# Cibiv/NextGenMap

Hardware: AMD Instinct MI355X
Metric: mapped reads/sec + SW Gcells/sec, 150bp vs GRCh38, at 1/2/4/8 MI355X (higher is better)
Workload: dtype int32

## Files before the change

include/ngm_pipeline.h:

```cpp
#ifndef NGM_PIPELINE_H
#define NGM_PIPELINE_H

#include <stddef.h>
#include <stdint.h>

#ifdef __cplusplus
extern "C" {
#endif

typedef struct ngm_ref ngm_ref;
typedef struct ngm_mapper ngm_mapper;

typedef struct ngm_ref_params {
	int kmer;
	int kmer_skip;
	int bin_size;
} ngm_ref_params;

const char *ngm_pipeline_last_error(void);

ngm_ref *ngm_ref_create(int device, const ngm_ref_params *p, int n_contigs, const char *const *names,
		const uint8_t *const *seqs, const uint64_t *lens);
ngm_ref *ngm_ref_create_from_fasta(int device, const ngm_ref_params *p, const char *path);
ngm_ref *ngm_ref_create_from_cache(int device, const ngm_ref_params *params, const char *fasta_path);
// ... 85 lines not shown
	int paired;
	int min_insert_size, max_insert_size;
	int min_mq;
	float min_identity, min_residues;
	int no_unal;
	const char *rg_id;
	int bs_mapping;
	int slam_seq;
	int bam;
} ngm_sam_options;
int ngm_mapper_set_sam_options(ngm_mapper *m, const ngm_sam_options *o);
typedef struct ngm_sam_read {
	uint32_t name_off;
	uint16_t name_len;
	uint16_t qual_len;
} ngm_sam_read;
long long ngm_mapper_map_sam(ngm_mapper *m, int n, const char *reads, const char *quals, const char *names, size_t names_bytes,
		const ngm_sam_read *meta, char *out, size_t out_cap, uint64_t stats[3], float *kernel_ms);
long long ngm_mapper_map_sam_trimmed(ngm_mapper *m, int n, const char *reads, const char *quals, const char *names, size_t names_bytes,
		const ngm_sam_read *meta, const uint16_t *polya_trimmed, char *out, size_t out_cap, uint64_t stats[3], float *kernel_ms);
int ngm_mapper_sam_fetch(ngm_mapper *m, char *out, size_t out_cap);

typedef struct ngm_pair_state ngm_pair_state;
ngm_pair_state *ngm_pair_state_create(void);
void ngm_pair_state_destroy(ngm_pair_state *ps);
int ngm_mapper_set_pair_state(ngm_mapper *m, ngm_pair_state *ps);
int ngm_mapper_set_batch_seq(ngm_mapper *m, uint64_t seq);
int ngm_mapper_set_fast_pairing(ngm_mapper *m, int on);

typedef struct ngm_bgzf ngm_bgzf;
ngm_bgzf *ngm_bgzf_create(int device);
void ngm_bgzf_destroy(ngm_bgzf *z);
size_t ngm_bgzf_bound(size_t n);
long long ngm_bgzf_compress(ngm_bgzf *z, const void *raw, size_t n, void *out, size_t out_cap);
long long ngm_bgzf_compress_device(ngm_bgzf *z, const void *d_raw, size_t n, void *out, size_t out_cap);
float ngm_bgzf_last_kernel_ms(const ngm_bgzf *z);
size_t ngm_bgzf_inflated_size(const void *members, size_t n);
long long ngm_bgzf_inflate(ngm_bgzf *z, const void *members, size_t n, void *out, size_t out_cap);

typedef struct ngm_bam_sort ngm_bam_sort;
typedef struct ngm_bam_sort_params {
	int device;
	size_t chunk_bytes;
	size_t max_bytes;
} ngm_bam_sort_params;
ngm_bam_sort *ngm_bam_sort_create(const ngm_bam_sort_params *p);
void ngm_bam_sort_destroy(ngm_bam_sort *s);
int ngm_bam_sort_add(ngm_bam_sort *s, uint64_t seq, const void *records, size_t n_bytes);
int ngm_bam_sort_finish(ngm_bam_sort *s, int n_ref);
long long ngm_bam_sort_next(ngm_bam_sort *s, void *out, size_t out_cap);
long long ngm_bam_sort_index(ngm_bam_sort *s, uint64_t first_member_offset, void *out, size_t out_cap);
int ngm_bam_sort_stats(const ngm_bam_sort *s, uint64_t counts[5], float ms[5]);
int ngm_mapper_set_bam_sorter(ngm_mapper *m, ngm_bam_sort *s);

void *ngm_host_alloc(size_t bytes);
void ngm_host_free(void *p);

int ngm_host_pin_to_device_node(int device);

int ngm_mapper_set_reference_score_buffer(ngm_mapper *m, int entries);
int ngm_mapper_lost_pairs(ngm_mapper *m, uint64_t *out);
int ngm_mapper_set_reference_cs_batch(ngm_mapper *m, int reads);

int ngm_mapper_path_counters(ngm_mapper *m, uint64_t out[8]);

int ngm_mapper_order_table_reads(ngm_mapper *m, uint64_t *out);

int ngm_debug_pair_walk(uint32_t cnt_a, int len_a, uint32_t cnt_b, int len_b, const uint32_t *loc, const uint32_t *sv, const float *score, const uint32_t *rank,
		float cutoff, int min_insert, int max_insert, uint32_t *out_a, uint32_t *out_b, int *mq_a, int *mq_b, uint64_t cap, float *combo_score, int *combo_dist, int *combo_a, int *combo_b,
		uint64_t *n_combo);

int ngm_debug_pair_eval(uint64_t n, const float *pair_score, const int *dist, const int *ia, const int *ib, int avg, int out_all[6], int out_kept[6]);

int ngm_debug_select_top1(int device, int n_reads, const uint32_t *base, const uint32_t *count, uint64_t n_cand, const float *scores, const uint32_t *loc,
		const uint32_t *strand_votes, uint32_t *winner, int32_t *mapq, int32_t *n_best, float *best_score);

int ngm_debug_align_finish(void *engine , int mode, int n, const char *const *ref, const char *const *qry, void *out ,
		uint64_t *n_fallback);

int ngm_debug_expand_pairs(int device, int n_reads, const uint32_t *base, const uint32_t *count, uint64_t n_cand, uint32_t *out);

int ngm_mapper_heavy_counters(ngm_mapper *m, uint64_t out[4]);

int ngm_mapper_cs_counters(ngm_mapper *m, uint64_t out[3]);

typedef struct ngm_stats_comm ngm_stats_comm;
int ngm_stats_unique_id(char hex[257]);
ngm_stats_comm *ngm_stats_comm_create(int device, int rank, int world, const char *hex);
int ngm_stats_allreduce(ngm_stats_comm *c, int64_t v[8]);
void ngm_stats_comm_destroy(ngm_stats_comm *c);
int ngm_mapper_last_pair_stats(ngm_mapper *m, uint64_t out[3]);

int ngm_mapper_last_kernel_ms(ngm_mapper *m, float ms[8]);
float ngm_mapper_last_order_replay_ms(ngm_mapper *m);

int ngm_mapper_set_argos(ngm_mapper *m, float min_score);
long long ngm_mapper_map_argos(ngm_mapper *m, int n, const char *reads, const char *names, size_t names_bytes, const ngm_sam_read *meta,
		char *out, size_t out_cap, uint64_t stats[3], float *kernel_ms);
int ngm_argos_prolog(const ngm_ref *ref, uint64_t total_reads, char *out, size_t cap);
int ngm_mapper_argos_counters(ngm_mapper *m, uint64_t out[4]);
int ngm_mapper_argos_path_counters(ngm_mapper *m, uint64_t out[2]);
int ngm_debug_argos_order(uint32_t n, const float *score, const uint32_t *rank, float min_score, int read_len, int match_bonus, uint32_t *order, uint32_t out[3]);

#ifdef __cplusplus
}
#endif
#endif
```

nextgenmap_amd/csrc/cigar_device.h:

```cpp
#pragma once

#include <hip/hip_runtime.h>
#include <stdint.h>

#include "sw_device.h"
#include "affine_device.h"

namespace ngm {

struct CigarDevOut {
	uint32_t cig_off, md_off;
	uint16_t cig_len, md_len;
	int32_t position_offset, qstart, qend, nm;
	float identity, score_token;
	int32_t flags;
};

__device__ __forceinline__ uint32_t packed_class(const uint32_t *base, int m_base, int j) {
	const uint32_t w = base[(size_t) (m_base + (j >> 3)) * kSlots];
	const int b = j & 7;
	return (b < 4) ? (w >> (8 * b)) & 15u : (w >> (8 * (b - 4) + 4)) & 15u;
}
__device__ __forceinline__ char class_to_char(uint32_t c) {
	switch (c) { case 0: return 'A'; case 1: return 'C'; case 2: return 'G'; case 3: return 'T'; case 4: return 'x'; case 5: return 'N'; default: return 0; }
// ... 78 lines not shown
						if (rc == 4u) odd_symbol = true;
						const bool eq = (op == 1) && ((variant_cpu && !alt) ? (rc <= 3u && rc == fc) : (rc == fc));
						if (eq) { match += 1; md_eq += 1; in_x_run = false; }
						else {
							if (alt && rc == bs_from && fc == bs_to) match += 1; else mismatch += 1;
							if (mo > lim) { fits = false; break; }
							if (!in_x_run) { mo += dev_put_num(mdp + mo, md_eq); md_eq = 0; in_x_run = true; }
							mdp[mo++] = class_to_char(fc);
						}
						m_len += 1; ref_i += 1; read_i += 1;
					}
				} else if (op == 3) {
					in_x_run = false;
					if (m_len > 0) { co += dev_put_num(cg + co, m_len); cg[co++] = 'M'; m_len = 0; }
					co += dev_put_num(cg + co, len); cg[co++] = 'D';
					mo += dev_put_num(mdp + mo, md_eq); md_eq = 0;
					mdp[mo++] = '^';
					for (int t = 0; t < len; ++t) { if (mo > lim) { fits = false; break; } mdp[mo++] = class_to_char(fclass(ref0 + ref_i)); ref_i += 1; }
					mismatch += len;
				} else {
					in_x_run = false;
					if (m_len > 0) { co += dev_put_num(cg + co, m_len); cg[co++] = 'M'; m_len = 0; }
					co += dev_put_num(cg + co, len); cg[co++] = 'I';
					read_i += len;
					mismatch += len;
				}
			}
			if (co > lim || mo > lim) fits = false;
			if (fits) {
				mo += dev_put_num(mdp + mo, md_eq);
				if (m_len > 0) { co += dev_put_num(cg + co, m_len); cg[co++] = 'M'; }
				if (trail > 0) {
					if (hard_clip == 1) { co += dev_put_num(cg + co, trail); cg[co++] = 'H'; }
					else if (silent_clip != 1) { co += dev_put_num(cg + co, trail); cg[co++] = 'S'; }
					o.qend = trail;
				}
			}
			o.identity = (float) match * 1.0f / (float) total;
			o.nm = mismatch;
			o.score_token = (float) read_i;
			o.position_offset = ref0;
			o.flags = ((fits && !odd_symbol) ? 1 : 0) | 2;
		}
	}
	}
	o.cig_len = (uint16_t) co; o.md_len = (uint16_t) mo;
	const uint32_t need = (live && (o.flags & 1)) ? (uint32_t) (co + mo) : 0u;
	uint32_t incl = need;
	const int lane = threadIdx.x & 63, wv = threadIdx.x >> 6;
#pragma unroll
	for (int d = 1; d < 64; d <<= 1) { const uint32_t t = __shfl_up(incl, d); if (lane >= d) incl += t; }
	if (lane == 63) s_wave[wv] = incl;
	__syncthreads();
	uint32_t before = incl - need, total = 0;
#pragma unroll
	for (int w2 = 0; w2 < 4; ++w2) { if (w2 < wv) before += s_wave[w2]; total += s_wave[w2]; }
	if (threadIdx.x == 0) s_base = total ? atomicAdd(cursor, (unsigned long long) total) : 0ull;
	__syncthreads();
	const unsigned long long base = s_base;
	if (!live) return;
	if (need) {
		if (base + total > capacity) o.flags &= ~1;
		else {
			const unsigned long long off = base + before;
			o.cig_off = (uint32_t) off; o.md_off = (uint32_t) off + o.cig_len;
			for (int t = 0; t < co; ++t) bytes[off + t] = cg[t];
			for (int t = 0; t < mo; ++t) bytes[off + co + t] = mdp[t];
		}
	}
	out[j] = o;
}

constexpr int kFinishRows = 8;

__device__ __forceinline__ uint32_t finish_sel8(uint32_t w0, uint32_t w1, uint32_t w2, uint32_t w3, uint32_t w4, uint32_t w5, uint32_t w6, uint32_t w7, int k) {
	const uint32_t a0 = (k & 1) ? w1 : w0, a1 = (k & 1) ? w3 : w2, a2 = (k & 1) ? w5 : w4, a3 = (k & 1) ? w7 : w6;
	const uint32_t b0 = (k & 2) ? a1 : a0, b1 = (k & 2) ? a3 : a2;
	return (k & 4) ? b1 : b0;
}

template <bool NIBBLES>
__global__ __launch_bounds__(256) void affine_finish_kernel(int n, const uint32_t *__restrict__ dirs, const int32_t *__restrict__ records,
		const uint32_t *__restrict__ packed, const uint16_t *__restrict__ lens, int q, int CP, int RW, int FW, CigarDevOut *__restrict__ out,
		char *__restrict__ bytes, unsigned long long capacity, unsigned long long *__restrict__ counters) {
	__shared__ char s_rows[256 * kCigarRow];
	__shared__ uint32_t s_wave[4];
	__shared__ unsigned long long s_base;
	const int j = blockIdx.x * blockDim.x + threadIdx.x;
	const bool live = j < n;
	const int lane = threadIdx.x & 63, wv = threadIdx.x >> 6;
	constexpr int lim = kCigarRow - 16;
	constexpr int WS = NIBBLES ? 3 : 2;
	const int DW = NIBBLES ? aff_nib_words(CP) : aff_dir_words(CP);
	char *row = s_rows + (size_t) threadIdx.x * kCigarRow;
	int pos = kCigarRow;
	auto put_back = [&](int num, char tag) {
		row[--pos] = tag;
		unsigned u = (unsigned) num;
		do { row[--pos] = (char) ('0' + u % 10u); u /= 10u; } while (u);
	};
	bool fits = true;
	int h = 0, v = 0, flags = 0, len_v = 0;
	if (live) {
		const int32_t *rec = records + (size_t) j * 8;
		flags = rec[3]; h = rec[6]; v = rec[7];
		len_v = (int) lens[j];
	}
	const int qend = len_v - v;
	if (live && qend > 0) put_back(qend, 'S');
	const int trail = kCigarRow - pos;
	const uint32_t *dp = dirs + (size_t) (j >> 6) * q * DW * kSlots + lane;
	const uint32_t *pk = packed + (size_t) (j >> 6) * (RW + FW) * kSlots + lane;
	int cur = -1, curlen = 0, total = 0, n_match = 0, n_mis = 0;
	bool done = !live, first = true, in_v = false, in_h = false;
	auto flush = [&]() {
		if (cur < 0) return;
		if (kCigarRow - pos - trail > lim) { fits = false; done = true; return; }
		put_back(curlen, cur == 1 ? 'M' : cur == 2 ? 'I' : 'D');
		total += cur == 1 ? curlen : 1;
	};
	auto emit = [&](int op) {
		if (op == cur) { ++curlen; return; }
		flush();
		cur = op; curlen = 1;
	};
	int gtop = (v - 1) >> 3;
#pragma unroll
	for (int s = 1; s < 64; s <<= 1) gtop = max(gtop, __shfl_xor(gtop, s));
	for (int g = gtop; g >= 0; --g) {
		const int r0 = g * kFinishRows;
		const bool act = !done && v - 1 >= r0;
		const int d0 = h - v;
		const int wi = min(max(d0 >> WS, 0), DW - 1);
		const int f0 = min(max((r0 + d0) >> 3, 0), FW - 1);
		uint32_t W[kFinishRows];
#pragma unroll
		for (int k = 0; k < kFinishRows; ++k) W[k] = (act && r0 + k <= v - 1) ? dp[((size_t) (r0 + k) * DW + wi) * kSlots] : 0u;
		const uint32_t rdw = act ? pk[(size_t) g * kSlots] : 0u;
		const uint32_t fw0 = act ? pk[(size_t) (RW + f0) * kSlots] : 0u;
		const uint32_t fw1 = (act && f0 + 1 < FW) ? pk[(size_t) (RW + f0 + 1) * kSlots] : 0u;
		if (act && (!first || (NIBBLES && flags == 0)) && !in_v && !in_h) {
			const int kc = v - 1 - r0;
			if (d0 >= 0 && d0 < CP && (d0 >> WS) == wi && ((r0 + d0) >> 3) == f0 && f0 + 1 < FW) {
				const int sh = NIBBLES ? 4 * (d0 & 7) : 8 * (d0 & 3);
				uint32_t m = 0;
#pragma unroll
				for (int k = 0; k < kFinishRows; ++k) m |= (NIBBLES ? (uint32_t) (((W[k] >> sh) & 0xCu) == 4u) : ((W[k] >> sh) & 1u)) << k;
				const uint32_t stop = ~m & ((2u << kc) - 1u);
				const int lo = stop ? 32 - __clz((int) stop) : 0;
				const int run = kc + 1 - lo;
				if (run > 0) {
					auto spread = [](uint32_t x) -> unsigned long long { return (unsigned long long) (x & 0x0F0F0F0Fu) | ((unsigned long long) ((x >> 4) & 0x0F0F0F0Fu) << 32); };
					const unsigned long long ones = 0x0101010101010101ull, RB = spread(rdw), A = spread(fw0), B = spread(fw1);
					const int o = (r0 + d0) & 7;
					const unsigned long long WB = o ? (A >> (8 * o)) | (B << (64 - 8 * o)) : A;
					const unsigned long long differ = (((RB ^ WB) + 0x0F0F0F0F0F0F0F0Full) >> 4) & ones;
					const unsigned long long odd = (RB >> 2) & (~RB | (RB >> 1)) & ones;
					const unsigned long long upto = kc == 7 ? ~0ull : (1ull << (8 * (kc + 1))) - 1ull;
					const int mis = __popcll((differ | odd) & upto & ~((1ull << (8 * lo)) - 1ull));
					n_mis += mis; n_match += run - mis;
					if (cur != 1) { flush(); cur = 1; curlen = 0; }
					curlen += run; h -= run; v -= run;
					first = false;
				}
			}
		}
		while (!done && v - 1 >= r0) {
			const int d = h - v;
			uint32_t tv = 0u;
			if (h > 0 && d >= 0 && d < CP) {
				const int w = d >> WS;
				const uint32_t word = (w == wi) ? finish_sel8(W[0], W[1], W[2], W[3], W[4], W[5], W[6], W[7], v - 1 - r0) : dp[((size_t) (v - 1) * DW + w) * kSlots];
				tv = NIBBLES ? aff_trace_from_nibble((word >> (4 * (d & 7))) & 15u, d, CP) : (word >> (8 * (d & 3))) & 0xFFu;
			}
// ... 74 lines not shown
```

nextgenmap_amd/csrc/engine_internal.h:

```cpp
#pragma once

#include <algorithm>

#include <hip/hip_runtime.h>

#include <cstdint>
#include <string>

#include "../../include/ngm_hip.h"
#include "sw_device.h"
#include "affine_device.h"
#include "cigar_device.h"
#include "jit.h"

namespace ngm {
template <typename T>
struct DevBuf {
	T *p = nullptr;
	size_t cap = 0;
	int reserve(size_t n) {
		if (n <= cap) return 0;
		if (p) (void) hipFree(p);
		p = nullptr;
		cap = 0;
		const size_t want = n + std::min<size_t>(n / 8, ((size_t) 64 << 20) / sizeof(T));
		if (hipMalloc(&p, want * sizeof(T)) == hipSuccess) { cap = want; return 0; }
		if (hipMalloc(&p, n * sizeof(T)) != hipSuccess) return -1;
		cap = n;
		return 0;
	}
	void release() { if (p) (void) hipFree(p); p = nullptr; cap = 0; }
};

template <typename T>
struct PinnedBuf {
	T *p = nullptr;
	size_t cap = 0;
	int reserve(size_t n) {
		if (n <= cap) return 0;
		if (p) (void) hipHostFree(p);
		p = nullptr;
		cap = 0;
		const size_t want = n + std::min<size_t>(n / 8, ((size_t) 64 << 20) / sizeof(T));
		if (hipHostMalloc(&p, want * sizeof(T), hipHostMallocDefault) == hipSuccess) { cap = want; return 0; }
		if (hipHostMalloc(&p, n * sizeof(T), hipHostMallocDefault) != hipSuccess) return -1;
		cap = n;
		return 0;
	}
	void release() { if (p) (void) hipHostFree(p); p = nullptr; cap = 0; }
};

}

struct ngm_hip_ctx {
	int device = 0;
	ngm_hip_params prm{};
	ngm::SwConst K{};
	ngm::AffConst KA{};
	const ngm::JitKernels *jit = nullptr;
	int q = 0, c = 0, rl = 0, RW = 0, FW = 0;
	int max_batch = 0;
	hipStream_t stream = nullptr;
	ngm::DevBuf<uint32_t> packed;
	ngm::DevBuf<uint16_t> lens, blk_rows;
	ngm::DevBuf<uint8_t> d_ref, d_qry, d_pair_dir;
	const uint8_t *pair_dir = nullptr;
	ngm::DevBuf<float> d_scores;
	ngm::DevBuf<uint32_t> dirs;
	ngm::DevBuf<int32_t> d_records;
	ngm::DevBuf<uint16_t> d_runs;
	ngm::PinnedBuf<uint8_t> h_ref, h_qry;
	ngm::PinnedBuf<float> h_scores;
	ngm::PinnedBuf<int32_t> h_records;
	ngm::PinnedBuf<uint16_t> h_runs;
	bool profiling = false;
	hipEvent_t ev[4] = {nullptr, nullptr, nullptr, nullptr};
	bool ev_valid[3] = {false, false, false};
	bool trace_nibbles = false;
	std::string error;
};

namespace ngm {
int engine_reserve(ngm_hip_ctx *ctx, int n);
int engine_score_packed(ngm_hip_ctx *ctx, int mode, int n, float *d_scores, hipStream_t st);
struct AlignFinish {
	CigarDevOut *out;
	char *bytes;
	unsigned long long capacity;
	unsigned long long *counters;
};
int engine_align_packed(ngm_hip_ctx *ctx, int mode, int n, int32_t *d_records, uint16_t *d_runs, int run_stride, hipStream_t st, const AlignFinish *fin = nullptr);
int engine_affine_traceback_packed(ngm_hip_ctx *ctx, int n, int32_t *d_records, uint16_t *d_runs, int run_stride, hipStream_t st);
}
```

nextgenmap_amd/csrc/gather_device.h:

```cpp
#pragma once

#include <hip/hip_runtime.h>
#include <stdint.h>

#include "sw_device.h"

namespace ngm {

struct WindowGeom {
	uint64_t concat_len;
	int buffer_len;
	int half_corridor;
};

__device__ __forceinline__ uint32_t window_class(const uint32_t *__restrict__ genome, const WindowGeom &G, uint64_t offset, int j) {
	uint64_t len = (uint64_t) G.buffer_len - 2;
	if (offset >= G.concat_len) return 5u;
	uint64_t end = 0;
	if (offset + len > G.concat_len) { end = offset + len - G.concat_len; len -= end; }
	const uint64_t emitted = ((offset & 1) ? 1 : 0) + 2 * ((len + 1) / 2);
	const uint64_t jj = (uint64_t) j;
	if (jj < emitted) {
		if ((len & 1) && jj == emitted - 1) return 4u;
		const uint64_t pos = offset + jj;
// ... 159 lines not shown
		for (uint32_t j = b + (uint32_t) lane; j < b + n; j += 64u) top1_add(S, scores[j], ((uint64_t) pair_loc[j] << 1) | (pair_sv[j] & 1u), j);
#pragma unroll
		for (int d = 1; d < 64; d <<= 1) {
			Top1State o;
			o.best = __shfl_xor(S.best, d); o.below = __shfl_xor(S.below, d); o.num = __shfl_xor(S.num, d);
			o.key = ((uint64_t) (uint32_t) __shfl_xor((int) (uint32_t) (S.key >> 32), d) << 32) | (uint32_t) __shfl_xor((int) (uint32_t) S.key, d);
			o.idx = (uint32_t) __shfl_xor((int) S.idx, d);
			S = top1_merge(S, o);
		}
		uint32_t aidx = S.idx;
		if (S.best < 0.0f) {
			uint64_t akey = ~0ull;
			aidx = 0xFFFFFFFFu;
			for (uint32_t j = b + (uint32_t) lane; j < b + n; j += 64u) {
				const uint64_t key = ((uint64_t) pair_loc[j] << 1) | (pair_sv[j] & 1u);
				if (key < akey) { akey = key; aidx = j; }
			}
#pragma unroll
			for (int d = 1; d < 64; d <<= 1) {
				const uint64_t ok = ((uint64_t) (uint32_t) __shfl_xor((int) (uint32_t) (akey >> 32), d) << 32) | (uint32_t) __shfl_xor((int) (uint32_t) akey, d);
				const uint32_t oi = (uint32_t) __shfl_xor((int) aidx, d);
				if (ok < akey || (ok == akey && oi < aidx)) { akey = ok; aidx = oi; }
			}
		}
		if (lane == 0) top1_store(S, aidx, rr, scores, winner, mapq, n_best, best_score);
	}
}

__global__ void pair_simple_kernel(int n_pairs, const uint32_t *__restrict__ cand_base, const uint32_t *__restrict__ cand_count,
		const float *__restrict__ scores, const uint32_t *__restrict__ pair_loc, const uint16_t *__restrict__ read_len, int min_d, int max_d,
		int32_t *__restrict__ mapq, int32_t *__restrict__ n_best, int32_t *__restrict__ info, uint32_t *__restrict__ list_small, uint32_t *__restrict__ list_large,
		uint32_t *__restrict__ list_counts) {
	const int pi = blockIdx.x * blockDim.x + threadIdx.x;
	const bool live = pi < n_pairs;
	const int rb = 2 * pi, ra = 2 * pi + 1;
	const uint32_t ca = live ? cand_count[ra] : 1u, cb = live ? cand_count[rb] : 1u;
	{
		const bool choice = live && (ca != 1u || cb != 1u) && ca != 0u && cb != 0u && list_counts != nullptr;
		const bool small = choice && ca <= 64u && cb <= 64u, large = choice && !small;
		const unsigned long long ms = __ballot(small), ml = __ballot(large);
		const int lane = threadIdx.x & 63;
		const unsigned long long below = (1ull << lane) - 1ull;
		uint32_t bs = 0, bl = 0;
		if (ms && lane == (int) __builtin_ctzll(ms)) bs = atomicAdd(&list_counts[0], (uint32_t) __popcll(ms));
		if (ml && lane == (int) __builtin_ctzll(ml)) bl = atomicAdd(&list_counts[1], (uint32_t) __popcll(ml));
		if (ms) bs = (uint32_t) __builtin_amdgcn_readlane((int) bs, (int) __builtin_ctzll(ms));
		if (ml) bl = (uint32_t) __builtin_amdgcn_readlane((int) bl, (int) __builtin_ctzll(ml));
		if (small) { const uint32_t at = bs + (uint32_t) __popcll(ms & below); list_small[at] = (uint32_t) pi; info[pi] = -2 - (int32_t) at; }
		if (large) { const uint32_t at = bl + (uint32_t) __popcll(ml & below); list_large[at] = (uint32_t) pi; info[pi] = -2 - (int32_t) (at + (1u << 30)); }
		if (choice) return;
	}
	if (!live) return;
	if (ca != 1u || cb != 1u) { info[pi] = -1; return; }
	const uint32_t ba = cand_base[ra], bb = cand_base[rb];
	const uint64_t l1 = pair_loc[ba], l2 = pair_loc[bb];
	const int cur = (int) ((l2 > l1) ? l2 - l1 + (uint64_t) read_len[rb] : l1 - l2 + (uint64_t) read_len[ra]);
	const float ps = scores[ba] + scores[bb];
	const bool found = cur > min_d && cur < max_d && ps > 0.0f;
	if (found) { mapq[ra] = 60; mapq[rb] = 60; n_best[ra] = 0; n_best[rb] = 0; }
	info[pi] = found ? ((cur << 1) | 1) : 0;
}

__global__ __launch_bounds__(256) void expand_pairs_kernel(int n_reads, const uint32_t *__restrict__ cand_base, const uint32_t *__restrict__ cand_count,
		uint32_t *__restrict__ pair_read) {
	__shared__ uint32_t s_big[256], s_nbig;
	const int tid = threadIdx.x, lane = tid & 63, wv = tid >> 6;
	if (tid == 0) s_nbig = 0;
	__syncthreads();
	const int r = blockIdx.x * 256 + tid;
	if (r < n_reads) {
		const uint32_t b = cand_base[r], n = cand_count[r];
		if (n <= kSelectSmall) { for (uint32_t j = 0; j < n; ++j) pair_read[b + j] = (uint32_t) r; }
		else s_big[atomicAdd(&s_nbig, 1u)] = (uint32_t) tid;
	}
	__syncthreads();
	const uint32_t nbig = s_nbig;
	for (uint32_t i = (uint32_t) wv; i < nbig; i += 4u) {
		const int rr = blockIdx.x * 256 + (int) s_big[i];
		const uint32_t b = cand_base[rr], n = cand_count[rr];
		for (uint32_t j = (uint32_t) lane; j < n; j += 64u) pair_read[b + j] = (uint32_t) rr;
	}
}

__global__ void collect_winners_kernel(int n_reads, const uint32_t *__restrict__ winner, const uint32_t *__restrict__ pair_loc,
		const uint32_t *__restrict__ pair_sv, const uint32_t *__restrict__ slot_of_read, uint32_t *__restrict__ a_read,
		uint32_t *__restrict__ a_loc, uint32_t *__restrict__ a_sv) {
	const int r = blockIdx.x * blockDim.x + threadIdx.x;
	if (r >= n_reads) return;
	const uint32_t w = winner[r];
	if (w == 0xFFFFFFFFu) return;
	const uint32_t s = slot_of_read[r];
	a_read[s] = (uint32_t) r;
	a_loc[s] = pair_loc[w];
	a_sv[s] = pair_sv[w];
}

__global__ void compact_runs_kernel(int n, int32_t *__restrict__ records, const uint16_t *__restrict__ runs, int run_stride,
		uint16_t *__restrict__ out, unsigned long long *__restrict__ cursor) {
	const int i = blockIdx.x * blockDim.x + threadIdx.x;
	if (i >= n) return;
	int32_t *rec = records + (size_t) i * 8;
	const int nr = rec[0] ? rec[4] : 0;
	const unsigned long long off = nr ? atomicAdd(cursor, (unsigned long long) nr) : 0ull;
	rec[6] = (int32_t) off;
	const uint16_t *src = runs + (size_t) i * run_stride;
	for (int k = 0; k < nr; ++k) out[off + k] = src[k];
}

}
```

nextgenmap_amd/csrc/mapper.cpp:

```cpp
#define NGM_SAM_KERNELS
#include "mapper_internal.h"
#include <rocprim/rocprim.hpp>
#include "align_device.h"
#include "gather_device.h"

using ngm::DevGuard;
using ngm::GpuStage;
using ngm::run_cs;
using ngm::cs_host_arrays;
using ngm::candidate_order;
using ngm::candidate_order_wait;

namespace ngm {
StageLock g_stage_lock[16][2];
std::atomic<long long> g_stage_hold_us[3], g_stage_wait_us[3];
}
using ngm::g_stage_hold_us;
using ngm::g_stage_wait_us;

namespace {

int upload_reads(ngm_mapper *m, int n, const char *reads) {
	const size_t bytes = (size_t) n * m->prm.qry_max_len;
	if (m->d_reads.reserve(bytes)) { ngm::pipeline_set_error("out of device memory (reads)"); return -12; }
	MAP_HIP_TRY(hipMemcpyAsync(m->d_reads.p, reads, bytes, hipMemcpyHostToDevice, m->st));
	return 0;
}

std::atomic<int> g_live_mappers{0};
template <typename F>
void parallel_for(int n, F f, int min_grain = 0) {
	ngm::ThreadPool::instance().parallel_for(n, f, min_grain > 0 ? min_grain : 2048);
}

char class_char(uint8_t c) {
	static const char t[8] = {'A', 'C', 'G', 'T', 'x', 'N', 0, 0};
	return t[c & 7];
}

void host_window(const ngm_ref *r, uint64_t offset, int buffer_len, int want, char *out) {
	const uint64_t concat_len = r->n_bases - 1;
	uint64_t len = (uint64_t) buffer_len - 2;
	if (offset >= concat_len) { memset(out, 'N', want); return; }
	uint64_t end = 0;
	if (offset + len > concat_len) { end = offset + len - concat_len; len -= end; }
	const uint64_t emitted = ((offset & 1) ? 1 : 0) + 2 * ((len + 1) / 2);
	for (int j = 0; j < want; ++j) {
		const uint64_t jj = (uint64_t) j;
		char ch;
		if (jj < emitted) ch = ((len & 1) && jj == emitted - 1) ? 'x' : class_char(r->host_cls[offset + jj]);
		else if (jj < emitted + end) ch = 'x';
		else ch = 0;
		out[j] = ch;
	}
}

}

namespace ngm {
int score_candidates(ngm_mapper *m, int n, uint64_t np, int alt_dir) {
	const ngm_ref *r = m->ref;
	ngm_hip_ctx *eng = m->eng;
	const int q = m->prm.qry_max_len, c = m->prm.corridor;
	hipLaunchKernelGGL(ngm::expand_pairs_kernel, dim3((n + 255) / 256), dim3(256), 0, m->st, n, m->d_cand_base.p, m->d_cand_count.p, m->d_pair_read.p);
	const int nb = (int) ((np + ngm::kSlots - 1) / ngm::kSlots);
	ngm::WindowGeom Gs{r->n_bases - 1, ((q + c) | 1) + 1, c >> 1};
	hipLaunchKernelGGL(ngm::gather_pairs_kernel, dim3(nb), dim3(256), 0, m->st, m->d_reads.p, m->d_read_len.p, q, r->d_genome, Gs,
			m->d_pair_read.p, m->d_out_loc.p, m->d_out_sv.p, (int) np, eng->RW, eng->FW, eng->packed.p, eng->lens.p, eng->blk_rows.p, alt_dir);
	MAP_HIP_TRY(hipGetLastError());
	MAP_HIP_TRY(hipEventRecord(m->ev[2], m->st));
	if (int rc = ngm::engine_score_packed(eng, m->prm.mode, (int) np, m->d_scores.p, m->st)) { ngm::pipeline_set_error("%s", ngm_hip_last_error(eng)); return rc; }
	MAP_HIP_TRY(hipEventRecord(m->ev[3], m->st));
	return 0;
}
}

extern "C" {

int ngm_ref_decode(const ngm_ref *r, uint64_t offset, int buffer_len, char *out) {
	DevGuard g(r->device);
	if (buffer_len < 2) return -22;
	const uint64_t concat_len = r->n_bases - 1;
	if (offset >= concat_len) { memset(out, 0, buffer_len); return 0; }
	const int q = 8, c = buffer_len;
	const int RW = ngm::read_words(q), FW = (q + c + 7) / 8 + 1;
	uint32_t *d_out; uint16_t *d_lens, *d_rows, *d_rl; uint8_t *d_reads; uint32_t *d_pr, *d_pl, *d_ps;
	MAP_HIP_TRY(hipMalloc(&d_out, (size_t) (RW + FW) * 64 * 4)); MAP_HIP_TRY(hipMalloc(&d_lens, 128)); MAP_HIP_TRY(hipMalloc(&d_rows, 8));
	MAP_HIP_TRY(hipMalloc(&d_rl, 8)); MAP_HIP_TRY(hipMalloc(&d_reads, q)); MAP_HIP_TRY(hipMalloc(&d_pr, 4)); MAP_HIP_TRY(hipMalloc(&d_pl, 4)); MAP_HIP_TRY(hipMalloc(&d_ps, 4));
	MAP_HIP_TRY(hipMemset(d_rl, 0, 8)); MAP_HIP_TRY(hipMemset(d_reads, 0, q)); MAP_HIP_TRY(hipMemset(d_pr, 0, 4)); MAP_HIP_TRY(hipMemset(d_ps, 0, 4));
	const uint32_t loc = (uint32_t) offset;
	MAP_HIP_TRY(hipMemcpy(d_pl, &loc, 4, hipMemcpyHostToDevice));
	ngm::WindowGeom G{concat_len, buffer_len, 0};
	hipLaunchKernelGGL(ngm::gather_pairs_kernel, dim3(1), dim3(256), 0, 0, d_reads, d_rl, q, r->d_genome, G, d_pr, d_pl, d_ps, 1, RW, FW, d_out, d_lens, d_rows);
	MAP_HIP_TRY(hipGetLastError());
	std::vector<uint32_t> h((size_t) (RW + FW) * 64);
	MAP_HIP_TRY(hipMemcpy(h.data(), d_out, h.size() * 4, hipMemcpyDeviceToHost));
	for (int j = 0; j < buffer_len; ++j) {
		const uint32_t w = h[(size_t) (RW + j / 8) * 64];
		const int b = j & 7;
		const uint32_t cls = (b < 4) ? (w >> (8 * b)) & 15u : (w >> (8 * (b - 4) + 4)) & 15u;
		out[j] = class_char((uint8_t) cls);
	}
	(void) hipFree(d_out); (void) hipFree(d_lens); (void) hipFree(d_rows); (void) hipFree(d_rl); (void) hipFree(d_reads); (void) hipFree(d_pr); (void) hipFree(d_pl); (void) hipFree(d_ps);
	return 1;
}

ngm_mapper *ngm_mapper_create(const ngm_ref *ref, const ngm_mapper_params *p) {
	if (!ref || !p) { ngm::pipeline_set_error("ngm_mapper_create: null argument"); return nullptr; }
	DevGuard g(ref->device);
	if (p->qry_max_len < ref->prm.kmer + 1 || p->qry_max_len > 1024) { ngm::pipeline_set_error("ngm_mapper_create: qry_max_len %d out of range", p->qry_max_len); return nullptr; }
	ngm_hip_params ep{};
	ep.abi_version = NGM_HIP_ABI_VERSION;
	ep.qry_max_len = p->qry_max_len; ep.corridor = p->corridor;
	ep.match_bonus = p->match_bonus; ep.mismatch_penalty = p->mismatch_penalty; ep.gap_read_penalty = p->gap_read_penalty; ep.gap_ref_penalty = p->gap_ref_penalty;
	ep.variant = p->variant; ep.hard_clip = p->hard_clip; ep.silent_clip = p->silent_clip; ep.max_batch = 0;
	ep.personality = p->personality; ep.gap_extend_penalty = p->gap_extend_penalty;
	if (p->bs_mapping) {
		if (ref->prm.kmer_skip != 0) { ngm::pipeline_set_error("ngm_mapper_create: bisulfite mapping needs a reference index built with kmer_skip 0 (src/PrefixTable.cpp:199-207)"); return nullptr; }
		if (p->mode != 0) { ngm::pipeline_set_error("ngm_mapper_create: '--bs-mapping' and '--end-to-end' can't be used at the same time"); return nullptr; }
		ep.alt_scoring = ep.alt_cigar = NGM_ALT_BISULFITE; ep.match_bonus_tt = p->match_bonus_tt; ep.match_bonus_tc = p->match_bonus_tc;
	}
	if (p->slam_seq) {
		if (p->bs_mapping) { ngm::pipeline_set_error("ngm_mapper_create: '--bs-mapping' and '--slam-seq' can't be used at the same time!"); return nullptr; }
		if (p->personality != NGM_PERSONALITY_LINEAR) { ngm::pipeline_set_error("ngm_mapper_create: '--slam-seq' needs the default (linear-gap) personality: EndToEndAffine produces no per-base records (Align::ExtendedData)"); return nullptr; }
		ep.alt_cigar = NGM_ALT_SLAMSEQ;
		if (p->slam_seq & 2) { ep.alt_scoring = NGM_ALT_SLAMSEQ; ep.match_bonus_tt = p->match_bonus_tt; ep.match_bonus_tc = p->match_bonus_tc; }
	}
	ngm_hip_ctx *eng = ngm_hip_create(ref->device, &ep);
	if (!eng) { ngm::pipeline_set_error("%s", ngm_hip_last_error(nullptr)); return nullptr; }
	ngm_mapper *m = new ngm_mapper();
	++g_live_mappers;
	m->ref = ref; m->prm = *p; m->eng = eng; m->st = eng->stream;
	{
		int lo = 0, hi = 0;
		(void) hipDeviceGetStreamPriorityRange(&lo, &hi);
		if (hipStreamCreateWithPriority(&m->st_hi, hipStreamNonBlocking, hi) != hipSuccess) m->st_hi = nullptr;
	}
	m->max_kfreq = p->max_kfreq > 0 ? p->max_kfreq : ref->auto_max_kfreq;
	for (auto &e : m->ev) (void) hipEventCreate(&e);
	for (auto &e : m->cev) (void) hipEventCreate(&e);
	for (auto &e : m->oev) (void) hipEventCreate(&e);
	if (ngm::cs_configure(m, p) != 0) { ngm_mapper_destroy(m); return nullptr; }
	return m;
}

void ngm_mapper_destroy(ngm_mapper *m) {
	if (!m) return;
	if (--g_live_mappers == 0 && getenv("NGM_HIP_HOST_TIMING"))
		fprintf(stderr, "[ngm-hip] GPU stage lock, ms summed over all mappers: search + score held %.1f (waited %.1f) | align held %.1f (waited %.1f) | SAM text held %.1f (waited %.1f)\n",
				g_stage_hold_us[0] / 1e3, g_stage_wait_us[0] / 1e3, g_stage_hold_us[1] / 1e3, g_stage_wait_us[1] / 1e3, g_stage_hold_us[2] / 1e3, g_stage_wait_us[2] / 1e3);
	DevGuard g(m->ref->device);
	(void) hipStreamSynchronize(m->st);
	ngm_bgzf_destroy(m->bz);
	if (m->st_hi) { (void) hipStreamSynchronize(m->st_hi); (void) hipStreamDestroy(m->st_hi); }
	ngm::cs_release(m);
	ngm::argos_release(m);
	m->d_reads.release(); m->d_scores.release(); m->d_best.release(); m->d_pair_read.release();
	m->d_winner.release(); m->d_a_read.release(); m->d_a_loc.release(); m->d_a_sv.release(); m->d_mapq.release(); m->d_nbest.release();
	m->d_records.release(); m->d_runs.release(); m->d_runs_c.release();
	m->d_pair_info.release(); m->p_pair_info.release(); m->d_sam_contig_start.release();
	m->d_pair_out.release(); m->d_pair_top.release(); m->d_pair_tied_n.release(); m->d_pair_list.release(); m->p_pair_out.release(); m->p_pair_top.release(); m->p_pair_tied_n.release();
	m->d_sam_contig_names.release(); m->d_sam_rg.release(); m->d_sam_names.release(); m->d_sam_text.release(); m->d_sam_contig_off.release(); m->d_sam_len.release(); m->d_sam_off.release();
	m->d_sam_quals.release(); m->d_sam_polya.release(); m->d_sam_meta.release(); m->d_sam_refs.release(); m->d_sam_hits.release(); m->p_sam_hits.release(); m->p_sam_refs.release(); m->p_sam_extra.release();
	for (auto &e : m->ev) if (e) (void) hipEventDestroy(e);
	for (auto &e : m->cev) if (e) (void) hipEventDestroy(e);
	for (auto &e : m->oev) if (e) (void) hipEventDestroy(e);
	m->p_winner.release(); m->p_loc.release(); m->p_sv.release(); m->p_mapq.release(); m->p_nbest.release(); m->p_rec.release();
	m->p_best.release(); m->p_scores.release(); m->p_runs.release();
	m->d_str.release(); m->d_cigout.release(); m->p_cigout.release(); m->p_str.release();
	ngm_hip_destroy(m->eng);
	delete m;
}

int ngm_mapper_cs(ngm_mapper *m, int n, const char *reads, uint32_t *cand_offsets, float *max_votes) {
	if (!m || n < 0) return -22;
	DevGuard g(m->ref->device);
	if (n == 0) { cand_offsets[0] = 0; m->n_reads = 0; m->n_cand = 0; return 0; }
	if (int r = upload_reads(m, n, reads)) return r;
	m->cs_paired = false;
	if (int r = run_cs(m, n)) return r;
	if (int r = cs_host_arrays(m)) return r;
	uint32_t acc = 0;
	for (int i = 0; i < n; ++i) { cand_offsets[i] = acc; acc += m->h_count[i]; max_votes[i] = m->h_maxv[i]; }
	cand_offsets[n] = acc;
	return 0;
}

int ngm_mapper_cs_fetch(ngm_mapper *m, uint64_t *loc, uint8_t *strand, float *votes) {
	if (!m) return -22;
	DevGuard g(m->ref->device);
	if (m->n_cand == 0) return 0;
	std::vector<uint32_t> hl(m->n_cand), hs(m->n_cand);
	MAP_HIP_TRY(hipMemcpy(hl.data(), m->d_out_loc.p, m->n_cand * 4, hipMemcpyDeviceToHost));
	MAP_HIP_TRY(hipMemcpy(hs.data(), m->d_out_sv.p, m->n_cand * 4, hipMemcpyDeviceToHost));
	size_t w = 0;
	std::vector<uint32_t> order;
	for (int i = 0; i < m->n_reads; ++i) {
		const uint32_t b = m->h_base[i], c = m->h_count[i];
		order.resize(c);
		std::iota(order.begin(), order.end(), b);
		std::sort(order.begin(), order.end(), [&](uint32_t x, uint32_t y) {
			const uint64_t kx = ((uint64_t) hl[x] << 1) | (hs[x] & 1), ky = ((uint64_t) hl[y] << 1) | (hs[y] & 1);
			return kx < ky;
		});
		for (uint32_t j : order) { loc[w] = hl[j]; strand[w] = (uint8_t) (hs[j] & 1); votes[w] = (float) (hs[j] >> 1); ++w; }
	}
	return 0;
}

struct SamCall { const char *quals; const char *names; size_t names_bytes; const ngm::SamMeta *meta; const uint16_t *polya; char *out; size_t out_cap; uint64_t *stats; long long text_bytes; float kernel_ms; };
static int map_impl(ngm_mapper *m, int n, const char *reads, const void *d_reads_ext, ngm_hit *hits, char *cigars, char *mds, bool paired, SamCall *sam = nullptr);

int ngm_mapper_map_se(ngm_mapper *m, int n, const char *reads, ngm_hit *hits, char *cigars, char *mds) {
	return map_impl(m, n, reads, nullptr, hits, cigars, mds, false);
}
int ngm_mapper_map_se_resident(ngm_mapper *m, int n, const char *reads, const void *d_reads_ext, ngm_hit *hits, char *cigars, char *mds) {
	return map_impl(m, n, reads, d_reads_ext, hits, cigars, mds, false);
}
int ngm_mapper_map_pe(ngm_mapper *m, int n, const char *reads, ngm_hit *hits, char *cigars, char *mds) {
	return map_impl(m, n, reads, nullptr, hits, cigars, mds, true);
}
int ngm_mapper_map_pe_resident(ngm_mapper *m, int n, const char *reads, const void *d_reads_ext, ngm_hit *hits, char *cigars, char *mds) {
	return map_impl(m, n, reads, d_reads_ext, hits, cigars, mds, true);
}

int ngm_mapper_set_sam_options(ngm_mapper *m, const ngm_sam_options *o) {
	if (!m || !o) return -22;
	DevGuard g(m->ref->device);
	m->sam_opt = *o;
	m->sam_opt.rg_id = nullptr;
	if (o->bam && !m->bz) { m->bz = ngm_bgzf_create(m->ref->device); if (!m->bz) return -12; }
	m->sam_rg = o->rg_id ? o->rg_id : "";
	const ngm_ref *r = m->ref;
	std::string names;
	std::vector<uint32_t> off(r->contigs.size() + 1, 0);
	for (size_t i = 0; i < r->contigs.size(); ++i) { off[i] = (uint32_t) names.size(); names += r->contigs[i].name; }
	off[r->contigs.size()] = (uint32_t) names.size();
	if (m->d_sam_contig_names.reserve(names.size() + 16) || m->d_sam_contig_off.reserve(off.size()) || m->d_sam_rg.reserve(m->sam_rg.size() + 16)) { ngm::pipeline_set_error("out of device memory (SAM options)"); return -12; }
	MAP_HIP_TRY(hipMemcpy(m->d_sam_contig_names.p, names.data(), names.size(), hipMemcpyHostToDevice));
	MAP_HIP_TRY(hipMemcpy(m->d_sam_contig_off.p, off.data(), off.size() * 4, hipMemcpyHostToDevice));
	if (!m->sam_rg.empty()) MAP_HIP_TRY(hipMemcpy(m->d_sam_rg.p, m->sam_rg.data(), m->sam_rg.size(), hipMemcpyHostToDevice));
	{
		std::vector<uint64_t> starts(r->contigs.size() + 1, 0);
		for (size_t i = 0; i < r->contigs.size(); ++i) starts[i] = r->contigs[i].start;
		if (m->d_sam_contig_start.reserve(starts.size())) { ngm::pipeline_set_error("out of device memory (SAM options)"); return -12; }
		MAP_HIP_TRY(hipMemcpy(m->d_sam_contig_start.p, starts.data(), starts.size() * 8, hipMemcpyHostToDevice));
	}
	m->sam_ready = true;
	return 0;
}

static_assert(sizeof(ngm_sam_read) == sizeof(ngm::SamMeta) && sizeof(ngm_sam_read) == 8, "ngm_sam_read is the device's per-read record");
// ... 298 lines not shown
		}
		bool released = false;
		~PairTurn() { release(); }
	} pair_turn{m, paired && m->ps != nullptr};
	if (n < 0) return -22;
	if (paired && m->prm.topn > 1) { ngm::pipeline_set_error("Paired end mode with topn > 1 not yet supported."); return -38; }
	if (paired && (n & 1)) { ngm::pipeline_set_error("paired-end batches need an even number of reads"); return -22; }
	if (n == 0) return 0;
	const ngm_ref *r = m->ref;
	DevGuard g(r->device);
	ngm_hip_ctx *eng = m->eng;
	const int q = m->prm.qry_max_len, c = m->prm.corridor, mode = m->prm.mode;
	const size_t str_stride = (size_t) 4 * std::max(1, q);
	for (auto &x : m->ms) x = 0.f;
	m->order_ms = 0.f;

	ngm::DevBuf<uint8_t> own = m->d_reads;
	struct Restore { ngm_mapper *m; ngm::DevBuf<uint8_t> own; bool on; ~Restore() { if (on) m->d_reads = own; } } restore{m, own, d_reads_ext != nullptr};
	if (d_reads_ext) { m->d_reads.p = (uint8_t *) d_reads_ext; m->d_reads.cap = (size_t) n * q; }
	const bool host_timing = getenv("NGM_HIP_HOST_TIMING") != nullptr;
	const int alt_cigar = m->prm.bs_mapping ? NGM_ALT_BISULFITE : (m->prm.slam_seq ? NGM_ALT_SLAMSEQ : NGM_ALT_NONE);
	const int alt_dir = alt_cigar ? (paired ? 2 : 1) : 0;
	auto now = [] { return std::chrono::steady_clock::now(); };
	auto tp0 = now();
	double t_stage[6] = {0, 0, 0, 0, 0, 0};
	auto lap = [&](int k) { auto t = now(); t_stage[k] += std::chrono::duration<double, std::milli>(t - tp0).count(); tp0 = t; };
	MAP_HIP_TRY(hipEventRecord(m->ev[0], m->st));
	if (!d_reads_ext) if (int rc = upload_reads(m, n, reads)) return rc;
	if (sam) {
		if (!m->sam_ready || (!paired) != (!m->sam_opt.paired) || m->prm.topn > 1) { ngm::pipeline_set_error("ngm_mapper_map_sam: call ngm_mapper_set_sam_options first (single alignments only; paired as configured)"); return -22; }
		if ((unsigned long long) n * (unsigned long long) (2 * q + 1024) + sam->names_bytes >= 0xFFFFFFFFull) { ngm::pipeline_set_error("ngm_mapper_map_sam: the text of %d reads may exceed the 32-bit offsets of a batch: use smaller batches", n); return -75; }
		if (m->d_sam_quals.reserve((size_t) n * q) || m->d_sam_names.reserve(sam->names_bytes + 16) || m->d_sam_meta.reserve(n) || m->p_sam_hits.reserve(n) || m->p_sam_refs.reserve(n) ||
				m->d_sam_hits.reserve(n) || m->d_sam_refs.reserve(n)) { ngm::pipeline_set_error("out of memory (SAM stage)"); return -12; }
		MAP_HIP_TRY(hipMemcpyAsync(m->d_sam_quals.p, sam->quals, (size_t) n * q, hipMemcpyHostToDevice, m->st));
		if (sam->names_bytes) MAP_HIP_TRY(hipMemcpyAsync(m->d_sam_names.p, sam->names, sam->names_bytes, hipMemcpyHostToDevice, m->st));
		MAP_HIP_TRY(hipMemcpyAsync(m->d_sam_meta.p, sam->meta, (size_t) n * sizeof(ngm::SamMeta), hipMemcpyHostToDevice, m->st));
		if (sam->polya && n > 0) {
			if (m->d_sam_polya.reserve((size_t) n)) { ngm::pipeline_set_error("out of memory (SAM stage)"); return -12; }
			MAP_HIP_TRY(hipMemcpyAsync(m->d_sam_polya.p, sam->polya, (size_t) n * sizeof(uint16_t), hipMemcpyHostToDevice, m->st));
		}
		hits = m->p_sam_hits.p;
	}
	GpuStage stage_cs(m);
	m->cs_paired = paired;
	if (int rc = run_cs(m, n, &stage_cs)) return rc;
	MAP_HIP_TRY(hipEventRecord(m->ev[1], m->st));
	const uint64_t np = m->n_cand;
	lap(0);
	if (const char *dump = getenv("NGM_HIP_DUMP_COUNTS")) {
		if (int rc = cs_host_arrays(m)) return rc;
		if (FILE *f = fopen(dump, "ab")) { fwrite(m->h_count.data(), 4, (size_t) n, f); fclose(f); }
	}

	if (m->p_winner.reserve(n) || m->p_mapq.reserve(n) || m->p_nbest.reserve(n) || m->p_best.reserve(n) || m->p_loc.reserve(np + 1) ||
			m->p_sv.reserve(np + 1) || (paired && m->p_scores.reserve(np + 1))) { ngm::pipeline_set_error("out of pinned host memory"); return -12; }
	uint32_t *h_winner = m->p_winner.p, *h_loc = m->p_loc.p, *h_sv = m->p_sv.p;
	int32_t *h_mapq = m->p_mapq.p, *h_nbest = m->p_nbest.p;
	float *h_best = m->p_best.p, *h_scores = m->p_scores.p;
	if (np == 0) { if (int rc = cs_host_arrays(m)) return rc; for (int i = 0; i < n; ++i) { h_winner[i] = 0xFFFFFFFFu; h_mapq[i] = 0; h_nbest[i] = 0; h_best[i] = 0.f; } }
	std::vector<int> pair_flags(n, 0);
	auto reference_buffer_walk = [&]() {
		uint64_t tot = m->scores_so_far, at = m->reads_so_far;
		const uint64_t rb = m->ref_cs_batch > 0 ? (uint64_t) m->ref_cs_batch : 0;
		const uint64_t sb = m->ref_score_buffer > 0 ? (uint64_t) m->ref_score_buffer : 0;
		uint64_t next_flush = rb ? (at + rb - 1) / rb * rb : ~0ull;
		uint64_t fill = sb ? tot % sb : 0;
		for (int pi = 0; pi < n / 2; ++pi, at += 2) {
			while (at > next_flush) next_flush += rb;
			if (at == next_flush) { tot = 0; fill = 0; next_flush += rb; }
			const uint32_t c1 = m->h_count[2 * pi], c2 = m->h_count[2 * pi + 1];
			tot += (uint64_t) c1 + c2;
			if (!sb) continue;
			fill += c1;
			const bool full_at_first_mate = c1 > 0 && fill % sb == 0;
			fill = (fill + c2) % sb;
			if (full_at_first_mate && c2 == 0) {
				++m->lost_pairs;
				pair_flags[2 * pi] = pair_flags[2 * pi + 1] = NGM_PAIR_LOST;
				h_winner[2 * pi] = h_winner[2 * pi + 1] = 0xFFFFFFFFu;
			}
		}
		m->scores_so_far = tot; m->reads_so_far = at;
	};
	if (np > 0) {
		if (m->d_pair_read.reserve(np) || m->d_scores.reserve(np) || m->d_winner.reserve(n) || m->d_mapq.reserve(n) || m->d_nbest.reserve(n) ||
				m->d_best.reserve(n)) { ngm::pipeline_set_error("out of device memory (score stage)"); return -12; }
		if (int rc = ngm::engine_reserve(eng, (int) np)) { ngm::pipeline_set_error("%s", ngm_hip_last_error(eng)); return rc; }
		stage_cs.acquire();
		if (int rc = ngm::score_candidates(m, n, np, alt_dir)) return rc;
		hipLaunchKernelGGL(ngm::select_top1_kernel, dim3((n + 255) / 256), dim3(256), 0, m->st, n, m->d_cand_base.p, m->d_cand_count.p,
				m->d_scores.p, m->d_out_loc.p, m->d_out_sv.p, m->d_winner.p, m->d_mapq.p, m->d_nbest.p, m->d_best.p);
		MAP_HIP_TRY(hipGetLastError());
		const bool pe_select = paired && !m->fast_pairing;
		const bool simple_on_gpu = pe_select && m->prm.strata == 0;
		static const bool pair_choice_host = getenv("NGM_HIP_HOST_PAIR_CHOICE") != nullptr, pair_choice_force = getenv("NGM_HIP_GPU_PAIR_CHOICE") != nullptr;
		const bool choice_on_gpu = simple_on_gpu && !pair_choice_host && (pair_choice_force || np >= 3ull * (uint64_t) n);
		if (simple_on_gpu) {
			const size_t npairs = (size_t) n / 2;
			if (m->d_pair_info.reserve(npairs + 1) || m->p_pair_info.reserve(npairs + 1)) { ngm::pipeline_set_error("out of memory (pair selection)"); return -12; }
			if (choice_on_gpu) {
				if (m->d_pair_out.reserve(2 * npairs + 2) || m->d_pair_top.reserve(npairs + 1) || m->d_pair_tied_n.reserve(4) || m->p_pair_tied_n.reserve(4) || m->d_pair_list.reserve(3 * npairs + 2)) {
					ngm::pipeline_set_error("out of memory (pair selection)"); return -12; }
				MAP_HIP_TRY(hipMemsetAsync(m->d_pair_tied_n.p, 0, 16, m->st));
			}
			uint32_t *counts = choice_on_gpu ? m->d_pair_tied_n.p + 1 : nullptr;
			hipLaunchKernelGGL(ngm::pair_simple_kernel, dim3((n / 2 + 255) / 256), dim3(256), 0, m->st, n / 2, m->d_cand_base.p, m->d_cand_count.p, m->d_scores.p,
					m->d_out_loc.p, m->d_read_len.p, m->prm.min_insert_size, m->prm.max_insert_size > 0 ? m->prm.max_insert_size : INT_MAX, m->d_mapq.p, m->d_nbest.p, m->d_pair_info.p,
					m->d_pair_list.p, m->d_pair_list.p + npairs, counts);
			MAP_HIP_TRY(hipGetLastError());
			if (choice_on_gpu) {
				const int min_d = m->prm.min_insert_size, max_d = m->prm.max_insert_size > 0 ? m->prm.max_insert_size : INT_MAX;
				const float cutoff = m->prm.pair_score_cutoff > 0 ? m->prm.pair_score_cutoff : 0.9f;
				uint32_t *const huge_list = m->d_pair_list.p + 2 * npairs, *const huge_count = m->d_pair_tied_n.p + 3;
				hipLaunchKernelGGL((ngm::pair_choice_kernel<64, 64>), dim3((unsigned) std::min<size_t>(npairs, 8192)), dim3(64), ngm::pair_choice_lds_bytes(64), m->st, (const uint32_t *) m->d_pair_list.p, (const uint32_t *) counts,
						m->d_cand_base.p, m->d_cand_count.p, m->d_scores.p, m->d_out_loc.p, m->d_read_len.p, min_d, max_d, cutoff, m->d_pair_out.p, m->d_pair_top.p, m->d_pair_tied_n.p, (uint32_t) npairs,
						(uint32_t *) nullptr, (uint32_t *) nullptr, (const uint32_t *) nullptr);
				hipLaunchKernelGGL((ngm::pair_choice_kernel<ngm::kPairThreads, ngm::kPairCap>), dim3((unsigned) std::min<size_t>(npairs, 1024)), dim3(ngm::kPairThreads), ngm::pair_choice_lds_bytes(ngm::kPairCap), m->st,
						(const uint32_t *) (m->d_pair_list.p + npairs), (const uint32_t *) (counts + 1), m->d_cand_base.p, m->d_cand_count.p, m->d_scores.p, m->d_out_loc.p, m->d_read_len.p, min_d, max_d, cutoff,
						m->d_pair_out.p + npairs, m->d_pair_top.p, m->d_pair_tied_n.p, (uint32_t) npairs, huge_list, huge_count, (const uint32_t *) nullptr);
				static const bool huge_attr = [] { (void) hipFuncSetAttribute((const void *) ngm::pair_choice_kernel<1024, ngm::kPairCapHuge>, hipFuncAttributeMaxDynamicSharedMemorySize, (int) ngm::pair_choice_lds_bytes(ngm::kPairCapHuge)); return true; }();
				(void) huge_attr;
				hipLaunchKernelGGL((ngm::pair_choice_kernel<1024, ngm::kPairCapHuge>), dim3((unsigned) std::min<size_t>(npairs, 256)), dim3(1024), ngm::pair_choice_lds_bytes(ngm::kPairCapHuge), m->st,
						(const uint32_t *) huge_list, (const uint32_t *) huge_count, m->d_cand_base.p, m->d_cand_count.p, m->d_scores.p, m->d_out_loc.p, m->d_read_len.p, min_d, max_d, cutoff,
						m->d_pair_out.p + npairs, m->d_pair_top.p, m->d_pair_tied_n.p, (uint32_t) npairs, (uint32_t *) nullptr, (uint32_t *) nullptr, (const uint32_t *) (m->d_pair_list.p + npairs));
				MAP_HIP_TRY(hipGetLastError());
				MAP_HIP_TRY(hipMemcpyAsync(m->p_pair_tied_n.p, m->d_pair_tied_n.p, 16, hipMemcpyDeviceToHost, m->st));
			}
			MAP_HIP_TRY(hipMemcpyAsync(m->p_pair_info.p, m->d_pair_info.p, (size_t) (n / 2) * 4, hipMemcpyDeviceToHost, m->st));
		}
		MAP_HIP_TRY(hipEventRecord(m->ev[4], m->st));
		MAP_HIP_TRY(hipMemcpyAsync(h_winner, m->d_winner.p, (size_t) n * 4, hipMemcpyDeviceToHost, m->st));
		MAP_HIP_TRY(hipMemcpyAsync(h_mapq, m->d_mapq.p, (size_t) n * 4, hipMemcpyDeviceToHost, m->st));
		MAP_HIP_TRY(hipMemcpyAsync(h_nbest, m->d_nbest.p, (size_t) n * 4, hipMemcpyDeviceToHost, m->st));
		MAP_HIP_TRY(hipMemcpyAsync(h_best, m->d_best.p, (size_t) n * 4, hipMemcpyDeviceToHost, m->st));
		MAP_HIP_TRY(hipMemcpyAsync(h_loc, m->d_out_loc.p, np * 4, hipMemcpyDeviceToHost, m->st));
		MAP_HIP_TRY(hipMemcpyAsync(h_sv, m->d_out_sv.p, np * 4, hipMemcpyDeviceToHost, m->st));
		if (paired) MAP_HIP_TRY(hipMemcpyAsync(h_scores, m->d_scores.p, np * 4, hipMemcpyDeviceToHost, m->st));
		stage_cs.done_after(m->ev[4]);
		MAP_HIP_TRY(hipStreamSynchronize(m->st));
		if (int rc = cs_host_arrays(m)) return rc;
		if (choice_on_gpu) {
			const size_t npairs = (size_t) n / 2;
			const size_t n_small = std::min<size_t>(m->p_pair_tied_n.p[1], npairs), n_large = std::min<size_t>(m->p_pair_tied_n.p[2], npairs), nt = std::min<size_t>(m->p_pair_tied_n.p[0], npairs);
			if (m->p_pair_out.reserve(2 * npairs + 2) || m->p_pair_top.reserve(nt + 1)) { ngm::pipeline_set_error("out of pinned host memory"); return -12; }
			if (n_small) MAP_HIP_TRY(hipMemcpyAsync(m->p_pair_out.p, m->d_pair_out.p, n_small * sizeof(ngm::PairOut), hipMemcpyDeviceToHost, m->st));
			if (n_large) MAP_HIP_TRY(hipMemcpyAsync(m->p_pair_out.p + npairs, m->d_pair_out.p + npairs, n_large * sizeof(ngm::PairOut), hipMemcpyDeviceToHost, m->st));
			if (nt) MAP_HIP_TRY(hipMemcpyAsync(m->p_pair_top.p, m->d_pair_top.p, nt * sizeof(ngm::PairTop), hipMemcpyDeviceToHost, m->st));
			MAP_HIP_TRY(hipStreamSynchronize(m->st));
		}
		lap(1);
		if ((!paired || m->fast_pairing) && m->prm.topn <= 1) {
			std::vector<uint32_t> tied;
			for (int i = 0; i < n; ++i) if (h_nbest[i] != 1 && m->h_count[i] > 1) tied.push_back((uint32_t) i);
			if (!tied.empty()) {
				uint32_t *h_rank = nullptr;
				if (int rc = candidate_order(m, tied, np, &h_rank)) return rc;
				if (m->p_scores.reserve(np + 1)) { ngm::pipeline_set_error("out of pinned host memory"); return -12; }
				h_scores = m->p_scores.p;
				MAP_HIP_TRY(hipMemcpy(h_scores, m->d_scores.p, np * 4, hipMemcpyDeviceToHost));
				for (uint32_t i : tied) {
					const uint32_t b = m->h_base[i], cnt = m->h_count[i];
					float best = h_scores[b];
					for (uint32_t c = 1; c < cnt; ++c) best = std::max(best, h_scores[b + c]);
					uint32_t pick = 0xFFFFFFFFu, pick_rank = ngm::kCsOrderUnknown;
					bool known = true;
					for (uint32_t c = 0; c < cnt; ++c) if (h_scores[b + c] == best || !(best > 0.0f)) {
						if (h_rank[b + c] == ngm::kCsOrderUnknown) { known = false; break; }
						if (h_rank[b + c] < pick_rank) { pick_rank = h_rank[b + c]; pick = b + c; }
					}
					if (known && pick != 0xFFFFFFFFu) { h_winner[i] = pick; h_best[i] = h_scores[pick]; }
				}
			}
		}
		if (pe_select) {
			const bool pe_strata = m->prm.strata != 0;
			auto commit = [&](int ra, int rb, bool found, int wa, int wb, int mqa, int mqb, int equal) {
				if (found && pe_strata && equal > 0) {
					h_winner[ra] = h_winner[rb] = 0xFFFFFFFFu;
					h_mapq[ra] = h_mapq[rb] = 0;
					pair_flags[ra] = pair_flags[rb] = NGM_PAIR_SELECTED;
				} else if (found) {
					h_winner[ra] = (uint32_t) wa; h_winner[rb] = (uint32_t) wb;
					h_mapq[ra] = mqa; h_mapq[rb] = mqb;
					h_nbest[ra] = h_nbest[rb] = equal;
					h_best[ra] = h_scores[wa]; h_best[rb] = h_scores[wb];
					pair_flags[ra] = pair_flags[rb] = NGM_PAIR_SELECTED;
				} else {
					pair_flags[ra] = pair_flags[rb] = NGM_PAIR_FAILED;
				}
			};
			auto len_of = [&](int rd) { return (int) strnlen(reads + (size_t) rd * q, q); };
			auto run_pair = [&](int pi, long sum, long cnt, const uint32_t *rank, int *wa, int *wb, int *mqa, int *mqb, int *equal, int *dist, bool *found, PairTies *ties) {
				const int rb = 2 * pi, ra = 2 * pi + 1;
				select_pair(m, sum, cnt, dist, m->h_base[ra], m->h_count[ra], len_of(ra), m->h_base[rb], m->h_count[rb], len_of(rb), h_loc, h_sv, h_scores, rank, wa, wb, mqa, mqb, equal, found, ties);
			};
			struct Tied { int pi; bool found, dup, open; int dmin, dmax, mqa, mqb; long avg_lo, avg_hi; int n_top, top_d[8], top_a[8], top_b[8]; long gap_sum, gap_cnt; int dist; int seq; };
			auto tq0 = now(); double tq[5] = {0, 0, 0, 0, 0};
			auto qlap = [&](int k) { auto t = now(); tq[k] += std::chrono::duration<double, std::milli>(t - tq0).count(); tq0 = t; };
			std::mutex tied_mu;
			std::vector<Tied> tied;
			std::vector<uint32_t> se_tied;
			struct Chunk { int plo; std::vector<Tied> tied; std::vector<uint32_t> se; long tail_sum, tail_cnt; };
			std::vector<Chunk> chunks;
			auto se_check = [&](std::vector<uint32_t> &out, int i) { if (h_nbest[i] != 1 && m->h_count[i] > 1) out.push_back((uint32_t) i); };
			const ngm::PairOut *h_po = choice_on_gpu ? m->p_pair_out.p : nullptr;
			const ngm::PairTop *h_pt = choice_on_gpu ? m->p_pair_top.p : nullptr;
			std::atomic<long> n_host_walk{0};
			parallel_for(n / 2, [&](int plo, int phi) {
				std::vector<Tied> local;
				std::vector<uint32_t> local_se;
				long gsum = 0, gcnt = 0, walked = 0;
				for (int pi = plo; pi < phi; ++pi) {
					const int rb = 2 * pi, ra = 2 * pi + 1;
					const int pinfo = simple_on_gpu ? m->p_pair_info.p[pi] : -1;
					if (simple_on_gpu && pinfo >= 0) {
						const int info = m->p_pair_info.p[pi];
						if (info & 1) { pair_flags[ra] = pair_flags[rb] = NGM_PAIR_SELECTED; gsum += info >> 1; ++gcnt; }
						else pair_flags[ra] = pair_flags[rb] = NGM_PAIR_FAILED;
						continue;
					}
// ... 151 lines not shown
				const PairOutcome o = eval_pair_seq(seqs[t.seq], (int) (m->pair_dist_sum / std::max(1L, m->pair_dist_count)));
				const int rb = 2 * pi, ra = 2 * pi + 1;
				commit(ra, rb, o.found, o.wa, o.wb, o.mqa, o.mqb, o.equal);
				if (o.found && !(pe_strata && o.equal > 0)) { m->pair_dist_sum += o.dist; m->pair_dist_count += 1; }
				if (!o.found) { if (h_nbest[ra] != 1 && m->h_count[ra] > 1) first_sorted((uint32_t) ra); if (h_nbest[rb] != 1 && m->h_count[rb] > 1) first_sorted((uint32_t) rb); }
			}
			m->pair_dist_sum += carry_sum; m->pair_dist_count += carry_cnt;
			pair_turn.release();
			qlap(4);
			if (host_timing) {
				g_walk_probe = true;
				const double pn = (double) std::max<uint64_t>(1, g_walk_ns[5].load());
				fprintf(stderr, "[ngm-hip] pair walks so far: %.0f pairs; per pair: sorts %.1f us, rest of the walk %.1f us, %.0f candidates, %.0f above the cut-off, %.0f combinations looked at\n", pn,
						g_walk_ns[0].load() / pn / 1e3, g_walk_ns[1].load() / pn / 1e3, g_walk_ns[2].load() / pn, g_walk_ns[3].load() / pn, g_walk_ns[4].load() / pn);
			}
			if (host_timing) fprintf(stderr, "[ngm-hip] pair selection: %zu tied pairs, %zu picked for the order replay + %zu single-end ties, %zu open in the turn, %zu of them late; %ld pairs walked on the host; "
					"ms: pass 1 %.2f | order replay %.2f | pass 3 %.2f | turn: pass 2 %.2f, late + pass 4 %.2f\n", tied.size(), picked.size(), se_tied.size(), n_open, late.size(), (long) n_host_walk, tq[0], tq[1], tq[2], tq[3], tq[4]);
		}
	}
	if (paired && (np == 0 || m->fast_pairing)) { pair_turn.acquire(); reference_buffer_walk(); pair_turn.release(); }
	if (paired && np > 0 && m->prm.strata)
		parallel_for(n, [&](int lo, int hi) { for (int i = lo; i < hi; ++i) if (!(pair_flags[i] & NGM_PAIR_SELECTED) && h_nbest[i] > 1) { h_winner[i] = 0xFFFFFFFFu; h_mapq[i] = 0; } }, 16384);
	const int topn = (!paired && m->prm.topn > 1) ? m->prm.topn : 1;
	std::vector<uint32_t> tn_pairs;
	if (!paired && np > 0 && (topn > 1 || m->prm.strata)) {
		if (topn == 1) {
			for (int i = 0; i < n; ++i) if (h_nbest[i] > 1) { h_winner[i] = 0xFFFFFFFFu; h_mapq[i] = 0; }
		} else {
			if (m->p_scores.reserve(np + 1)) { ngm::pipeline_set_error("out of pinned host memory"); return -12; }
			h_scores = m->p_scores.p;
			MAP_HIP_TRY(hipMemcpy(h_scores, m->d_scores.p, np * 4, hipMemcpyDeviceToHost));
			tn_pairs.assign((size_t) n * topn, 0xFFFFFFFFu);
			uint32_t *h_rank_tn = nullptr;
			{
				std::vector<uint32_t> need;
				for (int i = 0; i < n; ++i) {
					const uint32_t b = m->h_base[i], cnt = m->h_count[i];
					bool eq = false;
					for (uint32_t x = 0; x + 1 < cnt && !eq; ++x) for (uint32_t y = x + 1; y < cnt; ++y) if (h_scores[b + x] == h_scores[b + y]) { eq = true; break; }
					if (eq) need.push_back((uint32_t) i);
				}
				if (!need.empty()) if (int rc = candidate_order(m, need, np, &h_rank_tn)) return rc;
			}
			parallel_for(n, [&](int lo, int hi) {
				std::vector<uint32_t> v;
				for (int i = lo; i < hi; ++i) {
					const uint32_t b = m->h_base[i], cnt = m->h_count[i];
					if (cnt == 0) continue;
					v.resize(cnt);
					std::iota(v.begin(), v.end(), b);
					auto by_place = [&](uint32_t x, uint32_t y) { return h_loc[x] != h_loc[y] ? h_loc[x] < h_loc[y] : (h_sv[x] & 1u) < (h_sv[y] & 1u); };
					bool ranked = h_rank_tn != nullptr;
					for (uint32_t x = b; ranked && x < b + cnt; ++x) ranked = h_rank_tn[x] != ngm::kCsOrderUnknown;
					if (ranked) {
						std::sort(v.begin(), v.end(), [&](uint32_t x, uint32_t y) { return h_rank_tn[x] != h_rank_tn[y] ? h_rank_tn[x] < h_rank_tn[y] : by_place(x, y); });
						std::sort(v.begin(), v.end(), [&](uint32_t x, uint32_t y) { return h_scores[x] > h_scores[y]; });
					} else {
						std::sort(v.begin(), v.end(), by_place);
						std::stable_sort(v.begin(), v.end(), [&](uint32_t x, uint32_t y) { return h_scores[x] > h_scores[y]; });
					}
					int ntop = 1;
					while (ntop < (int) cnt && h_scores[v[0]] == h_scores[v[ntop]]) ++ntop;
					h_nbest[i] = ntop;
					int ns = 0;
					if (ntop <= topn || !m->prm.strata) {
						ns = m->prm.strata ? ntop : std::min<int>((int) cnt, topn);
						int mq = 60;
						if (cnt > 1) { const float bs = h_scores[v[0]], s2 = h_scores[v[1]]; mq = (bs > 0 && s2 >= 0) ? (int) ceilf(60.0f * (bs - s2) / bs) : 0; }
						h_mapq[i] = mq;
					} else {
						h_mapq[i] = 0;
					}
					for (int t = 0; t < ns; ++t) tn_pairs[(size_t) i * topn + t] = v[t];
					h_winner[i] = ns > 0 ? v[0] : 0xFFFFFFFFu;
					h_best[i] = h_scores[v[0]];
				}
			});
		}
	}
	stage_cs.done();
	lap(2);
	std::vector<uint32_t> a_read((size_t) n * topn), a_loc((size_t) n * topn), a_sv((size_t) n * topn), a_out((size_t) n * topn), a_pair((size_t) n * topn);
	int na = 0;
	if (topn == 1 || np == 0) {
		const int slices = std::max(1, std::min(256, n / 4096));
		std::vector<int> first(slices + 1, 0);
		parallel_for(slices, [&](int lo, int hi) {
			for (int s2 = lo; s2 < hi; ++s2) {
				const int i0 = (int) ((long long) n * s2 / slices), i1 = (int) ((long long) n * (s2 + 1) / slices);
				int cnt = 0;
				for (int i = i0; i < i1; ++i) cnt += h_winner[i] != 0xFFFFFFFFu;
				first[s2 + 1] = cnt;
			}
		}, 1);
		for (int s2 = 0; s2 < slices; ++s2) first[s2 + 1] += first[s2];
		na = first[slices];
		parallel_for(slices, [&](int lo, int hi) {
			for (int s2 = lo; s2 < hi; ++s2) {
				const int i0 = (int) ((long long) n * s2 / slices), i1 = (int) ((long long) n * (s2 + 1) / slices);
				int at = first[s2];
				for (int i = i0; i < i1; ++i) if (h_winner[i] != 0xFFFFFFFFu) {
					a_read[at] = (uint32_t) i; a_out[at] = (uint32_t) i; a_pair[at] = h_winner[i]; a_loc[at] = h_loc[h_winner[i]]; a_sv[at] = h_sv[h_winner[i]]; ++at;
				}
			}
		}, 1);
	} else {
		for (int i = 0; i < n; ++i) for (int t = 0; t < topn; ++t) {
			const uint32_t w = tn_pairs[(size_t) i * topn + t];
			if (w == 0xFFFFFFFFu) break;
			a_read[na] = i; a_out[na] = (uint32_t) (i * topn + t); a_pair[na] = w; a_loc[na] = h_loc[w]; a_sv[na] = h_sv[w]; ++na;
		}
	}
	const int rs = ngm::run_stride(q, c);
	if (m->p_rec.reserve((size_t) na * 8 + 8)) { ngm::pipeline_set_error("out of pinned host memory"); return -12; }
	int32_t *h_rec = m->p_rec.p;
	uint16_t *h_runs = nullptr;
	const int align_buf_len = (q + c) | 2;
	static const bool dev_strings = !getenv("NGM_HIP_HOST_CIGAR");
	uint64_t str_base = 0;
	GpuStage stage_align(m, 1, false);
	if (na > 0) {
		if (m->d_a_read.reserve(na) || m->d_a_loc.reserve(na) || m->d_a_sv.reserve(na) || m->d_records.reserve((size_t) na * 8) ||
				m->d_runs.reserve((size_t) na * rs)) { ngm::pipeline_set_error("out of device memory (align stage)"); return -12; }
		if (int rc = ngm::engine_reserve(eng, na)) { ngm::pipeline_set_error("%s", ngm_hip_last_error(eng)); return rc; }
		MAP_HIP_TRY(hipMemcpyAsync(m->d_a_read.p, a_read.data(), (size_t) na * 4, hipMemcpyHostToDevice, m->st));
		MAP_HIP_TRY(hipMemcpyAsync(m->d_a_loc.p, a_loc.data(), (size_t) na * 4, hipMemcpyHostToDevice, m->st));
		MAP_HIP_TRY(hipMemcpyAsync(m->d_a_sv.p, a_sv.data(), (size_t) na * 4, hipMemcpyHostToDevice, m->st));
		MAP_HIP_TRY(hipStreamSynchronize(m->st));
		stage_align.acquire();
		MAP_HIP_TRY(hipEventRecord(m->ev[5], m->st));
		ngm::WindowGeom Ga{r->n_bases - 1, align_buf_len, c >> 1};
		hipLaunchKernelGGL(ngm::gather_pairs_kernel, dim3((na + ngm::kSlots - 1) / ngm::kSlots), dim3(256), 0, m->st, m->d_reads.p, m->d_read_len.p, q,
				r->d_genome, Ga, m->d_a_read.p, m->d_a_loc.p, m->d_a_sv.p, na, eng->RW, eng->FW, eng->packed.p, eng->lens.p, eng->blk_rows.p, alt_dir);
		MAP_HIP_TRY(hipGetLastError());
		MAP_HIP_TRY(hipEventRecord(m->ev[6], m->st));
		const bool was_prof = eng->profiling;
		const bool affine = m->prm.personality == NGM_PERSONALITY_AFFINE;
		static const bool tail_split = getenv("NGM_HIP_ALIGN_TAIL_SPLIT") != nullptr;
		const bool finish = affine && dev_strings && topn == 1 && !tail_split;
		const unsigned long long scap = (unsigned long long) na * 96ull + 4096ull;
		unsigned long long n_runs_total = 0, n_str_total = 0;
		if (dev_strings && (m->d_cigout.reserve(na) || m->d_str.reserve(scap) || m->p_cigout.reserve(na))) { ngm::pipeline_set_error("out of memory (CIGAR strings)"); return -12; }
		if (finish) {
			unsigned long long ctr[2] = {0, 0};
			MAP_HIP_TRY(hipMemsetAsync(m->d_total.p + 8, 0, 16, m->st));
			const ngm::AlignFinish fin{m->d_cigout.p, m->d_str.p, scap, m->d_total.p + 8};
			eng->profiling = true;
			if (int rc = ngm::engine_align_packed(eng, mode, na, m->d_records.p, m->d_runs.p, rs, m->st, &fin)) { eng->profiling = was_prof; ngm::pipeline_set_error("%s", ngm_hip_last_error(eng)); return rc; }
			eng->profiling = was_prof;
			MAP_HIP_TRY(hipEventRecord(m->ev[7], m->st));
			MAP_HIP_TRY(hipEventRecord(m->ev[8], m->st));
			MAP_HIP_TRY(hipMemcpyAsync(m->p_cigout.p, m->d_cigout.p, (size_t) na * sizeof(ngm::CigarDevOut), hipMemcpyDeviceToHost, m->st));
			MAP_HIP_TRY(hipMemcpyAsync(ctr, m->d_total.p + 8, 16, hipMemcpyDeviceToHost, m->st));
			stage_align.done_after(m->ev[8]);
			MAP_HIP_TRY(hipStreamSynchronize(m->st));
			n_str_total = std::min<unsigned long long>(ctr[0], scap);
			str_base = n_str_total;
			if (m->p_str.reserve(n_str_total + 1)) { ngm::pipeline_set_error("out of pinned host memory"); return -12; }
			if (n_str_total && !sam) MAP_HIP_TRY(hipMemcpy(m->p_str.p, m->d_str.p, n_str_total, hipMemcpyDeviceToHost));
			if (ctr[1]) {
				if (m->d_runs_c.reserve((size_t) na * rs)) { ngm::pipeline_set_error("out of device memory (runs)"); return -12; }
				MAP_HIP_TRY(hipMemsetAsync(m->d_total.p, 0, 8, m->st));
				if (int rc = ngm::engine_affine_traceback_packed(eng, na, m->d_records.p, m->d_runs.p, rs, m->st)) { ngm::pipeline_set_error("%s", ngm_hip_last_error(eng)); return rc; }
				hipLaunchKernelGGL(ngm::compact_runs_kernel, dim3((na + 255) / 256), dim3(256), 0, m->st, na, m->d_records.p, m->d_runs.p, rs,
						m->d_runs_c.p, m->d_total.p);
				MAP_HIP_TRY(hipGetLastError());
				MAP_HIP_TRY(hipMemcpyAsync(h_rec, m->d_records.p, (size_t) na * 8 * 4, hipMemcpyDeviceToHost, m->st));
				MAP_HIP_TRY(hipMemcpyAsync(&n_runs_total, m->d_total.p, 8, hipMemcpyDeviceToHost, m->st));
				MAP_HIP_TRY(hipStreamSynchronize(m->st));
				if (m->p_runs.reserve(n_runs_total + 1)) { ngm::pipeline_set_error("out of pinned host memory"); return -12; }
				h_runs = m->p_runs.p;
				MAP_HIP_TRY(hipMemcpy(h_runs, m->d_runs_c.p, n_runs_total * 2, hipMemcpyDeviceToHost));
			}
		} else {
		eng->profiling = true;
		if (int rc = ngm::engine_align_packed(eng, mode, na, m->d_records.p, m->d_runs.p, rs, m->st)) { eng->profiling = was_prof; ngm::pipeline_set_error("%s", ngm_hip_last_error(eng)); return rc; }
		eng->profiling = was_prof;
		MAP_HIP_TRY(hipEventRecord(m->ev[7], m->st));
		if (m->d_runs_c.reserve((size_t) na * rs)) { ngm::pipeline_set_error("out of device memory (runs)"); return -12; }
		MAP_HIP_TRY(hipMemsetAsync(m->d_total.p, 0, 8, m->st));
		hipLaunchKernelGGL(ngm::compact_runs_kernel, dim3((na + 255) / 256), dim3(256), 0, m->st, na, m->d_records.p, m->d_runs.p, rs,
				m->d_runs_c.p, m->d_total.p);
		MAP_HIP_TRY(hipGetLastError());
		if (!dev_strings) { MAP_HIP_TRY(hipEventRecord(m->ev[8], m->st)); }
		if (dev_strings) {
			MAP_HIP_TRY(hipMemsetAsync(m->d_total.p + 8, 0, 8, m->st));
			if (affine) hipLaunchKernelGGL(ngm::cigar_strings_kernel<true>, dim3((na + 255) / 256), dim3(256), 0, m->st, na, m->d_records.p, m->d_runs_c.p, eng->packed.p, eng->RW, eng->FW,
					m->d_read_len.p, m->d_a_read.p, m->prm.variant == NGM_VARIANT_OCL_CPU ? 1 : 0, m->prm.hard_clip, m->prm.silent_clip, m->d_cigout.p, m->d_str.p, scap,
					(unsigned long long *) (m->d_total.p + 8), 0);
			else hipLaunchKernelGGL(ngm::cigar_strings_kernel<false>, dim3((na + 255) / 256), dim3(256), 0, m->st, na, m->d_records.p, m->d_runs_c.p, eng->packed.p, eng->RW, eng->FW,
					m->d_read_len.p, m->d_a_read.p, m->prm.variant == NGM_VARIANT_OCL_CPU ? 1 : 0, m->prm.hard_clip, m->prm.silent_clip, m->d_cigout.p, m->d_str.p, scap,
					(unsigned long long *) (m->d_total.p + 8), alt_cigar);
			MAP_HIP_TRY(hipGetLastError());
			MAP_HIP_TRY(hipEventRecord(m->ev[8], m->st));
			MAP_HIP_TRY(hipMemcpyAsync(m->p_cigout.p, m->d_cigout.p, (size_t) na * sizeof(ngm::CigarDevOut), hipMemcpyDeviceToHost, m->st));
			MAP_HIP_TRY(hipMemcpyAsync(&n_str_total, m->d_total.p + 8, 8, hipMemcpyDeviceToHost, m->st));
		}
		MAP_HIP_TRY(hipMemcpyAsync(h_rec, m->d_records.p, (size_t) na * 8 * 4, hipMemcpyDeviceToHost, m->st));
		MAP_HIP_TRY(hipMemcpyAsync(&n_runs_total, m->d_total.p, 8, hipMemcpyDeviceToHost, m->st));
		stage_align.done_after(m->ev[8]);
		MAP_HIP_TRY(hipStreamSynchronize(m->st));
		if (m->p_runs.reserve(n_runs_total + 1)) { ngm::pipeline_set_error("out of pinned host memory"); return -12; }
		h_runs = m->p_runs.p;
		MAP_HIP_TRY(hipMemcpy(h_runs, m->d_runs_c.p, n_runs_total * 2, hipMemcpyDeviceToHost));
		if (dev_strings) {
			n_str_total = std::min<unsigned long long>(n_str_total, scap);
			str_base = n_str_total;
			if (m->p_str.reserve(n_str_total + 1)) { ngm::pipeline_set_error("out of pinned host memory"); return -12; }
			if (n_str_total && !sam) MAP_HIP_TRY(hipMemcpy(m->p_str.p, m->d_str.p, n_str_total, hipMemcpyDeviceToHost));
		}
		}
	}
	stage_align.done();

	lap(3);
	ngm::SamRef *sam_refs = sam ? m->p_sam_refs.p : nullptr;
	std::mutex extra_mu;
	std::vector<char> extra;
	parallel_for(n, [&](int lo, int hi) {
		for (int i = lo; i < hi; ++i) for (int t = 0; t < topn; ++t) {
			const size_t o = (size_t) i * topn + t;
			ngm_hit &h = hits[o];
			memset(&h, 0, sizeof(h));
			h.n_candidates = (int) m->h_count[i];
			h.max_votes = m->h_maxv[i];
			h.mapq = h_mapq[i];
			h.n_best = h_nbest[i];
			h.score = h_best[i];
			h.pair_flags = pair_flags[i];
			if (!sam) { cigars[o * str_stride] = 0; mds[o * str_stride] = 0; }
			else sam_refs[o] = ngm::SamRef{0, 0, 0, 0};
		}
	});
	ngm::CigarParams cp{m->prm.match_bonus, -m->prm.mismatch_penalty, m->prm.variant, m->prm.hard_clip, m->prm.silent_clip, alt_cigar};
	parallel_for(na, [&](int lo, int hi) {
		std::vector<char> win((size_t) q + c + 8), qry((size_t) q + 8), scr(sam ? 2 * str_stride : 0);
		for (int j = lo; j < hi; ++j) {
			const int i = (int) a_read[j];
			const size_t o = a_out[j];
			ngm_hit &h = hits[o];
			if (topn > 1) h.score = h_scores[a_pair[j]];
			const bool rev = a_sv[j] & 1u;
			h.reverse = rev;
			const char *rd = reads + (size_t) i * q;
			int L_cached = -1;
			auto read_length = [&]() { if (L_cached < 0) L_cached = (int) strnlen(rd, q); return L_cached; };
			ngm_hip_align_out ao{};
			ao.cigar = sam ? scr.data() : cigars + o * str_stride;
			ao.md = sam ? scr.data() + str_stride : mds + o * str_stride;
			bool host_strings = true;
			const ngm::CigarDevOut *dv = dev_strings ? &m->p_cigout.p[j] : nullptr;
			if (dv && (dv->flags & 1)) {
				if (!(dv->flags & 2)) { h.mapped = 0; continue; }
				if (sam) { sam_refs[o] = ngm::SamRef{dv->cig_off, dv->md_off, dv->cig_len, dv->md_len}; host_strings = false; }
				else {
					memcpy(ao.cigar, m->p_str.p + dv->cig_off, dv->cig_len); ao.cigar[dv->cig_len] = 0;
					memcpy(ao.md, m->p_str.p + dv->md_off, dv->md_len); ao.md[dv->md_len] = 0;
				}
				ao.identity = dv->identity; ao.nm = dv->nm; ao.qstart = dv->qstart; ao.qend = dv->qend; ao.position_offset = dv->position_offset;
				ao.score_token = dv->score_token;
			} else if (m->prm.personality == NGM_PERSONALITY_AFFINE) {
				ngm::build_cigar_affine(&h_rec[(size_t) j * 8], &h_runs[(size_t) (uint32_t) h_rec[(size_t) j * 8 + 6]], nullptr, nullptr, q, &ao, read_length());
				memcpy(ao.md, "!!!", 4);
			} else {
				const uint64_t offset = (uint64_t) a_loc[j] - (uint64_t) (c >> 1);
				host_window(r, offset, align_buf_len, q + c, win.data());
				memset(qry.data(), 0, qry.size());
				const int L = read_length();
				if (!rev) memcpy(qry.data(), rd, L);
				else for (int t = 0; t < L; ++t) {
					const char ch = rd[L - 1 - t];
					qry[t] = ch == 'A' ? 'T' : ch == 'T' ? 'A' : ch == 'C' ? 'G' : ch == 'G' ? 'C' : ch;
				}
				const bool second = paired && (i & 1);
				ngm::build_cigar_md(cp, &h_rec[(size_t) j * 8], &h_runs[(size_t) (uint32_t) h_rec[(size_t) j * 8 + 6]], win.data(), qry.data(), &ao, cp.alt ? ((rev ? !second : second) ? 1 : 0) : 0);
				if (ao.score_token < 0) { h.mapped = 0; continue; }
			}
			if (sam && host_strings) {
				const size_t cl = strlen(ao.cigar), ml = strlen(ao.md);
				std::lock_guard<std::mutex> lk(extra_mu);
				const size_t at = extra.size();
				extra.insert(extra.end(), ao.cigar, ao.cigar + cl);
				extra.insert(extra.end(), ao.md, ao.md + ml);
				sam_refs[o] = ngm::SamRef{(uint32_t) (str_base + at), (uint32_t) (str_base + at + cl), (uint16_t) cl, (uint16_t) ml};
			}
			h.identity = ao.identity; h.nm = ao.nm; h.qstart = ao.qstart; h.qend = ao.qend;
			const uint64_t final_loc = (uint64_t) a_loc[j] + (uint64_t) (int64_t) ao.position_offset - (uint64_t) (c >> 1);
			int contig = 0; uint64_t cpos = 0;
			if (!ngm_ref_convert(r, final_loc, &contig, &cpos)) { h.mapped = 0; continue; }
			h.mapped = 1; h.contig = contig; h.pos = cpos;
		}
	});

	lap(4);
	if (sam) {
		GpuStage stage_sam(m, 1, false, 2);
		const int units = paired ? n / 2 : n;
		if (!extra.empty()) {
			const size_t need = (size_t) str_base + extra.size();
			if (need > m->d_str.cap) {
				ngm::DevBuf<char> bigger;
				if (bigger.reserve(need + 4096)) { ngm::pipeline_set_error("out of device memory (SAM strings)"); return -12; }
				if (str_base) MAP_HIP_TRY(hipMemcpyAsync(bigger.p, m->d_str.p, (size_t) str_base, hipMemcpyDeviceToDevice, m->st));
				MAP_HIP_TRY(hipStreamSynchronize(m->st));
				std::swap(bigger, m->d_str);
				bigger.release();
			}
			if (m->p_sam_extra.reserve(extra.size())) { ngm::pipeline_set_error("out of pinned host memory"); return -12; }
			memcpy(m->p_sam_extra.p, extra.data(), extra.size());
			MAP_HIP_TRY(hipMemcpyAsync(m->d_str.p + str_base, m->p_sam_extra.p, extra.size(), hipMemcpyHostToDevice, m->st));
		}
		if (m->d_sam_len.reserve((size_t) units + 1) || m->d_sam_off.reserve((size_t) units + 1)) { ngm::pipeline_set_error("out of device memory (SAM stage)"); return -12; }
		MAP_HIP_TRY(hipMemcpyAsync(m->d_sam_hits.p, hits, (size_t) n * sizeof(ngm_hit), hipMemcpyHostToDevice, m->st));
		MAP_HIP_TRY(hipMemcpyAsync(m->d_sam_refs.p, sam_refs, (size_t) n * sizeof(ngm::SamRef), hipMemcpyHostToDevice, m->st));
		MAP_HIP_TRY(hipMemsetAsync(m->d_total.p + 16, 0, 64, m->st));
		MAP_HIP_TRY(hipStreamSynchronize(m->st));
		stage_sam.acquire();
		ngm::SamArgs S{};
		S.n = n; S.q = q; S.paired = paired ? 1 : 0;
		S.unit_len_bound = (uint32_t) ((paired ? 2 : 1) * (2 * q + 1024));
		S.reads = m->d_reads.p; S.quals = m->d_sam_quals.p; S.names = m->d_sam_names.p; S.meta = m->d_sam_meta.p; S.hits = m->d_sam_hits.p; S.refs = m->d_sam_refs.p;
		S.str = m->d_str.p; S.contig_names = m->d_sam_contig_names.p; S.contig_name_off = m->d_sam_contig_off.p;
		S.min_insert = m->sam_opt.min_insert_size; S.max_insert = m->sam_opt.max_insert_size > 0 ? m->sam_opt.max_insert_size : 2147483647;
		S.min_mq = m->sam_opt.min_mq; S.no_unal = m->sam_opt.no_unal; S.hard_clip = m->prm.hard_clip; S.silent_clip = m->prm.silent_clip;
		S.min_identity = m->sam_opt.min_identity; S.min_residues = m->sam_opt.min_residues;
		S.rg = m->sam_rg.empty() ? nullptr : m->d_sam_rg.p; S.rg_len = (int) m->sam_rg.size(); S.bs_mapping = m->sam_opt.bs_mapping;
		S.slam_seq = m->sam_opt.slam_seq; S.variant_cpu = m->prm.variant == NGM_VARIANT_OCL_CPU ? 1 : 0; S.alt_scoring = (m->prm.bs_mapping || (m->prm.slam_seq & 2)) ? 1 : 0;
		S.genome = r->d_genome; S.contig_start = m->d_sam_contig_start.p;
		S.unit_len = m->d_sam_len.p; S.unit_off = m->d_sam_off.p; S.counters = m->d_total.p + 16;
		S.bam = m->sam_opt.bam ? 1 : 0;
		S.polya = sam->polya ? m->d_sam_polya.p : nullptr;
		hipEvent_t e0 = m->cev[0], e1 = m->cev[1];
		MAP_HIP_TRY(hipEventRecord(e0, m->st));
		unsigned long long total = 0;
		if (units > 0) {
			const bool bam_slam = S.bam && S.slam_seq;
			if (bam_slam) hipLaunchKernelGGL(ngm::sam_lengths_kernel<true>, dim3((units + 255) / 256), dim3(256), 0, m->st, S, units);
			else hipLaunchKernelGGL(ngm::sam_lengths_kernel<false>, dim3((units + 255) / 256), dim3(256), 0, m->st, S, units);
			MAP_HIP_TRY(hipGetLastError());
			size_t tmp_bytes = 0;
			(void) rocprim::exclusive_scan(nullptr, tmp_bytes, m->d_sam_len.p, m->d_sam_off.p, 0u, (size_t) units + 1, rocprim::plus<uint32_t>(), m->st);
			if (m->d_scan_tmp.reserve(tmp_bytes + 16)) { ngm::pipeline_set_error("out of device memory (scan)"); return -12; }
			MAP_HIP_TRY(hipMemsetAsync(m->d_sam_len.p + units, 0, 4, m->st));
			MAP_HIP_TRY(rocprim::exclusive_scan(m->d_scan_tmp.p, tmp_bytes, m->d_sam_len.p, m->d_sam_off.p, 0u, (size_t) units + 1, rocprim::plus<uint32_t>(), m->st));
			uint32_t total32 = 0;
			unsigned long long total64 = 0;
			MAP_HIP_TRY(hipMemcpyAsync(&total32, m->d_sam_off.p + units, 4, hipMemcpyDeviceToHost, m->st));
			MAP_HIP_TRY(hipMemcpyAsync(&total64, m->d_total.p + 19, 8, hipMemcpyDeviceToHost, m->st));
			MAP_HIP_TRY(hipStreamSynchronize(m->st));
			if (total64 != (unsigned long long) total32) {
				ngm::pipeline_set_error("ngm_mapper_map_sam: the text of this batch of %d reads is %llu bytes, beyond the 32-bit offsets of a batch: use smaller batches", n, total64);
				return -75;
			}
			total = total32;
			if (m->d_sam_text.reserve((size_t) total + 16)) { ngm::pipeline_set_error("out of device memory (SAM text)"); return -12; }
			S.out = m->d_sam_text.p;
			stage_sam.acquire();
			if (bam_slam) hipLaunchKernelGGL(ngm::sam_write_kernel<true>, dim3((units + 255) / 256), dim3(256), 0, m->st, S, units);
			else hipLaunchKernelGGL(ngm::sam_write_kernel<false>, dim3((units + 255) / 256), dim3(256), 0, m->st, S, units);
			MAP_HIP_TRY(hipGetLastError());
		}
		MAP_HIP_TRY(hipEventRecord(e1, m->st));
		unsigned long long ctr[7] = {0, 0, 0, 0, 0, 0, 0};
		MAP_HIP_TRY(hipMemcpyAsync(ctr, m->d_total.p + 16, 56, hipMemcpyDeviceToHost, m->st));
		m->sam_text_bytes = total;
		const bool bam = m->sam_opt.bam != 0;
		if (!bam && total <= sam->out_cap && total > 0) MAP_HIP_TRY(hipMemcpyAsync(sam->out, m->d_sam_text.p, (size_t) total, hipMemcpyDeviceToHost, m->st));
		stage_sam.done_after(e1);
		MAP_HIP_TRY(hipStreamSynchronize(m->st));
		sam->text_bytes = (long long) total;
		float bgzf_ms = 0.f;
		if (bam && total > 0) {
			if (m->sorter) {
				int rc;
				if (ngm::bam_sort_device(m->sorter) == r->device) rc = ngm::bam_sort_add_device(m->sorter, m->batch_seq, m->d_sam_text.p, (size_t) total, m->d_sam_off.p, (size_t) units);
				else {
					m->sorter_host.resize((size_t) total);
					MAP_HIP_TRY(hipMemcpy(m->sorter_host.data(), m->d_sam_text.p, (size_t) total, hipMemcpyDeviceToHost));
					rc = ngm_bam_sort_add(m->sorter, m->batch_seq, m->sorter_host.data(), (size_t) total);
				}
				if (rc < 0) return rc == -12 ? -28 : rc;
				sam->text_bytes = 0;
				m->sam_text_bytes = 0;
			} else if (sam->out_cap < ngm_bgzf_bound((size_t) total)) sam->text_bytes = (long long) ngm_bgzf_bound((size_t) total);
			else {
				const long long zlen = ngm_bgzf_compress_device(m->bz, m->d_sam_text.p, (size_t) total, sam->out, sam->out_cap);
				if (zlen < 0) return (int) zlen;
				sam->text_bytes = zlen;
				m->sam_text_bytes = 0;
				bgzf_ms = ngm_bgzf_last_kernel_ms(m->bz);
			}
		}
		if (sam->stats) { sam->stats[0] = ctr[0]; sam->stats[1] = ctr[1]; sam->stats[2] = ctr[2]; }
		m->pair_stats[0] = ctr[4]; m->pair_stats[1] = ctr[5]; m->pair_stats[2] = ctr[6];
		float t = 0;
		sam->kernel_ms = (hipEventElapsedTime(&t, e0, e1) == hipSuccess ? t : 0.f) + bgzf_ms;
		lap(5);
	}
	if (host_timing)
		fprintf(stderr, "[ngm-hip] host wall ms: candidate search %.1f | score stage + downloads %.1f | pair selection %.1f | align stage + downloads %.1f | CIGAR/positions %.1f\n",
				t_stage[0], t_stage[1], t_stage[2], t_stage[3], t_stage[4]);
	auto et = [&](int a, int b) { float t = 0; if (hipEventElapsedTime(&t, m->ev[a], m->ev[b]) != hipSuccess) t = 0; return t; };
	m->ms[0] = m->cs_kernel_ms;
	m->ms[7] = et(0, 1);
	if (np > 0) { m->ms[1] = et(1, 2); m->ms[2] = et(2, 3); m->ms[3] = et(3, 4); }
	if (na > 0) {
		m->ms[4] = et(5, 6);
		float t = 0;
		if (hipEventElapsedTime(&t, m->ev[6], eng->ev[2]) == hipSuccess) m->ms[5] = t;
		if (hipEventElapsedTime(&t, eng->ev[2], m->ev[7]) == hipSuccess) m->ms[6] = t;
	}
	return n;
}

ngm_pair_state *ngm_pair_state_create(void) { return new ngm_pair_state(); }
void ngm_pair_state_destroy(ngm_pair_state *ps) { delete ps; }
int ngm_mapper_set_pair_state(ngm_mapper *m, ngm_pair_state *ps) { if (!m) return -22; m->ps = ps; return 0; }
int ngm_mapper_set_batch_seq(ngm_mapper *m, uint64_t seq) { if (!m) return -22; m->batch_seq = seq; return 0; }
int ngm_mapper_set_fast_pairing(ngm_mapper *m, int on) { if (!m) return -22; m->fast_pairing = on ? 1 : 0; return 0; }
int ngm_mapper_set_bam_sorter(ngm_mapper *m, ngm_bam_sort *s) { if (!m) return -22; m->sorter = s; return 0; }

void *ngm_host_alloc(size_t bytes) {
	void *p = nullptr;
	if (hipHostMalloc(&p, bytes ? bytes : 1, hipHostMallocDefault) != hipSuccess) { ngm::pipeline_set_error("out of pinned host memory (%zu bytes)", bytes); return nullptr; }
	return p;
}
void ngm_host_free(void *p) { if (p) (void) hipHostFree(p); }

int ngm_host_pin_to_device_node(int device) {
	char bdf[64] = {0};
	if (hipDeviceGetPCIBusId(bdf, (int) sizeof(bdf), device) != hipSuccess) { ngm::pipeline_set_error("no PCI bus id for device %d", device); return -19; }
	for (char *c = bdf; *c; ++c) *c = (char) tolower((unsigned char) *c);
	char path[256], line[4096] = {0};
	snprintf(path, sizeof(path), "/sys/bus/pci/devices/%s/numa_node", bdf);
	int node = -1;
	if (FILE *f = fopen(path, "r")) { if (fscanf(f, "%d", &node) != 1) node = -1; fclose(f); }
	if (node < 0) return 0;
	snprintf(path, sizeof(path), "/sys/devices/system/node/node%d/cpulist", node);
	FILE *f = fopen(path, "r");
	if (!f) return 0;
	const bool got = fgets(line, sizeof(line), f) != nullptr;
	fclose(f);
	if (!got) return 0;
	cpu_set_t set;
	CPU_ZERO(&set);
	int n = 0;
	for (const char *c = line; *c;) {
		char *end = nullptr;
		const long a = strtol(c, &end, 10);
		if (end == c) break;
		long b = a;
		c = end;
		if (*c == '-') { b = strtol(c + 1, &end, 10); if (end == c + 1) break; c = end; }
		for (long x = a; x <= b && x < CPU_SETSIZE; ++x) if (x >= 0) { CPU_SET((int) x, &set); ++n; }
		if (*c == ',') ++c; else break;
	}
	if (n == 0) return 0;
	if (sched_setaffinity(0, sizeof(set), &set) != 0) return 0;
	return n;
}

int ngm_mapper_cs_max_combined(ngm_mapper *m, float *out) {
	if (!m) return -22;
	DevGuard g(m->ref->device);
	if (m->n_reads > 0) MAP_HIP_TRY(hipMemcpy(out, m->d_max_both.p, (size_t) m->n_reads * 4, hipMemcpyDeviceToHost));
	return 0;
}

int ngm_mapper_set_reference_cs_batch(ngm_mapper *m, int reads) {
	if (!m || reads < 0) return -22;
	m->ref_cs_batch = reads & ~1;
	return 0;
}

int ngm_mapper_set_reference_score_buffer(ngm_mapper *m, int entries) {
	if (!m || entries < 0) return -22;
	m->ref_score_buffer = entries;
	return 0;
}

int ngm_mapper_lost_pairs(ngm_mapper *m, uint64_t *out) {
	if (!m || !out) return -22;
	*out = m->lost_pairs;
	return 0;
}

int ngm_mapper_path_counters(ngm_mapper *m, uint64_t out[8]) {
	if (!m || !out) return -22;
	out[0] = m->st_reads; out[1] = m->st_cands; out[2] = m->st_exact_lds; out[3] = m->st_exact_global;
	out[4] = m->st_order_reads; out[5] = m->st_order_big; out[6] = m->st_order_unknown; out[7] = m->st_heavy;
	return 0;
}

int ngm_debug_pair_walk(uint32_t cnt_a, int len_a, uint32_t cnt_b, int len_b, const uint32_t *loc, const uint32_t *sv, const float *score, const uint32_t *rank,
// ... 3 lines not shown
	ngm_mapper_params prm{};
	prm.pair_score_cutoff = cutoff; prm.min_insert_size = min_insert; prm.max_insert_size = max_insert;
	sort_like_reference(out_a, 0, cnt_a, loc, sv, score, rank);
	sort_like_reference(out_b, cnt_a, cnt_b, loc, sv, score, rank);
	uint64_t n = 0;
	walk_pair(prm, 0, cnt_a, len_a, cnt_a, cnt_b, len_b, loc, sv, score, rank, mq_a, mq_b, [&](float ps, int cur, int ia, int ib) {
		if (n < cap && combo_score && combo_dist && combo_a && combo_b) { combo_score[n] = ps; combo_dist[n] = cur; combo_a[n] = ia; combo_b[n] = ib; }
		++n;
	});
	*n_combo = n;
	return 0;
}

int ngm_debug_pair_eval(uint64_t n, const float *pair_score, const int *dist, const int *ia, const int *ib, int avg, int out_all[6], int out_kept[6]) {
	if ((n && (!pair_score || !dist || !ia || !ib)) || !out_all || !out_kept) { ngm::pipeline_set_error("ngm_debug_pair_eval: bad arguments"); return -1; }
	PairSeq all, kept;
	PairSeqKeeper keep{kept};
	for (uint64_t x = 0; x < n; ++x) {
		all.ps.push_back(pair_score[x]); all.d.push_back(dist[x]); all.a.push_back(ia[x]); all.b.push_back(ib[x]);
		keep(pair_score[x], dist[x], ia[x], ib[x]);
	}
	auto put = [](const PairSeq &q, int avg_, int *o) {
		const PairOutcome r = eval_pair_seq(q, avg_);
		o[0] = r.found ? 1 : 0; o[1] = r.wa; o[2] = r.wb; o[3] = r.equal; o[4] = r.dist; o[5] = (int) q.ps.size();
	};
	put(all, avg, out_all); put(kept, avg, out_kept);
	return 0;
}

int ngm_debug_select_top1(int device, int n_reads, const uint32_t *base, const uint32_t *count, uint64_t n_cand, const float *scores, const uint32_t *loc,
		const uint32_t *strand_votes, uint32_t *winner, int32_t *mapq, int32_t *n_best, float *best_score) {
	if (n_reads <= 0 || !base || !count || !winner || !mapq || !n_best || !best_score) return -22;
	DevGuard g(device);
	ngm::DevBuf<uint32_t> d_base, d_count, d_loc, d_sv, d_win;
	ngm::DevBuf<int32_t> d_mq, d_nb;
	ngm::DevBuf<float> d_sc, d_best;
	const size_t nc = (size_t) std::max<uint64_t>(n_cand, 1);
	if (d_base.reserve(n_reads) || d_count.reserve(n_reads) || d_loc.reserve(nc) || d_sv.reserve(nc) || d_sc.reserve(nc) || d_win.reserve(n_reads) || d_mq.reserve(n_reads) ||
			d_nb.reserve(n_reads) || d_best.reserve(n_reads)) { ngm::pipeline_set_error("out of device memory (ngm_debug_select_top1)"); return -12; }
	MAP_HIP_TRY(hipMemcpy(d_base.p, base, (size_t) n_reads * 4, hipMemcpyHostToDevice));
	MAP_HIP_TRY(hipMemcpy(d_count.p, count, (size_t) n_reads * 4, hipMemcpyHostToDevice));
	if (n_cand) {
		MAP_HIP_TRY(hipMemcpy(d_sc.p, scores, (size_t) n_cand * 4, hipMemcpyHostToDevice));
		MAP_HIP_TRY(hipMemcpy(d_loc.p, loc, (size_t) n_cand * 4, hipMemcpyHostToDevice));
		MAP_HIP_TRY(hipMemcpy(d_sv.p, strand_votes, (size_t) n_cand * 4, hipMemcpyHostToDevice));
	}
	hipLaunchKernelGGL(ngm::select_top1_kernel, dim3((n_reads + 255) / 256), dim3(256), 0, 0, n_reads, d_base.p, d_count.p, d_sc.p, d_loc.p, d_sv.p, d_win.p, d_mq.p, d_nb.p, d_best.p);
	MAP_HIP_TRY(hipGetLastError());
	MAP_HIP_TRY(hipDeviceSynchronize());
	MAP_HIP_TRY(hipMemcpy(winner, d_win.p, (size_t) n_reads * 4, hipMemcpyDeviceToHost));
	MAP_HIP_TRY(hipMemcpy(mapq, d_mq.p, (size_t) n_reads * 4, hipMemcpyDeviceToHost));
	MAP_HIP_TRY(hipMemcpy(n_best, d_nb.p, (size_t) n_reads * 4, hipMemcpyDeviceToHost));
	MAP_HIP_TRY(hipMemcpy(best_score, d_best.p, (size_t) n_reads * 4, hipMemcpyDeviceToHost));
	d_base.release(); d_count.release(); d_loc.release(); d_sv.release(); d_win.release(); d_mq.release(); d_nb.release(); d_sc.release(); d_best.release();
	return 0;
}

int ngm_debug_expand_pairs(int device, int n_reads, const uint32_t *base, const uint32_t *count, uint64_t n_cand, uint32_t *out) {
	if (n_reads <= 0 || !base || !count || (n_cand && !out)) return -22;
	DevGuard g(device);
	ngm::DevBuf<uint32_t> d_base, d_count, d_out;
	auto run = [&]() -> int {
		if (d_base.reserve(n_reads) || d_count.reserve(n_reads) || d_out.reserve((size_t) std::max<uint64_t>(n_cand, 1))) { ngm::pipeline_set_error("out of device memory (ngm_debug_expand_pairs)"); return -12; }
		MAP_HIP_TRY(hipMemcpy(d_base.p, base, (size_t) n_reads * 4, hipMemcpyHostToDevice));
		MAP_HIP_TRY(hipMemcpy(d_count.p, count, (size_t) n_reads * 4, hipMemcpyHostToDevice));
		MAP_HIP_TRY(hipMemset(d_out.p, 0xFF, (size_t) std::max<uint64_t>(n_cand, 1) * 4));
		hipLaunchKernelGGL(ngm::expand_pairs_kernel, dim3((n_reads + 255) / 256), dim3(256), 0, 0, n_reads, d_base.p, d_count.p, d_out.p);
		MAP_HIP_TRY(hipGetLastError());
		MAP_HIP_TRY(hipDeviceSynchronize());
		if (n_cand) MAP_HIP_TRY(hipMemcpy(out, d_out.p, (size_t) n_cand * 4, hipMemcpyDeviceToHost));
		return 0;
	};
	const int rc = run();
	d_base.release(); d_count.release(); d_out.release();
	return rc;
}

int ngm_mapper_heavy_counters(ngm_mapper *m, uint64_t out[4]) {
	if (!m || !out) return -22;
	out[0] = m->st_heavy_second; out[1] = m->st_heavy_restart; out[2] = m->st_heavy_sent_on; out[3] = m->st_pool_regrown;
	return 0;
}

int ngm_mapper_order_table_reads(ngm_mapper *m, uint64_t *out) {
	if (!m || !out) return -22;
	*out = m->st_order_table;
	return 0;
}

int ngm_mapper_cs_counters(ngm_mapper *m, uint64_t out[3]) {
	if (!m) return -22;
	out[0] = m->cs_kmers; out[1] = m->cs_hits; out[2] = m->n_cand;
	return 0;
}

float ngm_mapper_last_order_replay_ms(ngm_mapper *m) { return m ? m->order_ms : 0.f; }

int ngm_mapper_last_pair_stats(ngm_mapper *m, uint64_t out[3]) {
	if (!m || !out) return -22;
	out[0] = m->pair_stats[0]; out[1] = m->pair_stats[1]; out[2] = m->pair_stats[2];
	return 0;
}

int ngm_mapper_last_kernel_ms(ngm_mapper *m, float ms[8]) {
	if (!m) return -22;
	for (int i = 0; i < 8; ++i) ms[i] = m->ms[i];
	return 0;
}

}
```

nextgenmap_amd/csrc/mapper_internal.h:

```cpp
#pragma once

#include <algorithm>
#include <atomic>
#include <chrono>
#include <climits>
#include <cmath>
#include <cstdlib>
#include <cstdio>
#include <cstring>
#include <condition_variable>
#include <mutex>
#include <numeric>
#include <thread>
#include <vector>

#include <string.h>
#include <ctype.h>
#include <sched.h>
#include "../../include/ngm_pipeline.h"
#include "refindex.h"
#include "engine_internal.h"
#include "cigar_md.h"
#include "cigar_device.h"
#include "cs_device.h"
// ... 10 lines not shown
		}                                                                                      \
	} while (0)

struct ngm_pair_state {
	std::mutex mu;
	std::condition_variable cv;
	uint64_t next = 0;
	long dist_count = 1, dist_sum = 0;
	uint64_t scores_so_far = 0;
	uint64_t reads_so_far = 0;
};

struct ngm_mapper {
	const ngm_ref *ref = nullptr;
	ngm_pair_state *ps = nullptr;
	uint64_t batch_seq = 0;
	int fast_pairing = 0;
	ngm_mapper_params prm{};
	ngm_hip_ctx *eng = nullptr;
	hipStream_t st = nullptr;
	int max_kfreq = 0;
	int cs_log2_slots = 14;
	int cs_log2_small = 10;
	uint32_t cs_plane_bits = 65536;
	uint32_t cs_plane_bits0 = 65536;
	int cs_log2_bits = 16;
	uint32_t cs_queued_exact = 0;
	int cs_fast_items = ngm::kCsFastItemsShort;
	size_t cs_region_cap = 0;
	double cs_hexp = 4096;
	int cs_waves = 3;
	bool cs_paired = false;
	int cs_canon = 0;
	long pair_dist_count = 1, pair_dist_sum = 0;
	uint64_t scores_so_far = 0, reads_so_far = 0;
	int ref_cs_batch = 0;
	int ref_score_buffer = 0;
	uint64_t lost_pairs = 0;
	uint64_t st_heavy_second = 0, st_heavy_restart = 0, st_heavy_sent_on = 0, st_pool_regrown = 0;
	int cus = 256;
	int heavy_per_cu[3] = {0, 0, 0};
	size_t heavy_lds[3] = {0, 0, 0};
	uint64_t st_heavy = 0, st_reads = 0, st_cands = 0, st_exact_lds = 0, st_exact_global = 0, st_order_reads = 0, st_order_big = 0, st_order_unknown = 0, st_order_table = 0;
	ngm::CsArgs last_cs{};
	hipStream_t st_hi = nullptr;
	ngm::DevBuf<uint32_t> d_order_list, d_cand_rank, d_order_scratch, d_order_info, d_order_big, d_order_gt, d_order_log2;
	ngm::DevBuf<uint64_t> d_order_off;
	ngm::CsArgs order_args{};
	ngm::PinnedBuf<uint32_t> p_rank, p_order_info;
	std::vector<uint32_t> order_pending;
	ngm::PinnedBuf<uint32_t> p_winner, p_loc, p_sv;
	ngm::PinnedBuf<int32_t> p_mapq, p_nbest, p_rec;
	ngm::PinnedBuf<float> p_best, p_scores;
	ngm::PinnedBuf<uint16_t> p_runs;
	ngm::DevBuf<uint8_t> d_reads;
	ngm::DevBuf<uint16_t> d_read_len;
	ngm::DevBuf<uint32_t> d_cand_base, d_cand_count, d_out_loc, d_out_sv, d_status, d_ovf_read, d_ovf_read2, d_ovf_hits, d_ovf_hits2, d_ovf_log2;
	ngm::PinnedBuf<uint32_t> p_cs_status;
	ngm::DevBuf<uint64_t> d_ovf_off;
	ngm::DevBuf<uint32_t> d_gt_keys, d_gt_votes, d_heavy_list, d_heavy_ctr;
	ngm::DevBuf<float> d_max_votes, d_max_both, d_scores, d_best;
	ngm::DevBuf<unsigned long long> d_total, d_counters, d_heavy_diag;
	ngm::DevBuf<uint32_t> d_out_loc2, d_out_sv2, d_new_base;
	ngm::DevBuf<uint8_t> d_scan_tmp;
	unsigned long long cs_kmers = 0, cs_hits = 0;
	float cs_kernel_ms = 0.f;
	hipEvent_t cev[6] = {};
	hipEvent_t oev[4] = {};
	float order_ms = 0.f;
	ngm::DevBuf<uint32_t> d_pair_read, d_winner, d_a_read, d_a_loc, d_a_sv;
	ngm::DevBuf<int32_t> d_mapq, d_nbest, d_records, d_pair_info;
	ngm::PinnedBuf<int32_t> p_pair_info;
	ngm::DevBuf<ngm::PairOut> d_pair_out;
	ngm::DevBuf<ngm::PairTop> d_pair_top;
	ngm::DevBuf<uint32_t> d_pair_tied_n, d_pair_list;
	ngm::PinnedBuf<ngm::PairOut> p_pair_out;
	ngm::PinnedBuf<ngm::PairTop> p_pair_top;
	ngm::PinnedBuf<uint32_t> p_pair_tied_n;
	ngm::DevBuf<uint16_t> d_runs, d_runs_c;
	ngm::DevBuf<char> d_str;
	ngm::DevBuf<ngm::CigarDevOut> d_cigout;
	ngm::PinnedBuf<ngm::CigarDevOut> p_cigout;
	ngm::PinnedBuf<char> p_str;
	ngm_sam_options sam_opt{};
	ngm_bgzf *bz = nullptr;
	ngm_bam_sort *sorter = nullptr;
	std::vector<char> sorter_host;
	bool sam_ready = false;
	std::string sam_rg;
	ngm::DevBuf<char> d_sam_contig_names, d_sam_rg, d_sam_names, d_sam_text;
	ngm::DevBuf<uint32_t> d_sam_contig_off, d_sam_len, d_sam_off;
	ngm::DevBuf<uint64_t> d_sam_contig_start;
	ngm::DevBuf<uint8_t> d_sam_quals;
	ngm::DevBuf<uint16_t> d_sam_polya;
	ngm::DevBuf<ngm::SamMeta> d_sam_meta;
	ngm::DevBuf<ngm::SamRef> d_sam_refs;
	ngm::DevBuf<ngm_hit> d_sam_hits;
	ngm::PinnedBuf<ngm_hit> p_sam_hits;
	ngm::PinnedBuf<ngm::SamRef> p_sam_refs;
	ngm::PinnedBuf<char> p_sam_extra;
	uint64_t sam_text_bytes = 0;
	bool argos_on = false;
	bool argos_text = false;
	float argos_min = 0.f;
	int argos_n_starts = 0;
	ngm::DevBuf<uint64_t> d_argos_starts, d_argos_loff, d_argos_gkeys;
	ngm::DevBuf<uint32_t> d_argos_ord, d_argos_nsurv, d_argos_npos, d_argos_list, d_argos_llist, d_argos_gvals, d_argos_hord, d_argos_hoff;
	ngm::DevBuf<uint8_t> d_argos_cls;
	ngm::DevBuf<unsigned long long> d_argos_ctr;
	ngm::PinnedBuf<uint8_t> p_argos_cls;
	ngm::PinnedBuf<uint32_t> p_argos_nsurv;
	uint64_t argos_ctr[4] = {0, 0, 0, 0};
	uint64_t argos_long = 0, argos_unknown = 0;
	hipEvent_t aev[4] = {};
	uint64_t pair_stats[3] = {0, 0, 0};
	int n_reads = 0;
	template <typename T> struct HostArr {
		ngm::PinnedBuf<T> b;
		T &operator[](size_t i) { return b.p[i]; }
		const T &operator[](size_t i) const { return b.p[i]; }
		T *data() { return b.p; }
	};
	HostArr<uint32_t> h_base, h_count;
	HostArr<float> h_maxv;
	uint64_t n_cand = 0;
	hipEvent_t ev[10] = {};
	float ms[8] = {};
};

namespace ngm {

struct DevGuard {
	int prev = -1;
	explicit DevGuard(int d) { if (hipGetDevice(&prev) != hipSuccess) prev = -1; if (prev != d) (void) hipSetDevice(d); else prev = -1; }
	~DevGuard() { if (prev >= 0) (void) hipSetDevice(prev); }
};

struct StageLock { std::mutex mu; };
extern StageLock g_stage_lock[16][2];
extern std::atomic<long long> g_stage_hold_us[3], g_stage_wait_us[3];
struct GpuStage {
	ngm_mapper *m;
	int kind, slot;
	bool held = false;
	StageLock *ch = nullptr;
	std::chrono::steady_clock::time_point t_acq;
	static int mode() { static const int v = getenv("NGM_HIP_GPU_STAGE_LOCK") ? atoi(getenv("NGM_HIP_GPU_STAGE_LOCK")) : 1; return v; }
	GpuStage(ngm_mapper *m_, int kind_ = 0, bool now = true, int slot_ = -1) : m(m_), kind(kind_), slot(slot_ < 0 ? kind_ : slot_) {
		ch = &g_stage_lock[(unsigned) m->ref->device & 15u][mode() == 2 ? kind : 0];
		if (now) acquire();
	}
	~GpuStage() { release(); }
	void acquire() {
		if (mode() == 0 || held) return;
		const auto t0 = std::chrono::steady_clock::now();
		ch->mu.lock();
		held = true;
		t_acq = std::chrono::steady_clock::now();
		g_stage_wait_us[slot] += std::chrono::duration_cast<std::chrono::microseconds>(t_acq - t0).count();
	}
	void release() {
		if (!held) return;
		g_stage_hold_us[slot] += std::chrono::duration_cast<std::chrono::microseconds>(std::chrono::steady_clock::now() - t_acq).count();
		held = false;
		ch->mu.unlock();
	}
	void done_after(hipEvent_t ev) { if (held) (void) hipEventSynchronize(ev); release(); }
	void done() { release(); }
};

int cs_configure(ngm_mapper *m, const ngm_mapper_params *p);
int run_cs(ngm_mapper *m, int n, GpuStage *stage = nullptr);
int cs_host_arrays(ngm_mapper *m);
int candidate_order(ngm_mapper *m, const std::vector<uint32_t> &list, uint64_t np, uint32_t **h_rank, bool wait = true);
int candidate_order_wait(ngm_mapper *m, uint32_t **h_rank);
void cs_release(ngm_mapper *m);
long test_limit(const char *key, long dflt);

int score_candidates(ngm_mapper *m, int n, uint64_t np, int alt_dir);
void argos_release(ngm_mapper *m);

}
```

nextgenmap_amd/csrc/ngm_cli.cpp:

```cpp
#include <dlfcn.h>
#include <fcntl.h>
#include <signal.h>
#include <sys/resource.h>
#include <sys/time.h>
#include <ucontext.h>
#include <malloc.h>
#include <getopt.h>
#include <sys/mman.h>
#include <poll.h>
#include <signal.h>
#include <sys/stat.h>
#include <sys/sendfile.h>
#include <sys/wait.h>
#include <zlib.h>

#include <algorithm>
#include <array>
#include <atomic>
#include <chrono>
#include <cmath>
#include <condition_variable>
#include <deque>
#include <map>
#include <memory>
// ... 1998 lines not shown
		if (stats_comm) {
			const auto t_ar = std::chrono::steady_clock::now();
			int64_t all[8];
			memcpy(all, sv, sizeof(all));
			if (ngm_stats_allreduce(stats_comm, all) == 0) {
				if (o.shard_i == 0) {
					snprintf(msg, sizeof(msg), "Statistics all-reduce over %d GPUs (RCCL, %.0f us): %lld reads, %lld mapped, %lld not mapped, %lld lines written; %lld pairs with both mates mapped, %lld of them broken, mean insert size %.1f",
							o.shard_n, std::chrono::duration<double, std::micro>(std::chrono::steady_clock::now() - t_ar).count(), (long long) all[0], (long long) all[1], (long long) all[2], (long long) all[3],
							(long long) all[4], (long long) all[5], all[7] > 0 ? (double) all[6] / (double) all[7] : 0.0);
					info("MAIN", msg);
				}
			} else info("MAIN", std::string("warning: statistics all-reduce failed: ") + ngm_pipeline_last_error());
			ngm_stats_comm_destroy(stats_comm);
		} else if (!stats_comm_error.empty() && o.shard_i == 0) info("MAIN", "note: no RCCL communicator for the statistics (" + stats_comm_error + "); the parent process sums them");
	}
	snprintf(msg, sizeof(msg), "Mapping pass: %.3f s, %.0f reads/s (%zu GPU(s) x %d worker(s), %d host threads, %s input)", secs, n_total / std::max(1e-9, secs),
			o.devices.size(), o.workers, pool.size(), plain ? (mf0.owned ? "gzip FASTQ inflated to memory" : "memory-mapped plain FASTQ") : "serial reader");
	info("MAIN", msg);
	snprintf(msg, sizeof(msg), "GPU kernels: %.3f s of the %.3f s mapping pass (%.0f %%; candidate search, gathers, score, select, align, traceback by HIP events)",
			t_gpu_us / 1e6, secs, 100.0 * (t_gpu_us / 1e6) / std::max(1e-9, secs));
	info("MAIN", msg);
	if (!gpu_sam) {
		snprintf(msg, sizeof(msg), "Records%s formatted on the host pool: %.3f s of thread time = %.0f %% of %d threads x %.3f s", (o.bam && !gpu_bgzf) ? " + BGZF blocks" : "", t_format_cpu_us / 1e6,
				100.0 * (t_format_cpu_us / 1e6) / std::max(1e-9, pool.size() * secs), pool.size(), secs);
		info("MAIN", msg);
	}
	if (gpu_bgzf) {
		snprintf(msg, sizeof(msg), "BGZF blocks written by the GPU: %.1f MB of records -> %.1f MB, %.3f s of kernels, %.3f s inside the calls (copies to and from page-locked memory, both transfers, the kernels)",
				bgzf_in_bytes.load() / 1e6, bgzf_out_bytes.load() / 1e6, t_bgzf_gpu_us / 1e6, t_bgzf_call_us / 1e6);
		info("MAIN", msg);
	}
	if (gpu_sam) { snprintf(msg, sizeof(msg), "%s on the GPU: %.3f s of kernels (included above)", o.bam ? "BAM records and their BGZF blocks written" : "SAM text assembled", t_sam_gpu_us / 1e6); info("MAIN", msg); }
	snprintf(msg, sizeof(msg), "Input to output: %.3f s (estimation pass + mapping pass, first input byte to output closed)",
			std::chrono::duration<double>(std::chrono::steady_clock::now() - t_input).count());
	info("MAIN", msg);
	if (getenv("NGM_HIP_HOST_TIMING")) {
		auto span = [](std::chrono::steady_clock::time_point a, std::chrono::steady_clock::time_point b) { return std::chrono::duration<double>(b - a).count(); };
		snprintf(msg, sizeof(msg), "Before the mapping pass, s: input mapped + record index + read lengths %.3f | sensitivity estimate %.3f | header, mappers, page-locked buffers %.3f",
				span(t_input, t_indexed), span(t_indexed, t_estimated), span(t_estimated, t_start));
		info("MAIN", msg);
		snprintf(msg, sizeof(msg), "Worker time summed over %zu workers, s: waiting for input %.3f | parse + pack %.3f | map (GPU + library host stages) %.3f | format %.3f",
				workers.size(), t_wait_us / 1e6, t_parse_us / 1e6, t_map_us / 1e6, t_format_us / 1e6);
		info("MAIN", msg);
		{
			struct timespec cpu1;
			clock_gettime(CLOCK_PROCESS_CPUTIME_ID, &cpu1);
			struct rusage ru1;
			getrusage(RUSAGE_SELF, &ru1);
			auto tv = [](const timeval &a, const timeval &b) { return (double) (b.tv_sec - a.tv_sec) + 1e-6 * (double) (b.tv_usec - a.tv_usec); };
			snprintf(msg, sizeof(msg), "Mapping pass, process totals: CPU %.2f s (user %.2f, system %.2f), page faults %ld minor / %ld major, context switches %ld voluntary / %ld involuntary",
					(double) (cpu1.tv_sec - cpu0.tv_sec) + 1e-9 * (double) (cpu1.tv_nsec - cpu0.tv_nsec), tv(ru0.ru_utime, ru1.ru_utime), tv(ru0.ru_stime, ru1.ru_stime),
					ru1.ru_minflt - ru0.ru_minflt, ru1.ru_majflt - ru0.ru_majflt, ru1.ru_nvcsw - ru0.ru_nvcsw, ru1.ru_nivcsw - ru0.ru_nivcsw);
			info("MAIN", msg);
		}
		snprintf(msg, sizeof(msg), "Pool thread time inside the stages, s: parse + pack %.3f | format %.3f | output copies %.3f (writer wall %.3f)",
				t_parse_cpu_us / 1e6, t_format_cpu_us / 1e6, t_write_cpu_us / 1e6, t_write_us / 1e6);
		info("MAIN", msg);
	}
	if (o.argos) {
		uint64_t ac[4] = {0, 0, 0, 0}, ap[2] = {0, 0};
		for (Worker &w : workers) {
			uint64_t c4[4], c2[2];
			if (ngm_mapper_argos_counters(w.m, c4) == 0) for (int x = 0; x < 4; ++x) ac[x] += c4[x];
			if (ngm_mapper_argos_path_counters(w.m, c2) == 0) for (int x = 0; x < 2; ++x) ap[x] += c2[x];
		}
		const double nl = (double) std::max<uint64_t>(1, ac[0] + ac[1] + ac[2]);
		snprintf(msg, sizeof(msg), "Argos order classes: U %llu (%.3f %%), S %llu (%.3f %%), H %llu (%.3f %%); %llu entries written; long-list path %llu reads; order by position (candidate order unknown) %llu reads",
				(unsigned long long) ac[0], 100.0 * ac[0] / nl, (unsigned long long) ac[1], 100.0 * ac[1] / nl, (unsigned long long) ac[2], 100.0 * ac[2] / nl,
				(unsigned long long) ac[3], (unsigned long long) ap[0], (unsigned long long) ap[1]);
		info("MAIN", msg);
	}
	{
		uint64_t pc[8] = {0, 0, 0, 0, 0, 0, 0, 0};
		for (Worker &w : workers) { uint64_t c8[8]; if (ngm_mapper_path_counters(w.m, c8) == 0) for (int x = 0; x < 8; ++x) pc[x] += c8[x]; }
		const double nr = (double) std::max<uint64_t>(1, pc[0]);
		snprintf(msg, sizeof(msg), "Candidate search: %llu reads, %.2f candidates per read; heavy-read kernel for %llu reads (%.3f %%), exact search with the table in LDS for %llu (%.3f %%), in global memory for %llu (%.3f %%)",
				(unsigned long long) pc[0], pc[1] / nr, (unsigned long long) pc[7], 100.0 * pc[7] / nr, (unsigned long long) pc[2], 100.0 * pc[2] / nr, (unsigned long long) pc[3], 100.0 * pc[3] / nr);
		info("MAIN", msg);
		uint64_t hc[4] = {0, 0, 0, 0};
		for (Worker &w : workers) { uint64_t c4[4]; if (ngm_mapper_heavy_counters(w.m, c4) == 0) for (int x = 0; x < 4; ++x) hc[x] += c4[x]; }
		snprintf(msg, sizeof(msg), "Heavy-read kernel: %llu second passes, %llu table passes started over, %llu reads sent on to the exact kernels; table pool regrown %llu times",
				(unsigned long long) hc[0], (unsigned long long) hc[1], (unsigned long long) hc[2], (unsigned long long) hc[3]);
		info("MAIN", msg);
		uint64_t by_table = 0;
		for (Worker &w : workers) { uint64_t c2 = 0; if (ngm_mapper_order_table_reads(w.m, &c2) == 0) by_table += c2; }
		snprintf(msg, sizeof(msg), "Candidate order replay: %llu reads, %llu of them beyond the LDS replay (exact replay through buckets in global memory, %llu of them with a table there); order left undetermined for %llu reads",
				(unsigned long long) pc[4], (unsigned long long) pc[5], (unsigned long long) by_table, (unsigned long long) pc[6]);
		info("MAIN", msg);
	}
	if (o.paired && o.ref_score_buffer > 0) {
		uint64_t lost = 0;
		for (Worker &w : workers) { uint64_t c2 = 0; if (ngm_mapper_lost_pairs(w.m, &c2) == 0) lost += c2; }
		snprintf(msg, sizeof(msg), "Pairs lost as NextGenMap loses them (first mate's last score fills the %d-entry score buffer, second mate without candidates; src/ScoreBuffer.cpp:196, :519-523): %llu",
				o.ref_score_buffer, (unsigned long long) lost);
		info("MAIN", msg);
	}
	if (const char *pf = getenv("NGM_HIP_PROFILE")) prof::dump(pf);
	for (Worker &w : workers) { ngm_mapper_destroy(w.m); ngm_host_free(w.rows); ngm_host_free(w.qrows); ngm_host_free(w.names); ngm_host_free(w.meta); ngm_host_free(w.polya);
		ngm_bgzf_destroy(w.bz); ngm_host_free(w.bam_raw); ngm_host_free(w.bam_out); }
	ngm_bam_sort_destroy(sorter);
	for (TextBuf &t : text_free) ngm_host_free(t.p);
	ngm_pair_state_destroy(pair_state);
	for (ngm_ref *r2 : refs) ngm_ref_destroy(r2);
	return 0;
}
```

nextgenmap_amd/csrc/ngm_hip.cpp:

```cpp
#include "../../include/ngm_hip.h"
#include "../../include/ngm_pipeline.h"

#include <hip/hip_runtime.h>

#include <algorithm>

#include <cstdarg>
#include <cstdio>
#include <cstdlib>
#include <cstring>
#include <mutex>
#include <string>
#include <vector>

#define NGM_ENGINE_KERNELS
#include "engine_internal.h"
#include "align_device.h"
#include "affine_device.h"
#include "cigar_md.h"
#include "jit.h"

namespace {

thread_local std::string g_last_error;
// ... 79 lines not shown
}
const void *find_pk_align_kernel(int c, bool window) {
#define X(C) if (c == C) return pk_align_ptr<C>(window);
	NGM_CORRIDORS(X)
#undef X
	return nullptr;
}

KernelRef find_kernel(ngm_hip_ctx *ctx, int kind) {
	KernelRef k;
	k.aot = find_aot_kernel(ctx->c, kind);
	if (!k.aot && ctx->jit) k.jit = ctx->jit->fn[kind];
	return k;
}

template <typename... Args>
hipError_t launch_kernel(const KernelRef &k, dim3 grid, dim3 block, hipStream_t st, Args... args) {
	void *argv[] = {(void *) &args...};
	if (k.aot) return hipLaunchKernel(k.aot, grid, block, argv, 0, st);
	return hipModuleLaunchKernel(k.jit, grid.x, grid.y, grid.z, block.x, block.y, block.z, 0, st, argv, nullptr);
}

int n_blocks_of(int n) { return (n + ngm::kSlots - 1) / ngm::kSlots; }

}
namespace ngm {
int engine_reserve(ngm_hip_ctx *ctx, int n) {
	const size_t nb = (size_t) n_blocks_of(n);
	if (ctx->packed.reserve(nb * (size_t) (ctx->RW + ctx->FW) * ngm::kSlots) || ctx->lens.reserve(nb * ngm::kSlots) ||
			ctx->blk_rows.reserve(nb)) {
		set_error(ctx, "out of device memory reserving the packed workspace for %d pairs", n);
		return -12;
	}
	return 0;
}

int engine_score_packed(ngm_hip_ctx *ctx, int mode, int n, float *d_scores, hipStream_t st) {
	const int nb = n_blocks_of(n);
	static const bool force32 = getenv("NGM_HIP_SCORE_32BIT") != nullptr;
	if (ctx->prm.personality == NGM_PERSONALITY_AFFINE) {
		const bool ef = (mode & NGM_MODE_ALIGN_MASK) == NGM_MODE_END_TO_END;
		if (!force32 && (long) ctx->q * ctx->KA.tM < 30000 && ctx->prm.gap_read_penalty + (long) ctx->q * (ctx->prm.gap_extend_penalty + ctx->KA.tZ) < 19000) {
			if (const void *sp = ef ? nullptr : find_pk_affine_score_split_kernel(ctx->c)) {
				KernelRef kp; kp.aot = sp;
				const int units = 2 * ((nb + 1) / 2);
				HIP_TRY(ctx, launch_kernel(kp, dim3((units + 3) / 4), dim3(256), st, (const uint32_t *) ctx->packed.p, (const uint16_t *) ctx->lens.p,
						(const uint16_t *) ctx->blk_rows.p, d_scores, n, nb, ctx->RW, ctx->KA));
				return 0;
			}
			if (const void *pk = find_pk_affine_score_kernel(ctx->c, ef)) {
				KernelRef kp; kp.aot = pk;
				HIP_TRY(ctx, launch_kernel(kp, dim3((nb + 7) / 8), dim3(256), st, (const uint32_t *) ctx->packed.p, (const uint16_t *) ctx->lens.p,
						(const uint16_t *) ctx->blk_rows.p, d_scores, n, nb, ctx->RW, ctx->KA));
				return 0;
			}
		}
		const KernelRef ka = find_kernel(ctx, 4 + ((mode & NGM_MODE_ALIGN_MASK) == NGM_MODE_END_TO_END ? 1 : 0));
		HIP_TRY(ctx, launch_kernel(ka, dim3((nb + 3) / 4), dim3(256), st, (const uint32_t *) ctx->packed.p, (const uint16_t *) ctx->lens.p,
				(const uint16_t *) ctx->blk_rows.p, d_scores, (uint32_t *) nullptr, (int32_t *) nullptr, n, nb, ctx->RW, ctx->q, ctx->KA));
		return 0;
	}
	const bool endfree = (mode & NGM_MODE_ALIGN_MASK) == NGM_MODE_END_TO_END;
	if (!force32 && (long) ctx->q * std::max(ctx->K.tM, ctx->K.alt ? std::max(ctx->K.tMA, ctx->K.tXA) : 0) < 30000 && (long) ctx->q * ctx->K.tZ < 14000) {
		if (const void *pk = find_pk_score_kernel(ctx->c, endfree)) {
			KernelRef kp; kp.aot = pk;
			HIP_TRY(ctx, launch_kernel(kp, dim3((nb + 7) / 8), dim3(256), st, (const uint32_t *) ctx->packed.p, (const uint16_t *) ctx->lens.p,
					(const uint16_t *) ctx->blk_rows.p, d_scores, n, nb, ctx->RW, ctx->K));
			return 0;
		}
	}
	const KernelRef k = find_kernel(ctx, endfree ? 1 : 0);
	HIP_TRY(ctx, launch_kernel(k, dim3((nb + 3) / 4), dim3(256), st, (const uint32_t *) ctx->packed.p, (const uint16_t *) ctx->lens.p,
			(const uint16_t *) ctx->blk_rows.p, d_scores, n, nb, ctx->RW, ctx->K));
	return 0;
}

int engine_affine_traceback_packed(ngm_hip_ctx *ctx, int n, int32_t *d_records, uint16_t *d_runs, int run_stride, hipStream_t st) {
	hipLaunchKernelGGL(ngm::affine_traceback_kernel, dim3((n + 255) / 256), dim3(256), 0, st, ctx->dirs.p, d_records, d_runs, n,
			ctx->q, ctx->c + 1, run_stride, (const uint32_t *) ctx->packed.p, ctx->RW, ctx->FW, ctx->trace_nibbles ? 1 : 0);
	HIP_TRY(ctx, hipGetLastError());
	return 0;
}

int engine_align_packed(ngm_hip_ctx *ctx, int mode, int n, int32_t *d_records, uint16_t *d_runs, int run_stride, hipStream_t st, const AlignFinish *fin) {
	const int am = mode & NGM_MODE_ALIGN_MASK;
	const int nb = n_blocks_of(n);
	if (ctx->prm.personality == NGM_PERSONALITY_AFFINE) {
		const int CP = ctx->c + 1, ADW = ngm::aff_dir_words(CP);
		if (ctx->dirs.reserve((size_t) nb * ctx->q * ADW * ngm::kSlots)) { set_error(ctx, "out of device memory for the trace matrix"); return -12; }
		static const bool force32 = getenv("NGM_HIP_ALIGN_32BIT") != nullptr;
		const void *pk = nullptr;
		if (!force32 && am != NGM_MODE_END_TO_END && ctx->KA.open < 0 && ctx->KA.ext < 0 && (long) ctx->q * ctx->KA.tM < 30000 &&
				ctx->prm.gap_read_penalty + (long) ctx->q * (ctx->prm.gap_extend_penalty + ctx->KA.tZ) < 19000) {
			const bool plain_key = (long) ctx->q * ctx->prm.match_bonus < 2048 && ctx->c + 1 <= 32;
			if (plain_key) pk = find_pk_affine_align_kernel(ctx->c, false);
			else if (ctx->KA.tZ > 0 && ctx->KA.tM > 0 && ctx->KA.tM + 1 <= 63) pk = find_pk_affine_align_kernel(ctx->c, true);
		}
		if (pk) {
			KernelRef kp; kp.aot = pk;
			HIP_TRY(ctx, launch_kernel(kp, dim3((nb + 7) / 8), dim3(256), st, (const uint32_t *) ctx->packed.p, (const uint16_t *) ctx->lens.p,
					(const uint16_t *) ctx->blk_rows.p, ctx->dirs.p, d_records, n, nb, ctx->RW, ctx->q, ctx->KA));
		} else {
			const KernelRef ka = find_kernel(ctx, 6 + (am == NGM_MODE_END_TO_END ? 1 : 0));
			HIP_TRY(ctx, launch_kernel(ka, dim3((nb + 3) / 4), dim3(256), st, (const uint32_t *) ctx->packed.p, (const uint16_t *) ctx->lens.p,
					(const uint16_t *) ctx->blk_rows.p, (float *) nullptr, ctx->dirs.p, d_records, n, nb, ctx->RW, ctx->q, ctx->KA));
		}
		if (ctx->profiling) HIP_TRY(ctx, hipEventRecord(ctx->ev[2], st));
		ctx->trace_nibbles = pk != nullptr;
		if (!fin) return engine_affine_traceback_packed(ctx, n, d_records, d_runs, run_stride, st);
		if (pk) hipLaunchKernelGGL(ngm::affine_finish_kernel<true>, dim3((n + 255) / 256), dim3(256), 0, st, n, (const uint32_t *) ctx->dirs.p, (const int32_t *) d_records,
				(const uint32_t *) ctx->packed.p, (const uint16_t *) ctx->lens.p, ctx->q, CP, ctx->RW, ctx->FW, fin->out, fin->bytes, fin->capacity, fin->counters);
		else hipLaunchKernelGGL(ngm::affine_finish_kernel<false>, dim3((n + 255) / 256), dim3(256), 0, st, n, (const uint32_t *) ctx->dirs.p, (const int32_t *) d_records,
				(const uint32_t *) ctx->packed.p, (const uint16_t *) ctx->lens.p, ctx->q, CP, ctx->RW, ctx->FW, fin->out, fin->bytes, fin->capacity, fin->counters);
		HIP_TRY(ctx, hipGetLastError());
		return 0;
	}
	if (fin) { set_error(ctx, "the finishing kernel serves the affine personality only"); return -22; }
	const int DW = ngm::dir_words(ctx->c);
	if (ctx->dirs.reserve((size_t) nb * ctx->q * DW * ngm::kSlots)) { set_error(ctx, "out of device memory for the direction matrix"); return -12; }
	static const bool force32 = getenv("NGM_HIP_ALIGN_32BIT") != nullptr;
	const void *pk = nullptr;
	const int max_gain = std::max(ctx->K.tM, ctx->K.alt ? std::max(ctx->K.tMA, ctx->K.tXA) : 0);
	if (!force32 && am != NGM_MODE_END_TO_END && (long) ctx->q * max_gain < 30000 && (long) ctx->q * ctx->K.tZ < 14000 && ctx->K.gl < 0 && ctx->K.gap_read < 0) {
		const bool plain_key = (long) ctx->q * (max_gain - ctx->K.tZ) < 2048 && ctx->c <= 32;
		if (plain_key) pk = find_pk_align_kernel(ctx->c, false);
		else if (ctx->K.tZ > 0 && max_gain + 1 <= 63) pk = find_pk_align_kernel(ctx->c, true);
	}
	if (pk) {
		KernelRef kp; kp.aot = pk;
		HIP_TRY(ctx, launch_kernel(kp, dim3((nb + 7) / 8), dim3(256), st, (const uint32_t *) ctx->packed.p, (const uint16_t *) ctx->lens.p,
				(const uint16_t *) ctx->blk_rows.p, ctx->dirs.p, d_records, n, nb, ctx->RW, ctx->q, ctx->K));
	} else {
		const KernelRef k = find_kernel(ctx, 2 + (am == NGM_MODE_END_TO_END ? 1 : 0));
		HIP_TRY(ctx, launch_kernel(k, dim3((nb + 3) / 4), dim3(256), st, (const uint32_t *) ctx->packed.p, (const uint16_t *) ctx->lens.p,
				(const uint16_t *) ctx->blk_rows.p, ctx->dirs.p, d_records, n, nb, ctx->RW, ctx->q, ctx->K));
	}
	if (ctx->profiling) HIP_TRY(ctx, hipEventRecord(ctx->ev[2], st));
	hipLaunchKernelGGL(ngm::sw_traceback_kernel, dim3((n + 255) / 256), dim3(256), 0, st, ctx->dirs.p, ctx->lens.p, d_records,
			d_runs, n, ctx->q, ctx->c, run_stride, am == NGM_MODE_END_TO_END ? 1 : 0);
	HIP_TRY(ctx, hipGetLastError());
	return 0;
}
}
namespace {
using ngm::engine_reserve;

struct ScopedDevice {
	int prev = -1;
	explicit ScopedDevice(int dev) { if (hipGetDevice(&prev) != hipSuccess) prev = -1; if (prev != dev) (void) hipSetDevice(dev); else prev = -1; }
	~ScopedDevice() { if (prev >= 0) (void) hipSetDevice(prev); }
};

int launch_pack(ngm_hip_ctx *ctx, int n, const void *d_ref, const void *d_qry, hipStream_t st) {
	const int nb = n_blocks_of(n);
	const size_t lds = (size_t) ngm::kSlots * (ctx->rl + ctx->q);
	hipLaunchKernelGGL(ngm::pack_pairs_kernel, dim3(nb), dim3(256), lds, st, (const uint8_t *) d_ref,
			(const uint8_t *) d_qry, n, ctx->q, ctx->rl, ctx->RW, ctx->FW, ctx->packed.p, ctx->lens.p, ctx->blk_rows.p,
			ctx->prm.personality == NGM_PERSONALITY_AFFINE ? 1 : 0, (ctx->K.alt || ctx->prm.alt_cigar) ? ctx->pair_dir : nullptr);
	HIP_TRY(ctx, hipGetLastError());
	return 0;
}

int stage_dirs(ngm_hip_ctx *ctx, int n, const char *dir) {
	ctx->pair_dir = nullptr;
	if ((!ctx->K.alt && !ctx->prm.alt_cigar) || !dir) return 0;
	if (ctx->d_pair_dir.reserve(n)) { set_error(ctx, "out of memory staging %d pairs", n); return -12; }
	HIP_TRY(ctx, hipMemcpyAsync(ctx->d_pair_dir.p, dir, (size_t) n, hipMemcpyHostToDevice, ctx->stream));
	ctx->pair_dir = ctx->d_pair_dir.p;
	return 0;
}

}

extern "C" {

const char *ngm_hip_last_error(const ngm_hip_ctx *ctx) { return ctx ? ctx->error.c_str() : g_last_error.c_str(); }

int ngm_hip_device_count(void) {
	int n = 0;
	if (hipGetDeviceCount(&n) != hipSuccess) return 0;
	return n;
}

ngm_hip_ctx *ngm_hip_create(int device, const ngm_hip_params *p) {
	if (!p || p->abi_version != NGM_HIP_ABI_VERSION) { set_error(nullptr, "ngm_hip_create: bad params / ABI version"); return nullptr; }
	if (p->qry_max_len < 2 || p->qry_max_len > 4096 || p->corridor < 2) { set_error(nullptr, "ngm_hip_create: qry_max_len=%d corridor=%d out of range", p->qry_max_len, p->corridor); return nullptr; }
	if (p->match_bonus <= 0 || p->mismatch_penalty <= 0 || p->gap_read_penalty <= 0 || p->gap_ref_penalty <= 0) {
		set_error(nullptr, "ngm_hip_create: scores must be positive integers (match %d mismatch %d gap_read %d gap_ref %d)", p->match_bonus, p->mismatch_penalty, p->gap_read_penalty, p->gap_ref_penalty);
		return nullptr;
	}
	if (p->personality != NGM_PERSONALITY_LINEAR && p->personality != NGM_PERSONALITY_AFFINE) { set_error(nullptr, "ngm_hip_create: unknown personality %d", p->personality); return nullptr; }
	if (p->personality == NGM_PERSONALITY_AFFINE && p->gap_extend_penalty <= 0) { set_error(nullptr, "ngm_hip_create: gap_extend_penalty must be a positive integer"); return nullptr; }
	if (p->match_bonus + p->mismatch_penalty > 255) { set_error(nullptr, "ngm_hip_create: match_bonus + mismatch_penalty must be <= 255"); return nullptr; }
	if (p->corridor > 200) { set_error(nullptr, "ngm_hip_create: corridor %d too wide (the band row lives in registers)", p->corridor); return nullptr; }
	if (p->alt_cigar != NGM_ALT_NONE && p->alt_cigar != NGM_ALT_BISULFITE && p->alt_cigar != NGM_ALT_SLAMSEQ) { set_error(nullptr, "ngm_hip_create: unknown alt_cigar %d", p->alt_cigar); return nullptr; }
	if (p->alt_cigar != NGM_ALT_NONE && p->personality != NGM_PERSONALITY_LINEAR) { set_error(nullptr, "ngm_hip_create: bisulfite / SLAM-seq and the affine personality can't be used at the same time"); return nullptr; }
// ... 265 lines not shown
```

nextgenmap_amd/pipeline.py:

```python
import ctypes as C

import numpy as np

from .engine import NgmHipError, load_library


class RefParams(C.Structure):
    _fields_ = [("kmer", C.c_int), ("kmer_skip", C.c_int), ("bin_size", C.c_int)]


class MapperParams(C.Structure):
    _fields_ = [("qry_max_len", C.c_int), ("corridor", C.c_int), ("match_bonus", C.c_int), ("mismatch_penalty", C.c_int),
                ("gap_read_penalty", C.c_int), ("gap_ref_penalty", C.c_int), ("mode", C.c_int), ("variant", C.c_int),
                ("sensitivity", C.c_float), ("kmer_min", C.c_float), ("max_cmrs", C.c_int), ("max_kfreq", C.c_int),
                ("hard_clip", C.c_int), ("silent_clip", C.c_int), ("personality", C.c_int), ("gap_extend_penalty", C.c_int),
                ("min_insert_size", C.c_int), ("max_insert_size", C.c_int), ("pair_score_cutoff", C.c_float),
                ("topn", C.c_int), ("strata", C.c_int), ("bs_mapping", C.c_int), ("bs_cutoff", C.c_int), ("bs_read_skip", C.c_int),
                ("match_bonus_tt", C.c_int), ("match_bonus_tc", C.c_int), ("slam_seq", C.c_int)]


class SamOptions(C.Structure):
    _fields_ = [("paired", C.c_int), ("min_insert_size", C.c_int), ("max_insert_size", C.c_int), ("min_mq", C.c_int),
                ("min_identity", C.c_float), ("min_residues", C.c_float), ("no_unal", C.c_int), ("rg_id", C.c_char_p),
                ("bs_mapping", C.c_int), ("slam_seq", C.c_int), ("bam", C.c_int)]


HIT_DTYPE = np.dtype([("mapped", "i4"), ("contig", "i4"), ("pos", "u8"), ("reverse", "i4"), ("mapq", "i4"),
                      ("score", "f4"), ("identity", "f4"), ("nm", "i4"), ("qstart", "i4"), ("qend", "i4"),
                      ("n_candidates", "i4"), ("n_best", "i4"), ("max_votes", "f4"), ("pair_flags", "i4")], align=True)

_bound = False


class BamSortParams(C.Structure):
    _fields_ = [("device", C.c_int), ("chunk_bytes", C.c_size_t), ("max_bytes", C.c_size_t)]


def _lib():
    global _bound
    lib = load_library()
    if not _bound:
        lib.ngm_pipeline_last_error.restype = C.c_char_p
        lib.ngm_ref_create.restype = C.c_void_p
        lib.ngm_ref_create.argtypes = [C.c_int, C.POINTER(RefParams), C.c_int, C.c_void_p, C.c_void_p, C.c_void_p]
        lib.ngm_ref_create_from_fasta.restype = C.c_void_p
        lib.ngm_ref_create_from_fasta.argtypes = [C.c_int, C.POINTER(RefParams), C.c_char_p]
        lib.ngm_ref_create_from_fasta_vcf.restype = C.c_void_p
        lib.ngm_ref_create_from_fasta_vcf.argtypes = [C.c_int, C.POINTER(RefParams), C.c_char_p, C.c_char_p]
        lib.ngm_ref_vcf_summary.argtypes = [C.c_void_p, C.c_void_p]
        lib.ngm_vcf_parse_text.restype = C.c_longlong
        lib.ngm_vcf_parse_text.argtypes = [C.c_int, C.c_void_p, C.c_void_p, C.c_char_p, C.c_void_p, C.c_size_t, C.POINTER(C.c_size_t)]
        lib.ngm_ref_create_from_cache.restype = C.c_void_p
        lib.ngm_ref_create_from_cache.argtypes = [C.c_int, C.POINTER(RefParams), C.c_char_p]
        lib.ngm_ref_destroy.argtypes = [C.c_void_p]
        lib.ngm_ref_contig_count.argtypes = [C.c_void_p]
        lib.ngm_ref_contig_name.restype = C.c_char_p
        lib.ngm_ref_contig_name.argtypes = [C.c_void_p, C.c_int]
        for f in ("ngm_ref_contig_start", "ngm_ref_contig_len"):
            getattr(lib, f).restype = C.c_uint64
            getattr(lib, f).argtypes = [C.c_void_p, C.c_int]
        for f in ("ngm_ref_concat_len", "ngm_ref_index_entries"):
            getattr(lib, f).restype = C.c_uint64
            getattr(lib, f).argtypes = [C.c_void_p]
        lib.ngm_ref_auto_max_kfreq.argtypes = [C.c_void_p]
        lib.ngm_ref_index_copy.argtypes = [C.c_void_p, C.c_void_p, C.c_void_p, C.c_void_p]
        if not hasattr(lib, "ngm_mapper_create"):
            raise NgmHipError("libngm_hip.so was built without the mapping pipeline")
        lib.ngm_ref_write_ngm_cache.argtypes = [C.c_void_p, C.c_char_p]
        lib.ngm_ref_decode.argtypes = [C.c_void_p, C.c_uint64, C.c_int, C.c_void_p]
        lib.ngm_ref_convert.argtypes = [C.c_void_p, C.c_uint64, C.POINTER(C.c_int), C.POINTER(C.c_uint64)]
        lib.ngm_mapper_create.restype = C.c_void_p
        lib.ngm_mapper_create.argtypes = [C.c_void_p, C.POINTER(MapperParams)]
        lib.ngm_mapper_destroy.argtypes = [C.c_void_p]
        lib.ngm_mapper_cs.argtypes = [C.c_void_p, C.c_int, C.c_void_p, C.c_void_p, C.c_void_p]
        lib.ngm_mapper_cs_fetch.argtypes = [C.c_void_p, C.c_void_p, C.c_void_p, C.c_void_p]
        lib.ngm_mapper_map_se.argtypes = [C.c_void_p, C.c_int, C.c_void_p, C.c_void_p, C.c_void_p, C.c_void_p]
        lib.ngm_mapper_map_se_resident.argtypes = [C.c_void_p, C.c_int, C.c_void_p, C.c_void_p, C.c_void_p, C.c_void_p, C.c_void_p]
        lib.ngm_mapper_map_pe_resident.argtypes = [C.c_void_p, C.c_int, C.c_void_p, C.c_void_p, C.c_void_p, C.c_void_p, C.c_void_p]
        lib.ngm_mapper_cs_counters.argtypes = [C.c_void_p, C.c_void_p]
        lib.ngm_mapper_path_counters.argtypes = [C.c_void_p, C.c_void_p]
        lib.ngm_mapper_order_table_reads.argtypes = [C.c_void_p, C.c_void_p]
        lib.ngm_mapper_heavy_counters.argtypes = [C.c_void_p, C.c_void_p]
        lib.ngm_mapper_last_kernel_ms.argtypes = [C.c_void_p, C.POINTER(C.c_float)]
        lib.ngm_mapper_last_order_replay_ms.restype = C.c_float
        lib.ngm_mapper_last_order_replay_ms.argtypes = [C.c_void_p]
        lib.ngm_mapper_set_argos.argtypes = [C.c_void_p, C.c_float]
        lib.ngm_mapper_map_argos.restype = C.c_longlong
        lib.ngm_mapper_map_argos.argtypes = [C.c_void_p, C.c_int, C.c_void_p, C.c_void_p, C.c_size_t, C.c_void_p, C.c_void_p, C.c_size_t,
                                             C.c_void_p, C.POINTER(C.c_float)]
        lib.ngm_mapper_sam_fetch.argtypes = [C.c_void_p, C.c_void_p, C.c_size_t]
        lib.ngm_mapper_set_sam_options.argtypes = [C.c_void_p, C.c_void_p]
        lib.ngm_mapper_map_sam_trimmed.restype = C.c_longlong
        lib.ngm_mapper_map_sam_trimmed.argtypes = [C.c_void_p, C.c_int, C.c_void_p, C.c_void_p, C.c_void_p, C.c_size_t, C.c_void_p, C.c_void_p,
                                                   C.c_void_p, C.c_size_t, C.c_void_p, C.POINTER(C.c_float)]
        lib.ngm_argos_prolog.argtypes = [C.c_void_p, C.c_uint64, C.c_void_p, C.c_size_t]
        lib.ngm_mapper_argos_counters.argtypes = [C.c_void_p, C.c_void_p]
        lib.ngm_mapper_argos_path_counters.argtypes = [C.c_void_p, C.c_void_p]
        lib.ngm_debug_argos_order.argtypes = [C.c_uint32, C.c_void_p, C.c_void_p, C.c_float, C.c_int, C.c_int, C.c_void_p, C.c_void_p]
        lib.ngm_bgzf_create.restype = C.c_void_p
        lib.ngm_bgzf_create.argtypes = [C.c_int]
        lib.ngm_bgzf_destroy.argtypes = [C.c_void_p]
        lib.ngm_bgzf_bound.restype = C.c_size_t
        lib.ngm_bgzf_bound.argtypes = [C.c_size_t]
        lib.ngm_bgzf_compress.restype = C.c_longlong
        lib.ngm_bgzf_compress.argtypes = [C.c_void_p, C.c_void_p, C.c_size_t, C.c_void_p, C.c_size_t]
        lib.ngm_bgzf_inflated_size.restype = C.c_size_t
        lib.ngm_bgzf_inflated_size.argtypes = [C.c_char_p, C.c_size_t]
        lib.ngm_bgzf_inflate.restype = C.c_longlong
        lib.ngm_bgzf_inflate.argtypes = [C.c_void_p, C.c_char_p, C.c_size_t, C.c_void_p, C.c_size_t]
        lib.ngm_bgzf_last_kernel_ms.restype = C.c_float
        lib.ngm_bgzf_last_kernel_ms.argtypes = [C.c_void_p]
        lib.ngm_bam_sort_create.restype = C.c_void_p
        lib.ngm_bam_sort_create.argtypes = [C.POINTER(BamSortParams)]
        lib.ngm_bam_sort_destroy.argtypes = [C.c_void_p]
        lib.ngm_bam_sort_add.argtypes = [C.c_void_p, C.c_uint64, C.c_char_p, C.c_size_t]
        lib.ngm_bam_sort_finish.argtypes = [C.c_void_p, C.c_int]
        lib.ngm_bam_sort_next.restype = C.c_longlong
        lib.ngm_bam_sort_next.argtypes = [C.c_void_p, C.c_void_p, C.c_size_t]
        lib.ngm_bam_sort_index.restype = C.c_longlong
        lib.ngm_bam_sort_index.argtypes = [C.c_void_p, C.c_uint64, C.c_void_p, C.c_size_t]
        lib.ngm_bam_sort_stats.argtypes = [C.c_void_p, C.c_void_p, C.c_void_p]
        lib.ngm_mapper_set_bam_sorter.argtypes = [C.c_void_p, C.c_void_p]
        _bound = True
    return lib


def _err():
    return NgmHipError(_lib().ngm_pipeline_last_error().decode())


class Bgzf:

    def __init__(self, device=0):
        self._h = _lib().ngm_bgzf_create(device)
        if not self._h:
            raise _err()

    def compress(self, data):
        lib = _lib()
        data = bytes(data)
        cap = lib.ngm_bgzf_bound(len(data))
        out = C.create_string_buffer(cap)
        n = lib.ngm_bgzf_compress(self._h, data, len(data), out, cap)
        if n < 0:
            raise _err()
        return out.raw[:n]

    def decompress(self, data):
        lib = _lib()
        data = bytes(data)
        cap = lib.ngm_bgzf_inflated_size(data, len(data))
        if cap == C.c_size_t(-1).value:
            raise RuntimeError("not a run of whole BGZF members")
        out = C.create_string_buffer(max(1, cap))
        n = lib.ngm_bgzf_inflate(self._h, data, len(data), out, cap)
        if n < 0:
            raise _err()
        return out.raw[:n]

    def last_kernel_ms(self):
        return float(_lib().ngm_bgzf_last_kernel_ms(self._h))

    def close(self):
        if self._h:
            _lib().ngm_bgzf_destroy(self._h)
# ... 205 lines not shown
            self.h = None

    def __del__(self):
        try:
            self.close()
        except Exception:
            pass

    @staticmethod
    def reads_to_rows(reads, q):
        out = np.zeros((len(reads), q), np.uint8)
        lut = np.full(256, ord("N"), np.uint8)
        for a, b in zip(b"ACGTacgt", b"ACGTACGT"):
            lut[a] = b
        for i, r in enumerate(reads):
            a = np.frombuffer(bytes(r), dtype=np.uint8)[:q - 1]
            out[i, :a.size] = lut[a]
        return out

    def candidate_search(self, rows):
        rows = np.ascontiguousarray(rows, dtype=np.uint8)
        n = rows.shape[0]
        offs = np.zeros(n + 1, np.uint32)
        mx = np.zeros(n, np.float32)
        if self.lib.ngm_mapper_cs(self.h, n, rows.ctypes.data, offs.ctypes.data, mx.ctypes.data) < 0:
            raise _err()
        tot = int(offs[-1])
        loc = np.zeros(max(1, tot), np.uint64)
        strand = np.zeros(max(1, tot), np.uint8)
        votes = np.zeros(max(1, tot), np.float32)
        if self.lib.ngm_mapper_cs_fetch(self.h, loc.ctypes.data, strand.ctypes.data, votes.ctypes.data) < 0:
            raise _err()
        return offs, mx, loc[:tot], strand[:tot], votes[:tot]

    def map_pe_raw(self, rows, d_rows=None, out=None):
        return self.map_se_raw(rows, d_rows, out, paired=True)

    def map_pe(self, rows):
        rows = np.ascontiguousarray(rows, dtype=np.uint8)
        hits, cig, md = self.map_pe_raw(rows)
        return hits, [bytes(r).split(b"\0", 1)[0] for r in cig], [bytes(r).split(b"\0", 1)[0] for r in md]

    def map_se_raw(self, rows, d_rows=None, out=None, paired=False):
        n = rows.shape[0]
        stride = 4 * max(1, self.q)
        if out is None:
            no = n * (1 if paired else self.topn)
            out = (np.zeros(no, HIT_DTYPE), np.zeros((no, stride), np.uint8), np.zeros((no, stride), np.uint8))
        hits, cig, md = out
        dp = None if d_rows is None else (d_rows.data_ptr() if hasattr(d_rows, "data_ptr") else int(d_rows))
        fn = self.lib.ngm_mapper_map_pe_resident if paired else self.lib.ngm_mapper_map_se_resident
        r = fn(self.h, n, rows.ctypes.data, dp, hits.ctypes.data, cig.ctypes.data, md.ctypes.data)
        if r < 0:
            raise _err()
        return hits, cig, md

    def map_se(self, rows):
        rows = np.ascontiguousarray(rows, dtype=np.uint8)
        hits, cig, md = self.map_se_raw(rows)
        return hits, [bytes(r).split(b"\0", 1)[0] for r in cig], [bytes(r).split(b"\0", 1)[0] for r in md]

    def set_bam_sorter(self, sorter):
        if self.lib.ngm_mapper_set_bam_sorter(self.h, sorter._h if sorter is not None else None) < 0:
            raise _err()

    def last_kernel_ms(self):
        ms = (C.c_float * 8)()
        self.lib.ngm_mapper_last_kernel_ms(self.h, ms)
        return list(ms)

    def last_order_replay_ms(self):
        return float(self.lib.ngm_mapper_last_order_replay_ms(self.h))

    def path_counters(self):
        out = np.zeros(8, np.uint64)
        self.lib.ngm_mapper_path_counters(self.h, out.ctypes.data)
        return dict(zip(("reads", "candidates", "exact_lds", "exact_global", "order_replayed", "order_exact_global", "order_undetermined", "heavy"), (int(x) for x in out[:8])))

    def heavy_counters(self):
        out = np.zeros(4, np.uint64)
        self.lib.ngm_mapper_heavy_counters(self.h, out.ctypes.data)
        return dict(zip(("second_passes", "table_pass_restarts", "sent_on", "pool_regrown"), (int(x) for x in out)))

    def order_table_reads(self):
        out = np.zeros(1, np.uint64)
        self.lib.ngm_mapper_order_table_reads(self.h, out.ctypes.data)
        return int(out[0])

    def map_argos(self, reads, names, min_score=0.0):
        rows = reads if isinstance(reads, np.ndarray) else self.reads_to_rows(reads, self.q)
        rows = np.ascontiguousarray(rows, dtype=np.uint8)
        n = rows.shape[0]
        if len(names) != n:
            raise ValueError("one name per read")
        if self.lib.ngm_mapper_set_argos(self.h, float(min_score)) < 0:
            raise _err()
        nb = [x.encode() if isinstance(x, str) else bytes(x) for x in names]
        meta = np.zeros((n, 2), np.uint32)
        off = 0
        for i, b in enumerate(nb):
            meta[i, 0], meta[i, 1] = off, min(len(b), 0xFFFF)
            off += len(b)
        blob = np.frombuffer(b"".join(nb) + b"\0", np.uint8)
        stats = np.zeros(3, np.uint64)
        kms = C.c_float(0)
        cap = max(1 << 16, n * 64)
        out = np.zeros(cap, np.uint8)
        total = self.lib.ngm_mapper_map_argos(self.h, n, rows.ctypes.data, blob.ctypes.data, off, meta.ctypes.data, out.ctypes.data, cap,
                                              stats.ctypes.data, C.byref(kms))
        if total < 0:
            raise _err()
        if total > cap:
            out = np.zeros(total, np.uint8)
            if self.lib.ngm_mapper_sam_fetch(self.h, out.ctypes.data, total) < 0:
                raise _err()
        return out[:total].tobytes(), [int(x) for x in stats]

    def map_sam(self, reads, quals, names, polya_trimmed=None, paired=False, rg_id=None, slam_seq=0, bam=False, min_insert_size=0,
                max_insert_size=1000, min_mq=0, min_identity=0.65, min_residues=0.5, no_unal=False):
        rows = reads if isinstance(reads, np.ndarray) else self.reads_to_rows(reads, self.q)
        rows = np.ascontiguousarray(rows, dtype=np.uint8)
        n = rows.shape[0]
        if len(names) != n or len(quals) != n or (polya_trimmed is not None and len(polya_trimmed) != n):
            raise ValueError("one name, one quality string and one poly-A count per read")
        so = SamOptions(int(paired), min_insert_size, max_insert_size, min_mq, min_identity, min_residues, int(no_unal),
                        rg_id.encode() if isinstance(rg_id, str) else rg_id, 0, int(slam_seq), int(bam))
        if self.lib.ngm_mapper_set_sam_options(self.h, C.byref(so)) < 0:
            raise _err()
        nb = [x.encode() if isinstance(x, str) else bytes(x) for x in names]
        qrows = np.zeros((n, self.q), np.uint8)
        meta = np.zeros(n, np.dtype([("name_off", np.uint32), ("name_len", np.uint16), ("qual_len", np.uint16)]))
        off = 0
        for i, b in enumerate(nb):
            ql = quals[i].encode() if isinstance(quals[i], str) else bytes(quals[i])
            qrows[i, :min(len(ql), self.q - 1)] = np.frombuffer(ql[:self.q - 1], np.uint8)
            meta[i] = (off, min(len(b), 0xFFFF), min(len(ql), 0x7FFF))
            off += len(b)
        blob = np.frombuffer(b"".join(nb) + b"\0", np.uint8)
        polya = None if polya_trimmed is None else np.ascontiguousarray(polya_trimmed, dtype=np.uint16)
        stats = np.zeros(3, np.uint64)
        kms = C.c_float(0)
        cap = max(1 << 16, n * (2 * self.q + 512))
        out = np.zeros(cap, np.uint8)
        total = self.lib.ngm_mapper_map_sam_trimmed(self.h, n, rows.ctypes.data, qrows.ctypes.data, blob.ctypes.data, off, meta.ctypes.data,
                                                    None if polya is None else polya.ctypes.data, out.ctypes.data, cap, stats.ctypes.data, C.byref(kms))
        if total < 0:
            raise _err()
        if total > cap:
            out = np.zeros(total, np.uint8)
            got = self.lib.ngm_mapper_sam_fetch(self.h, out.ctypes.data, total)
            if got < 0:
                raise _err()
            if bam:
                total = got
        return out[:total].tobytes(), [int(x) for x in stats]

    def argos_counters(self):
        out = np.zeros(4, np.uint64)
        self.lib.ngm_mapper_argos_counters(self.h, out.ctypes.data)
        p = np.zeros(2, np.uint64)
        self.lib.ngm_mapper_argos_path_counters(self.h, p.ctypes.data)
        return dict(zip(("U", "S", "H", "entries", "long_list", "unknown_order"), [int(x) for x in out] + [int(x) for x in p]))

    def cs_counters(self):
        out = np.zeros(3, np.uint64)
        self.lib.ngm_mapper_cs_counters(self.h, out.ctypes.data)
# ... 2 lines not shown
```

Before: 57.14 million.

## Align single-candidate reads once in the score stage, skipping separate score pass

```diff
diff --git a/include/ngm_pipeline.h b/include/ngm_pipeline.h
--- a/include/ngm_pipeline.h
+++ b/include/ngm_pipeline.h
@@ -191,6 +191,8 @@
 
 int ngm_mapper_heavy_counters(ngm_mapper *m, uint64_t out[4]);
 
+int ngm_mapper_align_once_counters(ngm_mapper *m, uint64_t out[5]);
+
 int ngm_mapper_cs_counters(ngm_mapper *m, uint64_t out[3]);
 
 typedef struct ngm_stats_comm ngm_stats_comm;
diff --git a/nextgenmap_amd/csrc/cigar_device.h b/nextgenmap_amd/csrc/cigar_device.h
--- a/nextgenmap_amd/csrc/cigar_device.h
+++ b/nextgenmap_amd/csrc/cigar_device.h
@@ -184,14 +184,13 @@
 template <bool NIBBLES>
 __global__ __launch_bounds__(256) void affine_finish_kernel(int n, const uint32_t *__restrict__ dirs, const int32_t *__restrict__ records,
 		const uint32_t *__restrict__ packed, const uint16_t *__restrict__ lens, int q, int CP, int RW, int FW, CigarDevOut *__restrict__ out,
-		char *__restrict__ bytes, unsigned long long capacity, unsigned long long *__restrict__ counters) {
+		char *__restrict__ bytes, unsigned long long capacity, unsigned long long *__restrict__ counters, int lim = kCigarRow - 16) {
 	__shared__ char s_rows[256 * kCigarRow];
 	__shared__ uint32_t s_wave[4];
 	__shared__ unsigned long long s_base;
 	const int j = blockIdx.x * blockDim.x + threadIdx.x;
 	const bool live = j < n;
 	const int lane = threadIdx.x & 63, wv = threadIdx.x >> 6;
-	constexpr int lim = kCigarRow - 16;
 	constexpr int WS = NIBBLES ? 3 : 2;
 	const int DW = NIBBLES ? aff_nib_words(CP) : aff_dir_words(CP);
 	char *row = s_rows + (size_t) threadIdx.x * kCigarRow;
diff --git a/nextgenmap_amd/csrc/engine_internal.h b/nextgenmap_amd/csrc/engine_internal.h
--- a/nextgenmap_amd/csrc/engine_internal.h
+++ b/nextgenmap_amd/csrc/engine_internal.h
@@ -88,7 +88,10 @@
 	char *bytes;
 	unsigned long long capacity;
 	unsigned long long *counters;
+	hipEvent_t dp_done = nullptr;
+	int row_limit = 0;
 };
+bool engine_affine_align_is_packed(const ngm_hip_ctx *ctx, int mode);
 int engine_align_packed(ngm_hip_ctx *ctx, int mode, int n, int32_t *d_records, uint16_t *d_runs, int run_stride, hipStream_t st, const AlignFinish *fin = nullptr);
 int engine_affine_traceback_packed(ngm_hip_ctx *ctx, int n, int32_t *d_records, uint16_t *d_runs, int run_stride, hipStream_t st);
 }
diff --git a/nextgenmap_amd/csrc/gather_device.h b/nextgenmap_amd/csrc/gather_device.h
--- a/nextgenmap_amd/csrc/gather_device.h
+++ b/nextgenmap_amd/csrc/gather_device.h
@@ -265,6 +265,55 @@
 	}
 }
 
+__host__ __device__ constexpr int align_once_gate_len(int q, int c) {
+	const int sl = ((q + c) | 1) + 1, al = (q + c) | 2;
+	return sl == al ? 65535 : (sl < al ? sl : al) - 2 - c;
+}
+
+__global__ void split_flag_kernel(int n_reads, const uint32_t *__restrict__ cand_count, const uint16_t *__restrict__ read_len, int gate_len,
+		uint32_t *__restrict__ flag) {
+	const int r = blockIdx.x * blockDim.x + threadIdx.x;
+	if (r > n_reads) return;
+	flag[r] = (r < n_reads && cand_count[r] == 1u && (int) read_len[r] <= gate_len) ? 1u : 0u;
+}
+
+__global__ __launch_bounds__(256) void split_candidates_kernel(int n_reads, const uint32_t *__restrict__ cand_base, const uint32_t *__restrict__ cand_count,
+		const uint32_t *__restrict__ flag_scan, const uint32_t *__restrict__ pair_loc, const uint32_t *__restrict__ pair_sv, int32_t *__restrict__ early_slot,
+		uint32_t *__restrict__ s_read, uint32_t *__restrict__ s_loc, uint32_t *__restrict__ s_sv, uint32_t *__restrict__ s_cand,
+		uint32_t *__restrict__ m_read, uint32_t *__restrict__ m_loc, uint32_t *__restrict__ m_sv, uint32_t *__restrict__ m_cand) {
+	__shared__ uint32_t s_big[256], s_nbig;
+	const int tid = threadIdx.x, lane = tid & 63, wv = tid >> 6;
+	if (tid == 0) s_nbig = 0;
+	__syncthreads();
+	const int r = blockIdx.x * 256 + tid;
+	if (r < n_reads) {
+		const uint32_t b = cand_base[r], n = cand_count[r], before = flag_scan[r];
+		if (flag_scan[r + 1] != before) {
+			s_read[before] = (uint32_t) r; s_loc[before] = pair_loc[b]; s_sv[before] = pair_sv[b]; s_cand[before] = b;
+			early_slot[r] = (int32_t) before;
+		} else {
+			early_slot[r] = -1;
+			if (n <= kSelectSmall) {
+				for (uint32_t j = b; j < b + n; ++j) { const uint32_t at = j - before; m_read[at] = (uint32_t) r; m_loc[at] = pair_loc[j]; m_sv[at] = pair_sv[j]; m_cand[at] = j; }
+			} else s_big[atomicAdd(&s_nbig, 1u)] = (uint32_t) tid;
+		}
+	}
+	__syncthreads();
+	const uint32_t nbig = s_nbig;
+	for (uint32_t i = (uint32_t) wv; i < nbig; i += 4u) {
+		const int rr = blockIdx.x * 256 + (int) s_big[i];
+		const uint32_t b = cand_base[rr], n = cand_count[rr], before = flag_scan[rr];
+		for (uint32_t j = b + (uint32_t) lane; j < b + n; j += 64u) { const uint32_t at = j - before; m_read[at] = (uint32_t) rr; m_loc[at] = pair_loc[j]; m_sv[at] = pair_sv[j]; m_cand[at] = j; }
+	}
+}
+
+__global__ void scatter_scores_kernel(int n_m, const uint32_t *__restrict__ m_cand, const float *__restrict__ m_scores, int n_s,
+		const uint32_t *__restrict__ s_cand, const int32_t *__restrict__ s_records, float *__restrict__ scores) {
+	const int i = blockIdx.x * blockDim.x + threadIdx.x;
+	if (i < n_m) scores[m_cand[i]] = m_scores[i];
+	else if (i - n_m < n_s) scores[s_cand[i - n_m]] = (float) s_records[(size_t) (i - n_m) * 8 + 5];
+}
+
 __global__ void collect_winners_kernel(int n_reads, const uint32_t *__restrict__ winner, const uint32_t *__restrict__ pair_loc,
 		const uint32_t *__restrict__ pair_sv, const uint32_t *__restrict__ slot_of_read, uint32_t *__restrict__ a_read,
 		uint32_t *__restrict__ a_loc, uint32_t *__restrict__ a_sv) {
diff --git a/nextgenmap_amd/csrc/mapper.cpp b/nextgenmap_amd/csrc/mapper.cpp
--- a/nextgenmap_amd/csrc/mapper.cpp
+++ b/nextgenmap_amd/csrc/mapper.cpp
@@ -71,6 +71,60 @@
 	MAP_HIP_TRY(hipEventRecord(m->ev[2], m->st));
 	if (int rc = ngm::engine_score_packed(eng, m->prm.mode, (int) np, m->d_scores.p, m->st)) { ngm::pipeline_set_error("%s", ngm_hip_last_error(eng)); return rc; }
 	MAP_HIP_TRY(hipEventRecord(m->ev[3], m->st));
+	return 0;
+}
+
+int score_candidates_once(ngm_mapper *m, int n, uint64_t np, int *n_early) {
+	const ngm_ref *r = m->ref;
+	ngm_hip_ctx *eng = m->eng;
+	const int q = m->prm.qry_max_len, c = m->prm.corridor;
+	*n_early = 0;
+	size_t tmp_bytes = 0;
+	(void) rocprim::exclusive_scan(nullptr, tmp_bytes, m->d_split_flag.p, m->d_split_scan.p, 0u, (size_t) n + 1, rocprim::plus<uint32_t>(), m->st);
+	if (m->d_split_flag.reserve((size_t) n + 1) || m->d_split_scan.reserve((size_t) n + 1) || m->d_scan_tmp.reserve(tmp_bytes + 16) || m->d_early_slot.reserve(n) || m->d_s_read.reserve(n) ||
+			m->d_s_loc.reserve(n) || m->d_s_sv.reserve(n) || m->d_s_cand.reserve(n) || m->d_m_loc.reserve(np) || m->d_m_sv.reserve(np) || m->d_m_cand.reserve(np) || m->d_m_scores.reserve(np) ||
+			m->p_split_n.reserve(1)) { ngm::pipeline_set_error("out of device memory (candidate split)"); return -12; }
+	hipLaunchKernelGGL(ngm::split_flag_kernel, dim3((n + 256) / 256), dim3(256), 0, m->st, n, m->d_cand_count.p, m->d_read_len.p, ngm::align_once_gate_len(q, c), m->d_split_flag.p);
+	MAP_HIP_TRY(hipGetLastError());
+	MAP_HIP_TRY(rocprim::exclusive_scan(m->d_scan_tmp.p, tmp_bytes, m->d_split_flag.p, m->d_split_scan.p, 0u, (size_t) n + 1, rocprim::plus<uint32_t>(), m->st));
+	MAP_HIP_TRY(hipMemcpyAsync(m->p_split_n.p, m->d_split_scan.p + n, 4, hipMemcpyDeviceToHost, m->st));
+	hipLaunchKernelGGL(ngm::split_candidates_kernel, dim3((n + 255) / 256), dim3(256), 0, m->st, n, m->d_cand_base.p, m->d_cand_count.p, m->d_split_scan.p, m->d_out_loc.p, m->d_out_sv.p,
+			m->d_early_slot.p, m->d_s_read.p, m->d_s_loc.p, m->d_s_sv.p, m->d_s_cand.p, m->d_pair_read.p, m->d_m_loc.p, m->d_m_sv.p, m->d_m_cand.p);
+	MAP_HIP_TRY(hipGetLastError());
+	MAP_HIP_TRY(hipMemsetAsync(m->d_total.p + 8, 0, 16, m->st));
+	MAP_HIP_TRY(hipStreamSynchronize(m->st));
+	const uint64_t ns64 = m->p_split_n.p[0];
+	if (ns64 > (uint64_t) n || ns64 > np) { ngm::pipeline_set_error("candidate split: %llu single-candidate reads of %d reads, %llu candidates", (unsigned long long) ns64, n, (unsigned long long) np); return -5; }
+	const int ns = (int) ns64, nm = (int) (np - ns64);
+	if (nm > 0) {
+		ngm::WindowGeom Gs{r->n_bases - 1, ((q + c) | 1) + 1, c >> 1};
+		hipLaunchKernelGGL(ngm::gather_pairs_kernel, dim3((nm + ngm::kSlots - 1) / ngm::kSlots), dim3(256), 0, m->st, m->d_reads.p, m->d_read_len.p, q, r->d_genome, Gs,
+				m->d_pair_read.p, m->d_m_loc.p, m->d_m_sv.p, nm, eng->RW, eng->FW, eng->packed.p, eng->lens.p, eng->blk_rows.p, 0);
+		MAP_HIP_TRY(hipGetLastError());
+	}
+	MAP_HIP_TRY(hipEventRecord(m->ev[2], m->st));
+	if (nm > 0) if (int rc = ngm::engine_score_packed(eng, m->prm.mode, nm, m->d_m_scores.p, m->st)) { ngm::pipeline_set_error("%s", ngm_hip_last_error(eng)); return rc; }
+	MAP_HIP_TRY(hipEventRecord(m->ev[3], m->st));
+	if (ns > 0) {
+		const unsigned long long scap = (unsigned long long) ns * 96ull + 4096ull;
+		if (m->d_early_rec.reserve((size_t) ns * 8) || m->d_early_cigout.reserve(ns) || m->p_early_cigout.reserve(ns) || m->d_str.reserve(scap + (unsigned long long) n * 96ull + 4096ull)) {
+			ngm::pipeline_set_error("out of memory (early alignments)"); return -12; }
+		ngm::WindowGeom Ga{r->n_bases - 1, (q + c) | 2, c >> 1};
+		hipLaunchKernelGGL(ngm::gather_pairs_kernel, dim3((ns + ngm::kSlots - 1) / ngm::kSlots), dim3(256), 0, m->st, m->d_reads.p, m->d_read_len.p, q, r->d_genome, Ga,
+				m->d_s_read.p, m->d_s_loc.p, m->d_s_sv.p, ns, eng->RW, eng->FW, eng->packed.p, eng->lens.p, eng->blk_rows.p, 0);
+		MAP_HIP_TRY(hipGetLastError());
+		MAP_HIP_TRY(hipEventRecord(m->ev[10], m->st));
+		ngm::AlignFinish fin{m->d_early_cigout.p, m->d_str.p, scap, m->d_total.p + 8};
+		fin.dp_done = m->ev[11];
+		fin.row_limit = (int) ngm::test_limit("finish_row", 0);
+		if (int rc = ngm::engine_align_packed(eng, m->prm.mode, ns, m->d_early_rec.p, nullptr, ngm::run_stride(q, c), m->st, &fin)) { ngm::pipeline_set_error("%s", ngm_hip_last_error(eng)); return rc; }
+		MAP_HIP_TRY(hipEventRecord(m->ev[12], m->st));
+	} else {
+		for (int e = 10; e <= 12; ++e) MAP_HIP_TRY(hipEventRecord(m->ev[e], m->st));
+	}
+	hipLaunchKernelGGL(ngm::scatter_scores_kernel, dim3((unsigned) ((np + 255) / 256)), dim3(256), 0, m->st, nm, m->d_m_cand.p, m->d_m_scores.p, ns, m->d_s_cand.p, m->d_early_rec.p, m->d_scores.p);
+	MAP_HIP_TRY(hipGetLastError());
+	*n_early = ns;
 	return 0;
 }
 }
@@ -168,6 +222,9 @@
 	m->p_winner.release(); m->p_loc.release(); m->p_sv.release(); m->p_mapq.release(); m->p_nbest.release(); m->p_rec.release();
 	m->p_best.release(); m->p_scores.release(); m->p_runs.release();
 	m->d_str.release(); m->d_cigout.release(); m->p_cigout.release(); m->p_str.release();
+	m->d_split_flag.release(); m->d_split_scan.release(); m->d_s_read.release(); m->d_s_loc.release(); m->d_s_sv.release(); m->d_s_cand.release(); m->d_m_loc.release(); m->d_m_sv.release();
+	m->d_m_cand.release(); m->d_early_slot.release(); m->d_early_rec.release(); m->d_m_scores.release(); m->d_early_cigout.release(); m->p_early_cigout.release(); m->p_early_slot.release();
+	m->p_split_n.release();
 	ngm_hip_destroy(m->eng);
 	delete m;
 }
@@ -632,12 +689,20 @@
 		}
 		m->scores_so_far = tot; m->reads_so_far = at;
 	};
+	static const bool once_fits = !getenv("NGM_HIP_HOST_CIGAR") && !getenv("NGM_HIP_ALIGN_TAIL_SPLIT");
+	const char *once_env = getenv("NGM_HIP_ALIGN_ONCE");
+	const bool once = once_fits && !(once_env && atoi(once_env) == 0) && np > 0 && m->prm.personality == NGM_PERSONALITY_AFFINE && (mode & NGM_MODE_ALIGN_MASK) == NGM_MODE_LOCAL && (paired || m->prm.topn <= 1) &&
+			m->prm.strata == 0 && alt_cigar == NGM_ALT_NONE && !m->argos_on && ngm::engine_affine_align_is_packed(eng, mode);
+	int n_early = 0;
+	unsigned long long early_ctr[2] = {0, 0};
+	const int32_t *h_early_slot = nullptr;
 	if (np > 0) {
 		if (m->d_pair_read.reserve(np) || m->d_scores.reserve(np) || m->d_winner.reserve(n) || m->d_mapq.reserve(n) || m->d_nbest.reserve(n) ||
 				m->d_best.reserve(n)) { ngm::pipeline_set_error("out of device memory (score stage)"); return -12; }
 		if (int rc = ngm::engine_reserve(eng, (int) np)) { ngm::pipeline_set_error("%s", ngm_hip_last_error(eng)); return rc; }
 		stage_cs.acquire();
-		if (int rc = ngm::score_candidates(m, n, np, alt_dir)) return rc;
+		if (once) { if (int rc = ngm::score_candidates_once(m, n, np, &n_early)) return rc; }
+		else if (int rc = ngm::score_candidates(m, n, np, alt_dir)) return rc;
 		hipLaunchKernelGGL(ngm::select_top1_kernel, dim3((n + 255) / 256), dim3(256), 0, m->st, n, m->d_cand_base.p, m->d_cand_count.p,
 				m->d_scores.p, m->d_out_loc.p, m->d_out_sv.p, m->d_winner.p, m->d_mapq.p, m->d_nbest.p, m->d_best.p);
 		MAP_HIP_TRY(hipGetLastError());
@@ -686,6 +751,13 @@
 		MAP_HIP_TRY(hipMemcpyAsync(h_loc, m->d_out_loc.p, np * 4, hipMemcpyDeviceToHost, m->st));
 		MAP_HIP_TRY(hipMemcpyAsync(h_sv, m->d_out_sv.p, np * 4, hipMemcpyDeviceToHost, m->st));
 		if (paired) MAP_HIP_TRY(hipMemcpyAsync(h_scores, m->d_scores.p, np * 4, hipMemcpyDeviceToHost, m->st));
+		if (once) {
+			if (m->p_early_slot.reserve(n)) { ngm::pipeline_set_error("out of pinned host memory"); return -12; }
+			MAP_HIP_TRY(hipMemcpyAsync(m->p_early_slot.p, m->d_early_slot.p, (size_t) n * 4, hipMemcpyDeviceToHost, m->st));
+			if (n_early) MAP_HIP_TRY(hipMemcpyAsync(m->p_early_cigout.p, m->d_early_cigout.p, (size_t) n_early * sizeof(ngm::CigarDevOut), hipMemcpyDeviceToHost, m->st));
+			MAP_HIP_TRY(hipMemcpyAsync(early_ctr, m->d_total.p + 8, 16, hipMemcpyDeviceToHost, m->st));
+			h_early_slot = m->p_early_slot.p;
+		}
 		stage_cs.done_after(m->ev[4]);
 		MAP_HIP_TRY(hipStreamSynchronize(m->st));
 		if (int rc = cs_host_arrays(m)) return rc;
@@ -1003,25 +1075,56 @@
 	lap(2);
 	std::vector<uint32_t> a_read((size_t) n * topn), a_loc((size_t) n * topn), a_sv((size_t) n * topn), a_out((size_t) n * topn), a_pair((size_t) n * topn);
 	int na = 0;
+	int nl = 0;
+	std::vector<uint32_t> l_read, l_loc, l_sv;
+	std::vector<int32_t> a_src;
+	auto early_of = [&](int i) -> int {
+		const int s2 = h_early_slot[i];
+		return (s2 >= 0 && (m->p_early_cigout.p[s2].flags & 1)) ? s2 : -1;
+	};
 	if (topn == 1 || np == 0) {
 		const int slices = std::max(1, std::min(256, n / 4096));
-		std::vector<int> first(slices + 1, 0);
+		std::vector<int> first(slices + 1, 0), first_l(slices + 1, 0);
+		std::atomic<uint64_t> oc[5];
+		for (auto &x : oc) x = 0;
 		parallel_for(slices, [&](int lo, int hi) {
 			for (int s2 = lo; s2 < hi; ++s2) {
 				const int i0 = (int) ((long long) n * s2 / slices), i1 = (int) ((long long) n * (s2 + 1) / slices);
 				int cnt = 0;
 				for (int i = i0; i < i1; ++i) cnt += h_winner[i] != 0xFFFFFFFFu;
 				first[s2 + 1] = cnt;
+				if (!h_early_slot) continue;
+				uint64_t c5[5] = {0, 0, 0, 0, 0};
+				for (int i = i0; i < i1; ++i) {
+					const int slot = h_early_slot[i];
+					const bool won = h_winner[i] != 0xFFFFFFFFu, stands = slot >= 0 && early_of(i) >= 0;
+					c5[0] += won && stands; c5[1] += won && !stands;
+					c5[2] += slot < 0 && m->h_count[i] == 1u;
+					c5[3] += !won && stands; c5[4] += slot >= 0 && !stands;
+				}
+				first_l[s2 + 1] = (int) c5[1];
+				for (int x = 0; x < 5; ++x) oc[x] += c5[x];
 			}
 		}, 1);
-		for (int s2 = 0; s2 < slices; ++s2) first[s2 + 1] += first[s2];
+		for (int s2 = 0; s2 < slices; ++s2) { first[s2 + 1] += first[s2]; first_l[s2 + 1] += first_l[s2]; }
 		na = first[slices];
+		if (h_early_slot) {
+			nl = first_l[slices];
+			l_read.resize((size_t) nl + 1); l_loc.resize((size_t) nl + 1); l_sv.resize((size_t) nl + 1); a_src.resize((size_t) na + 1);
+			for (int x = 0; x < 5; ++x) m->once_ctr[x] += oc[x];
+		}
 		parallel_for(slices, [&](int lo, int hi) {
 			for (int s2 = lo; s2 < hi; ++s2) {
 				const int i0 = (int) ((long long) n * s2 / slices), i1 = (int) ((long long) n * (s2 + 1) / slices);
-				int at = first[s2];
+				int at = first[s2], lat = first_l[s2];
 				for (int i = i0; i < i1; ++i) if (h_winner[i] != 0xFFFFFFFFu) {
-					a_read[at] = (uint32_t) i; a_out[at] = (uint32_t) i; a_pair[at] = h_winner[i]; a_loc[at] = h_loc[h_winner[i]]; a_sv[at] = h_sv[h_winner[i]]; ++at;
+					a_read[at] = (uint32_t) i; a_out[at] = (uint32_t) i; a_pair[at] = h_winner[i]; a_loc[at] = h_loc[h_winner[i]]; a_sv[at] = h_sv[h_winner[i]];
+					if (h_early_slot) {
+						const int slot = early_of(i);
+						if (slot >= 0) a_src[at] = -1 - slot;
+						else { a_src[at] = lat; l_read[lat] = a_read[at]; l_loc[lat] = a_loc[at]; l_sv[lat] = a_sv[at]; ++lat; }
+					}
+					++at;
 				}
 			}
 		}, 1);
@@ -1039,39 +1142,44 @@
 	const int align_buf_len = (q + c) | 2;
 	static const bool dev_strings = !getenv("NGM_HIP_HOST_CIGAR");
 	uint64_t str_base = 0;
+	const int ng = h_early_slot ? nl : na;
+	const uint32_t *g_read = h_early_slot ? l_read.data() : a_read.data(), *g_loc = h_early_slot ? l_loc.data() : a_loc.data(), *g_sv = h_early_slot ? l_sv.data() : a_sv.data();
+	if (h_early_slot) str_base = std::min<unsigned long long>(early_ctr[0], (unsigned long long) n_early * 96ull + 4096ull);
 	GpuStage stage_align(m, 1, false);
-	if (na > 0) {
-		if (m->d_a_read.reserve(na) || m->d_a_loc.reserve(na) || m->d_a_sv.reserve(na) || m->d_records.reserve((size_t) na * 8) ||
-				m->d_runs.reserve((size_t) na * rs)) { ngm::pipeline_set_error("out of device memory (align stage)"); return -12; }
-		if (int rc = ngm::engine_reserve(eng, na)) { ngm::pipeline_set_error("%s", ngm_hip_last_error(eng)); return rc; }
-		MAP_HIP_TRY(hipMemcpyAsync(m->d_a_read.p, a_read.data(), (size_t) na * 4, hipMemcpyHostToDevice, m->st));
-		MAP_HIP_TRY(hipMemcpyAsync(m->d_a_loc.p, a_loc.data(), (size_t) na * 4, hipMemcpyHostToDevice, m->st));
-		MAP_HIP_TRY(hipMemcpyAsync(m->d_a_sv.p, a_sv.data(), (size_t) na * 4, hipMemcpyHostToDevice, m->st));
+	if (ng > 0) {
+		if (m->d_a_read.reserve(ng) || m->d_a_loc.reserve(ng) || m->d_a_sv.reserve(ng) || m->d_records.reserve((size_t) ng * 8) ||
+				m->d_runs.reserve((size_t) ng * rs)) { ngm::pipeline_set_error("out of device memory (align stage)"); return -12; }
+		if (int rc = ngm::engine_reserve(eng, ng)) { ngm::pipeline_set_error("%s", ngm_hip_last_error(eng)); return rc; }
+		MAP_HIP_TRY(hipMemcpyAsync(m->d_a_read.p, g_read, (size_t) ng * 4, hipMemcpyHostToDevice, m->st));
+		MAP_HIP_TRY(hipMemcpyAsync(m->d_a_loc.p, g_loc, (size_t) ng * 4, hipMemcpyHostToDevice, m->st));
+		MAP_HIP_TRY(hipMemcpyAsync(m->d_a_sv.p, g_sv, (size_t) ng * 4, hipMemcpyHostToDevice, m->st));
 		MAP_HIP_TRY(hipStreamSynchronize(m->st));
 		stage_align.acquire();
 		MAP_HIP_TRY(hipEventRecord(m->ev[5], m->st));
 		ngm::WindowGeom Ga{r->n_bases - 1, align_buf_len, c >> 1};
-		hipLaunchKernelGGL(ngm::gather_pairs_kernel, dim3((na + ngm::kSlots - 1) / ngm::kSlots), dim3(256), 0, m->st, m->d_reads.p, m->d_read_len.p, q,
-				r->d_genome, Ga, m->d_a_read.p, m->d_a_loc.p, m->d_a_sv.p, na, eng->RW, eng->FW, eng->packed.p, eng->lens.p, eng->blk_rows.p, alt_dir);
+		hipLaunchKernelGGL(ngm::gather_pairs_kernel, dim3((ng + ngm::kSlots - 1) / ngm::kSlots), dim3(256), 0, m->st, m->d_reads.p, m->d_read_len.p, q,
+				r->d_genome, Ga, m->d_a_read.p, m->d_a_loc.p, m->d_a_sv.p, ng, eng->RW, eng->FW, eng->packed.p, eng->lens.p, eng->blk_rows.p, alt_dir);
 		MAP_HIP_TRY(hipGetLastError());
 		MAP_HIP_TRY(hipEventRecord(m->ev[6], m->st));
 		const bool was_prof = eng->profiling;
 		const bool affine = m->prm.personality == NGM_PERSONALITY_AFFINE;
 		static const bool tail_split = getenv("NGM_HIP_ALIGN_TAIL_SPLIT") != nullptr;
 		const bool finish = affine && dev_strings && topn == 1 && !tail_split;
-		const unsigned long long scap = (unsigned long long) na * 96ull + 4096ull;
+		const unsigned long long scap = (unsigned long long) ng * 96ull + 4096ull + (h_early_slot ? (unsigned long long) n_early * 96ull + 4096ull : 0ull);
 		unsigned long long n_runs_total = 0, n_str_total = 0;
-		if (dev_strings && (m->d_cigout.reserve(na) || m->d_str.reserve(scap) || m->p_cigout.reserve(na))) { ngm::pipeline_set_error("out of memory (CIGAR strings)"); return -12; }
+		if (dev_strings && (m->d_cigout.reserve(ng) || m->d_str.reserve(scap) || m->p_cigout.reserve(ng))) { ngm::pipeline_set_error("out of memory (CIGAR strings)"); return -12; }
 		if (finish) {
 			unsigned long long ctr[2] = {0, 0};
-			MAP_HIP_TRY(hipMemsetAsync(m->d_total.p + 8, 0, 16, m->st));
-			const ngm::AlignFinish fin{m->d_cigout.p, m->d_str.p, scap, m->d_total.p + 8};
+			if (h_early_slot) MAP_HIP_TRY(hipMemsetAsync(m->d_total.p + 9, 0, 8, m->st));
+			else MAP_HIP_TRY(hipMemsetAsync(m->d_total.p + 8, 0, 16, m->st));
+			ngm::AlignFinish fin{m->d_cigout.p, m->d_str.p, scap, m->d_total.p + 8};
+			fin.row_limit = (int) ngm::test_limit("finish_row", 0);
 			eng->profiling = true;
-			if (int rc = ngm::engine_align_packed(eng, mode, na, m->d_records.p, m->d_runs.p, rs, m->st, &fin)) { eng->profiling = was_prof; ngm::pipeline_set_error("%s", ngm_hip_last_error(eng)); return rc; }
+			if (int rc = ngm::engine_align_packed(eng, mode, ng, m->d_records.p, m->d_runs.p, rs, m->st, &fin)) { eng->profiling = was_prof; ngm::pipeline_set_error("%s", ngm_hip_last_error(eng)); return rc; }
 			eng->profiling = was_prof;
 			MAP_HIP_TRY(hipEventRecord(m->ev[7], m->st));
 			MAP_HIP_TRY(hipEventRecord(m->ev[8], m->st));
-			MAP_HIP_TRY(hipMemcpyAsync(m->p_cigout.p, m->d_cigout.p, (size_t) na * sizeof(ngm::CigarDevOut), hipMemcpyDeviceToHost, m->st));
+			MAP_HIP_TRY(hipMemcpyAsync(m->p_cigout.p, m->d_cigout.p, (size_t) ng * sizeof(ngm::CigarDevOut), hipMemcpyDeviceToHost, m->st));
 			MAP_HIP_TRY(hipMemcpyAsync(ctr, m->d_total.p + 8, 16, hipMemcpyDeviceToHost, m->st));
 			stage_align.done_after(m->ev[8]);
 			MAP_HIP_TRY(hipStreamSynchronize(m->st));
@@ -1080,13 +1188,13 @@
 			if (m->p_str.reserve(n_str_total + 1)) { ngm::pipeline_set_error("out of pinned host memory"); return -12; }
 			if (n_str_total && !sam) MAP_HIP_TRY(hipMemcpy(m->p_str.p, m->d_str.p, n_str_total, hipMemcpyDeviceToHost));
 			if (ctr[1]) {
-				if (m->d_runs_c.reserve((size_t) na * rs)) { ngm::pipeline_set_error("out of device memory (runs)"); return -12; }
+				if (m->d_runs_c.reserve((size_t) ng * rs)) { ngm::pipeline_set_error("out of device memory (runs)"); return -12; }
 				MAP_HIP_TRY(hipMemsetAsync(m->d_total.p, 0, 8, m->st));
-				if (int rc = ngm::engine_affine_traceback_packed(eng, na, m->d_records.p, m->d_runs.p, rs, m->st)) { ngm::pipeline_set_error("%s", ngm_hip_last_error(eng)); return rc; }
-				hipLaunchKernelGGL(ngm::compact_runs_kernel, dim3((na + 255) / 256), dim3(256), 0, m->st, na, m->d_records.p, m->d_runs.p, rs,
+				if (int rc = ngm::engine_affine_traceback_packed(eng, ng, m->d_records.p, m->d_runs.p, rs, m->st)) { ngm::pipeline_set_error("%s", ngm_hip_last_error(eng)); return rc; }
+				hipLaunchKernelGGL(ngm::compact_runs_kernel, dim3((ng + 255) / 256), dim3(256), 0, m->st, ng, m->d_records.p, m->d_runs.p, rs,
 						m->d_runs_c.p, m->d_total.p);
 				MAP_HIP_TRY(hipGetLastError());
-				MAP_HIP_TRY(hipMemcpyAsync(h_rec, m->d_records.p, (size_t) na * 8 * 4, hipMemcpyDeviceToHost, m->st));
+				MAP_HIP_TRY(hipMemcpyAsync(h_rec, m->d_records.p, (size_t) ng * 8 * 4, hipMemcpyDeviceToHost, m->st));
 				MAP_HIP_TRY(hipMemcpyAsync(&n_runs_total, m->d_total.p, 8, hipMemcpyDeviceToHost, m->st));
 				MAP_HIP_TRY(hipStreamSynchronize(m->st));
 				if (m->p_runs.reserve(n_runs_total + 1)) { ngm::pipeline_set_error("out of pinned host memory"); return -12; }
@@ -1095,29 +1203,29 @@
 			}
 		} else {
 		eng->profiling = true;
-		if (int rc = ngm::engine_align_packed(eng, mode, na, m->d_records.p, m->d_runs.p, rs, m->st)) { eng->profiling = was_prof; ngm::pipeline_set_error("%s", ngm_hip_last_error(eng)); return rc; }
+		if (int rc = ngm::engine_align_packed(eng, mode, ng, m->d_records.p, m->d_runs.p, rs, m->st)) { eng->profiling = was_prof; ngm::pipeline_set_error("%s", ngm_hip_last_error(eng)); return rc; }
 		eng->profiling = was_prof;
 		MAP_HIP_TRY(hipEventRecord(m->ev[7], m->st));
-		if (m->d_runs_c.reserve((size_t) na * rs)) { ngm::pipeline_set_error("out of device memory (runs)"); return -12; }
+		if (m->d_runs_c.reserve((size_t) ng * rs)) { ngm::pipeline_set_error("out of device memory (runs)"); return -12; }
 		MAP_HIP_TRY(hipMemsetAsync(m->d_total.p, 0, 8, m->st));
-		hipLaunchKernelGGL(ngm::compact_runs_kernel, dim3((na + 255) / 256), dim3(256), 0, m->st, na, m->d_records.p, m->d_runs.p, rs,
+		hipLaunchKernelGGL(ngm::compact_runs_kernel, dim3((ng + 255) / 256), dim3(256), 0, m->st, ng, m->d_records.p, m->d_runs.p, rs,
 				m->d_runs_c.p, m->d_total.p);
 		MAP_HIP_TRY(hipGetLastError());
 		if (!dev_strings) { MAP_HIP_TRY(hipEventRecord(m->ev[8], m->st)); }
 		if (dev_strings) {
 			MAP_HIP_TRY(hipMemsetAsync(m->d_total.p + 8, 0, 8, m->st));
-			if (affine) hipLaunchKernelGGL(ngm::cigar_strings_kernel<true>, dim3((na + 255) / 256), dim3(256), 0, m->st, na, m->d_records.p, m->d_runs_c.p, eng->packed.p, eng->RW, eng->FW,
+			if (affine) hipLaunchKernelGGL(ngm::cigar_strings_kernel<true>, dim3((ng + 255) / 256), dim3(256), 0, m->st, ng, m->d_records.p, m->d_runs_c.p, eng->packed.p, eng->RW, eng->FW,
 					m->d_read_len.p, m->d_a_read.p, m->prm.variant == NGM_VARIANT_OCL_CPU ? 1 : 0, m->prm.hard_clip, m->prm.silent_clip, m->d_cigout.p, m->d_str.p, scap,
 					(unsigned long long *) (m->d_total.p + 8), 0);
-			else hipLaunchKernelGGL(ngm::cigar_strings_kernel<false>, dim3((na + 255) / 256), dim3(256), 0, m->st, na, m->d_records.p, m->d_runs_c.p, eng->packed.p, eng->RW, eng->FW,
+			else hipLaunchKernelGGL(ngm::cigar_strings_kernel<false>, dim3((ng + 255) / 256), dim3(256), 0, m->st, ng, m->d_records.p, m->d_runs_c.p, eng->packed.p, eng->RW, eng->FW,
 					m->d_read_len.p, m->d_a_read.p, m->prm.variant == NGM_VARIANT_OCL_CPU ? 1 : 0, m->prm.hard_clip, m->prm.silent_clip, m->d_cigout.p, m->d_str.p, scap,
 					(unsigned long long *) (m->d_total.p + 8), alt_cigar);
 			MAP_HIP_TRY(hipGetLastError());
 			MAP_HIP_TRY(hipEventRecord(m->ev[8], m->st));
-			MAP_HIP_TRY(hipMemcpyAsync(m->p_cigout.p, m->d_cigout.p, (size_t) na * sizeof(ngm::CigarDevOut), hipMemcpyDeviceToHost, m->st));
+			MAP_HIP_TRY(hipMemcpyAsync(m->p_cigout.p, m->d_cigout.p, (size_t) ng * sizeof(ngm::CigarDevOut), hipMemcpyDeviceToHost, m->st));
 			MAP_HIP_TRY(hipMemcpyAsync(&n_str_total, m->d_total.p + 8, 8, hipMemcpyDeviceToHost, m->st));
 		}
-		MAP_HIP_TRY(hipMemcpyAsync(h_rec, m->d_records.p, (size_t) na * 8 * 4, hipMemcpyDeviceToHost, m->st));
+		MAP_HIP_TRY(hipMemcpyAsync(h_rec, m->d_records.p, (size_t) ng * 8 * 4, hipMemcpyDeviceToHost, m->st));
 		MAP_HIP_TRY(hipMemcpyAsync(&n_runs_total, m->d_total.p, 8, hipMemcpyDeviceToHost, m->st));
 		stage_align.done_after(m->ev[8]);
 		MAP_HIP_TRY(hipStreamSynchronize(m->st));
@@ -1133,6 +1241,10 @@
 		}
 	}
 	stage_align.done();
+	if (h_early_slot && ng == 0 && str_base && !sam) {
+		if (m->p_str.reserve(str_base + 1)) { ngm::pipeline_set_error("out of pinned host memory"); return -12; }
+		MAP_HIP_TRY(hipMemcpy(m->p_str.p, m->d_str.p, str_base, hipMemcpyDeviceToHost));
+	}
 
 	lap(3);
 	ngm::SamRef *sam_refs = sam ? m->p_sam_refs.p : nullptr;
@@ -1170,7 +1282,8 @@
 			ao.cigar = sam ? scr.data() : cigars + o * str_stride;
 			ao.md = sam ? scr.data() + str_stride : mds + o * str_stride;
 			bool host_strings = true;
-			const ngm::CigarDevOut *dv = dev_strings ? &m->p_cigout.p[j] : nullptr;
+			const int src = h_early_slot ? a_src[j] : j, jl = src >= 0 ? src : 0;
+			const ngm::CigarDevOut *dv = dev_strings ? (src >= 0 ? &m->p_cigout.p[jl] : &m->p_early_cigout.p[-1 - src]) : nullptr;
 			if (dv && (dv->flags & 1)) {
 				if (!(dv->flags & 2)) { h.mapped = 0; continue; }
 				if (sam) { sam_refs[o] = ngm::SamRef{dv->cig_off, dv->md_off, dv->cig_len, dv->md_len}; host_strings = false; }
@@ -1181,7 +1294,7 @@
 				ao.identity = dv->identity; ao.nm = dv->nm; ao.qstart = dv->qstart; ao.qend = dv->qend; ao.position_offset = dv->position_offset;
 				ao.score_token = dv->score_token;
 			} else if (m->prm.personality == NGM_PERSONALITY_AFFINE) {
-				ngm::build_cigar_affine(&h_rec[(size_t) j * 8], &h_runs[(size_t) (uint32_t) h_rec[(size_t) j * 8 + 6]], nullptr, nullptr, q, &ao, read_length());
+				ngm::build_cigar_affine(&h_rec[(size_t) jl * 8], &h_runs[(size_t) (uint32_t) h_rec[(size_t) jl * 8 + 6]], nullptr, nullptr, q, &ao, read_length());
 				memcpy(ao.md, "!!!", 4);
 			} else {
 				const uint64_t offset = (uint64_t) a_loc[j] - (uint64_t) (c >> 1);
@@ -1194,7 +1307,7 @@
 					qry[t] = ch == 'A' ? 'T' : ch == 'T' ? 'A' : ch == 'C' ? 'G' : ch == 'G' ? 'C' : ch;
 				}
 				const bool second = paired && (i & 1);
-				ngm::build_cigar_md(cp, &h_rec[(size_t) j * 8], &h_runs[(size_t) (uint32_t) h_rec[(size_t) j * 8 + 6]], win.data(), qry.data(), &ao, cp.alt ? ((rev ? !second : second) ? 1 : 0) : 0);
+				ngm::build_cigar_md(cp, &h_rec[(size_t) jl * 8], &h_runs[(size_t) (uint32_t) h_rec[(size_t) jl * 8 + 6]], win.data(), qry.data(), &ao, cp.alt ? ((rev ? !second : second) ? 1 : 0) : 0);
 				if (ao.score_token < 0) { h.mapped = 0; continue; }
 			}
 			if (sam && host_strings) {
@@ -1324,13 +1437,14 @@
 	auto et = [&](int a, int b) { float t = 0; if (hipEventElapsedTime(&t, m->ev[a], m->ev[b]) != hipSuccess) t = 0; return t; };
 	m->ms[0] = m->cs_kernel_ms;
 	m->ms[7] = et(0, 1);
-	if (np > 0) { m->ms[1] = et(1, 2); m->ms[2] = et(2, 3); m->ms[3] = et(3, 4); }
-	if (na > 0) {
+	if (np > 0) { m->ms[1] = et(1, 2); m->ms[2] = et(2, 3); m->ms[3] = once ? et(12, 4) : et(3, 4); }
+	if (ng > 0) {
 		m->ms[4] = et(5, 6);
 		float t = 0;
 		if (hipEventElapsedTime(&t, m->ev[6], eng->ev[2]) == hipSuccess) m->ms[5] = t;
 		if (hipEventElapsedTime(&t, eng->ev[2], m->ev[7]) == hipSuccess) m->ms[6] = t;
 	}
+	if (once) { m->ms[4] += et(3, 10); m->ms[5] += et(10, 11); m->ms[6] += et(11, 12); }
 	return n;
 }
 
@@ -1500,6 +1614,12 @@
 	return 0;
 }
 
+int ngm_mapper_align_once_counters(ngm_mapper *m, uint64_t out[5]) {
+	if (!m || !out) return -22;
+	for (int x = 0; x < 5; ++x) out[x] = m->once_ctr[x];
+	return 0;
+}
+
 int ngm_mapper_order_table_reads(ngm_mapper *m, uint64_t *out) {
 	if (!m || !out) return -22;
 	*out = m->st_order_table;
diff --git a/nextgenmap_amd/csrc/mapper_internal.h b/nextgenmap_amd/csrc/mapper_internal.h
--- a/nextgenmap_amd/csrc/mapper_internal.h
+++ b/nextgenmap_amd/csrc/mapper_internal.h
@@ -116,6 +116,14 @@
 	ngm::DevBuf<ngm::CigarDevOut> d_cigout;
 	ngm::PinnedBuf<ngm::CigarDevOut> p_cigout;
 	ngm::PinnedBuf<char> p_str;
+	ngm::DevBuf<uint32_t> d_split_flag, d_split_scan, d_s_read, d_s_loc, d_s_sv, d_s_cand, d_m_loc, d_m_sv, d_m_cand;
+	ngm::DevBuf<int32_t> d_early_slot, d_early_rec;
+	ngm::DevBuf<float> d_m_scores;
+	ngm::DevBuf<ngm::CigarDevOut> d_early_cigout;
+	ngm::PinnedBuf<ngm::CigarDevOut> p_early_cigout;
+	ngm::PinnedBuf<int32_t> p_early_slot;
+	ngm::PinnedBuf<uint32_t> p_split_n;
+	uint64_t once_ctr[5] = {0, 0, 0, 0, 0};
 	ngm_sam_options sam_opt{};
 	ngm_bgzf *bz = nullptr;
 	ngm_bam_sort *sorter = nullptr;
@@ -158,7 +166,7 @@
 	HostArr<uint32_t> h_base, h_count;
 	HostArr<float> h_maxv;
 	uint64_t n_cand = 0;
-	hipEvent_t ev[10] = {};
+	hipEvent_t ev[13] = {};
 	float ms[8] = {};
 };
 
diff --git a/nextgenmap_amd/csrc/ngm_cli.cpp b/nextgenmap_amd/csrc/ngm_cli.cpp
--- a/nextgenmap_amd/csrc/ngm_cli.cpp
+++ b/nextgenmap_amd/csrc/ngm_cli.cpp
@@ -2104,6 +2104,14 @@
 		snprintf(msg, sizeof(msg), "Heavy-read kernel: %llu second passes, %llu table passes started over, %llu reads sent on to the exact kernels; table pool regrown %llu times",
 				(unsigned long long) hc[0], (unsigned long long) hc[1], (unsigned long long) hc[2], (unsigned long long) hc[3]);
 		info("MAIN", msg);
+		if (getenv("NGM_HIP_HOST_TIMING")) {
+			uint64_t oc[5] = {0, 0, 0, 0, 0};
+			for (Worker &w : workers) { uint64_t c5[5]; if (ngm_mapper_align_once_counters(w.m, c5) == 0) for (int x = 0; x < 5; ++x) oc[x] += c5[x]; }
+			const double nal = (double) std::max<uint64_t>(1, oc[0] + oc[1]);
+			snprintf(msg, sizeof(msg), "Align once: %llu reads aligned in the score stage (%.2f %%), %llu in the align stage; %llu single-candidate reads above the window gate; early alignments dropped %llu, handed to the align stage %llu",
+					(unsigned long long) oc[0], 100.0 * oc[0] / nal, (unsigned long long) oc[1], (unsigned long long) oc[2], (unsigned long long) oc[3], (unsigned long long) oc[4]);
+			info("MAIN", msg);
+		}
 		uint64_t by_table = 0;
 		for (Worker &w : workers) { uint64_t c2 = 0; if (ngm_mapper_order_table_reads(w.m, &c2) == 0) by_table += c2; }
 		snprintf(msg, sizeof(msg), "Candidate order replay: %llu reads, %llu of them beyond the LDS replay (exact replay through buckets in global memory, %llu of them with a table there); order left undetermined for %llu reads",
diff --git a/nextgenmap_amd/csrc/ngm_hip.cpp b/nextgenmap_amd/csrc/ngm_hip.cpp
--- a/nextgenmap_amd/csrc/ngm_hip.cpp
+++ b/nextgenmap_amd/csrc/ngm_hip.cpp
@@ -185,20 +185,27 @@
 	return 0;
 }
 
+static const void *affine_align_pk_kernel(const ngm_hip_ctx *ctx, int mode) {
+	static const bool force32 = getenv("NGM_HIP_ALIGN_32BIT") != nullptr;
+	const int am = mode & NGM_MODE_ALIGN_MASK;
+	const void *pk = nullptr;
+	if (!force32 && am != NGM_MODE_END_TO_END && ctx->KA.open < 0 && ctx->KA.ext < 0 && (long) ctx->q * ctx->KA.tM < 30000 &&
+			ctx->prm.gap_read_penalty + (long) ctx->q * (ctx->prm.gap_extend_penalty + ctx->KA.tZ) < 19000) {
+		const bool plain_key = (long) ctx->q * ctx->prm.match_bonus < 2048 && ctx->c + 1 <= 32;
+		if (plain_key) pk = find_pk_affine_align_kernel(ctx->c, false);
+		else if (ctx->KA.tZ > 0 && ctx->KA.tM > 0 && ctx->KA.tM + 1 <= 63) pk = find_pk_affine_align_kernel(ctx->c, true);
+	}
+	return pk;
+}
+bool engine_affine_align_is_packed(const ngm_hip_ctx *ctx, int mode) { return ctx->prm.personality == NGM_PERSONALITY_AFFINE && affine_align_pk_kernel(ctx, mode) != nullptr; }
+
 int engine_align_packed(ngm_hip_ctx *ctx, int mode, int n, int32_t *d_records, uint16_t *d_runs, int run_stride, hipStream_t st, const AlignFinish *fin) {
 	const int am = mode & NGM_MODE_ALIGN_MASK;
 	const int nb = n_blocks_of(n);
 	if (ctx->prm.personality == NGM_PERSONALITY_AFFINE) {
 		const int CP = ctx->c + 1, ADW = ngm::aff_dir_words(CP);
 		if (ctx->dirs.reserve((size_t) nb * ctx->q * ADW * ngm::kSlots)) { set_error(ctx, "out of device memory for the trace matrix"); return -12; }
-		static const bool force32 = getenv("NGM_HIP_ALIGN_32BIT") != nullptr;
-		const void *pk = nullptr;
-		if (!force32 && am != NGM_MODE_END_TO_END && ctx->KA.open < 0 && ctx->KA.ext < 0 && (long) ctx->q * ctx->KA.tM < 30000 &&
-				ctx->prm.gap_read_penalty + (long) ctx->q * (ctx->prm.gap_extend_penalty + ctx->KA.tZ) < 19000) {
-			const bool plain_key = (long) ctx->q * ctx->prm.match_bonus < 2048 && ctx->c + 1 <= 32;
-			if (plain_key) pk = find_pk_affine_align_kernel(ctx->c, false);
-			else if (ctx->KA.tZ > 0 && ctx->KA.tM > 0 && ctx->KA.tM + 1 <= 63) pk = find_pk_affine_align_kernel(ctx->c, true);
-		}
+		const void *pk = affine_align_pk_kernel(ctx, mode);
 		if (pk) {
 			KernelRef kp; kp.aot = pk;
 			HIP_TRY(ctx, launch_kernel(kp, dim3((nb + 7) / 8), dim3(256), st, (const uint32_t *) ctx->packed.p, (const uint16_t *) ctx->lens.p,
@@ -209,12 +216,14 @@
 					(const uint16_t *) ctx->blk_rows.p, (float *) nullptr, ctx->dirs.p, d_records, n, nb, ctx->RW, ctx->q, ctx->KA));
 		}
 		if (ctx->profiling) HIP_TRY(ctx, hipEventRecord(ctx->ev[2], st));
+		if (fin && fin->dp_done) HIP_TRY(ctx, hipEventRecord(fin->dp_done, st));
 		ctx->trace_nibbles = pk != nullptr;
+		const int lim = (fin && fin->row_limit > 0) ? std::min(fin->row_limit, ngm::kCigarRow - 16) : ngm::kCigarRow - 16;
 		if (!fin) return engine_affine_traceback_packed(ctx, n, d_records, d_runs, run_stride, st);
 		if (pk) hipLaunchKernelGGL(ngm::affine_finish_kernel<true>, dim3((n + 255) / 256), dim3(256), 0, st, n, (const uint32_t *) ctx->dirs.p, (const int32_t *) d_records,
-				(const uint32_t *) ctx->packed.p, (const uint16_t *) ctx->lens.p, ctx->q, CP, ctx->RW, ctx->FW, fin->out, fin->bytes, fin->capacity, fin->counters);
+				(const uint32_t *) ctx->packed.p, (const uint16_t *) ctx->lens.p, ctx->q, CP, ctx->RW, ctx->FW, fin->out, fin->bytes, fin->capacity, fin->counters, lim);
 		else hipLaunchKernelGGL(ngm::affine_finish_kernel<false>, dim3((n + 255) / 256), dim3(256), 0, st, n, (const uint32_t *) ctx->dirs.p, (const int32_t *) d_records,
-				(const uint32_t *) ctx->packed.p, (const uint16_t *) ctx->lens.p, ctx->q, CP, ctx->RW, ctx->FW, fin->out, fin->bytes, fin->capacity, fin->counters);
+				(const uint32_t *) ctx->packed.p, (const uint16_t *) ctx->lens.p, ctx->q, CP, ctx->RW, ctx->FW, fin->out, fin->bytes, fin->capacity, fin->counters, lim);
 		HIP_TRY(ctx, hipGetLastError());
 		return 0;
 	}
diff --git a/nextgenmap_amd/pipeline.py b/nextgenmap_amd/pipeline.py
--- a/nextgenmap_amd/pipeline.py
+++ b/nextgenmap_amd/pipeline.py
@@ -81,6 +81,7 @@
         lib.ngm_mapper_path_counters.argtypes = [C.c_void_p, C.c_void_p]
         lib.ngm_mapper_order_table_reads.argtypes = [C.c_void_p, C.c_void_p]
         lib.ngm_mapper_heavy_counters.argtypes = [C.c_void_p, C.c_void_p]
+        lib.ngm_mapper_align_once_counters.argtypes = [C.c_void_p, C.c_void_p]
         lib.ngm_mapper_last_kernel_ms.argtypes = [C.c_void_p, C.POINTER(C.c_float)]
         lib.ngm_mapper_last_order_replay_ms.restype = C.c_float
         lib.ngm_mapper_last_order_replay_ms.argtypes = [C.c_void_p]
@@ -452,6 +453,11 @@
         self.lib.ngm_mapper_heavy_counters(self.h, out.ctypes.data)
         return dict(zip(("second_passes", "table_pass_restarts", "sent_on", "pool_regrown"), (int(x) for x in out)))
 
+    def align_once_counters(self):
+        out = np.zeros(5, np.uint64)
+        self.lib.ngm_mapper_align_once_counters(self.h, out.ctypes.data)
+        return dict(zip(("early", "late", "above_gate", "discarded", "handed_over"), (int(x) for x in out)))
+
     def order_table_reads(self):
         out = np.zeros(1, np.uint64)
         self.lib.ngm_mapper_order_table_reads(self.h, out.ctypes.data)
```

Measured after the change: 49.44 million. 0.865x the previous value.
